# UVA-Computer-Vision-Lab/FrameINO

Measured on AMD Instinct MI355X. Metric: denoise-steps/sec (Wan2.2-5B FrameINO, 49f 704x1280, cond+uncond DiT forward + CFG + Euler), higher is better.
Workload: dtype bf16; 1 GPU; wan2.2-5b-49f-704x1280; layers=30, id_frames=1, hip_graph=False, parallelism=single, dead_rows_last_block=1760

## Files before the change

### frameino_amd/_lib.py

```python
import ctypes
import os
import re

_HERE = os.path.dirname(os.path.abspath(__file__))
LIB_PATH = os.environ.get("FINO_LIB_PATH") or os.path.join(_HERE, "lib", "libframeino_hip.so")
HEADER_PATH = os.path.join(os.path.dirname(_HERE), "include", "frameino_hip.h")

c_void_p, c_int, c_i64, c_float = ctypes.c_void_p, ctypes.c_int, ctypes.c_int64, ctypes.c_float

SIGNATURES = {
    "fino_version": [],
    "fino_last_error": [],
    "fino_tune_set": [c_int, c_int],
    "fino_tune_get": [c_int],
    "fino_adaln_modulate": [c_void_p, c_void_p, c_i64, c_int, c_i64, c_i64, c_void_p, c_void_p, c_i64, c_void_p,
                            c_float, c_int, c_void_p],
    "fino_layernorm": [c_void_p, c_void_p, c_i64, c_int, c_i64, c_i64, c_void_p, c_void_p, c_float, c_int, c_void_p],
    "fino_gated_residual": [c_void_p, c_void_p, c_void_p, c_i64, c_int, c_i64, c_i64, c_i64, c_void_p, c_i64,
                            c_void_p, c_int, c_void_p],
    "fino_gated_residual_staged": [c_void_p, c_void_p, c_void_p, c_i64, c_int, c_i64, c_i64, c_i64, c_void_p, c_i64,
                                   c_void_p, c_int, c_void_p],
    "fino_layernorm_zero": [c_void_p, c_void_p, c_i64, c_int, c_i64, c_i64, c_void_p, c_void_p, c_void_p, c_void_p,
                            c_i64, c_void_p, c_float, c_int, c_void_p],
    "fino_rmsnorm_rope": [c_void_p, c_i64, c_int, c_i64, c_void_p, c_float, c_void_p, c_void_p, c_int, c_int,
                          c_void_p],
    "fino_rmsnorm_rope_scaled": [c_void_p, c_i64, c_int, c_i64, c_void_p, c_float, c_void_p, c_void_p, c_int, c_float,
                                 c_int, c_void_p],
    "fino_qkv_rmsnorm_rope": [c_void_p, c_i64, c_int, c_i64, c_void_p, c_float, c_void_p, c_float, c_void_p, c_void_p, c_int,
                              c_float, c_void_p, c_void_p, c_void_p, c_int, c_void_p],
    "fino_rmsnorm_rope_scatter": [c_void_p, c_i64, c_int, c_i64, c_void_p, c_float, c_void_p, c_void_p, c_int, c_float,
                                  c_void_p, c_void_p, c_void_p, c_int, c_void_p],
    "fino_diag_mfma_peak": [c_int, c_int, c_int, c_void_p, ctypes.POINTER(ctypes.c_double), c_void_p],
    "fino_headnorm_rope": [c_void_p, c_int, c_i64, c_int, c_int, c_i64, c_i64, c_void_p, c_void_p, c_float,
                           c_void_p, c_void_p, c_i64, c_int, c_void_p],
    "fino_headnorm_rope_scaled": [c_void_p, c_int, c_i64, c_int, c_int, c_i64, c_i64, c_void_p, c_void_p, c_float,
                                  c_void_p, c_void_p, c_i64, c_float, c_int, c_void_p],
    "fino_attn_fwd": [c_void_p] * 4 + [c_int, c_int, c_i64, c_i64, c_int] + [c_i64] * 12 + [c_float, c_int, c_void_p],
    "fino_attn_fwd_ws": [c_void_p] * 4 + [c_int, c_int, c_i64, c_i64, c_int] + [c_i64] * 12 +
                        [c_float, c_int, c_void_p, c_i64, c_void_p],
    "fino_attn_workspace_bytes": [c_int, c_int, c_i64, c_i64, c_int],
    "fino_attn_tail_supported": [c_int, c_int, c_i64, c_i64, c_int],
    "fino_attn_ranges_supported": [c_int, c_int, c_i64, c_i64, c_int],
    "fino_attn_fwd_ranges": [c_void_p] * 4 + [c_int, c_int, c_i64, c_i64, c_int] + [c_i64] * 12 + [c_float, c_int, c_void_p, c_void_p],
    "fino_attn_tiles_supported": [c_int, c_int, c_i64, c_i64, c_int],
    "fino_attn_fwd_tiles": [c_void_p] * 4 + [c_int, c_int, c_i64, c_i64, c_int] + [c_i64] * 12 + [c_float, c_int, c_void_p, c_i64, c_i64,
                                                                                             c_int, c_void_p],
    "fino_attn_tile_plan_bytes": [c_int, c_int, c_i64, c_i64, c_int],
    "fino_attn_tile_plan": [c_void_p] * 2 + [c_int, c_int, c_i64, c_i64, c_int] + [c_i64] * 6 + [c_float, c_int, c_float, c_void_p,
                                                                                             c_void_p, c_int, c_void_p, c_i64, c_void_p],
    "fino_attn_tile_plan_gated_bytes": [c_int, c_int, c_i64, c_i64, c_int],
    "fino_attn_tile_plan_gated": [c_void_p] * 2 + [c_int, c_int, c_i64, c_i64, c_int] + [c_i64] * 6 +
                                 [c_float, c_int, c_float, c_void_p, c_float, c_void_p, c_void_p, c_int, c_void_p, c_i64, c_void_p],
    "fino_attn_fp8_ranges_supported": [c_int, c_int, c_i64, c_i64, c_int],
    "fino_attn_fwd_fp8_ranges": [c_void_p] * 4 + [c_int, c_int, c_i64, c_i64, c_int] + [c_i64] * 8 + [c_float, c_int, c_int, c_void_p,
                                                                                               c_i64, c_int, c_void_p, c_void_p],
    "fino_attn_fwd_tail": [c_void_p] * 4 + [c_int, c_int, c_i64, c_i64, c_int] + [c_i64] * 12 + [c_float, c_int, c_void_p, c_void_p,
                                                                                            c_void_p],
    "fino_attn_probs_supported": [c_int, c_int, c_i64, c_i64, c_int],
    "fino_attn_probs": [c_void_p] * 3 + [c_int, c_int, c_i64, c_i64, c_int] + [c_i64] * 6 + [c_int, c_i64, c_i64, c_float, c_int,
                                                                                         c_void_p, c_void_p, c_void_p, c_i64,
                                                                                         c_void_p, c_void_p],
    "fino_row_rrms": [c_void_p, c_i64, c_int, c_i64, c_float, c_void_p, c_int, c_void_p],
    "fino_attn_fp8_kv_bytes": [c_int, c_int, c_i64, c_int],
    "fino_attn_fwd_fp8": [c_void_p] * 4 + [c_int, c_int, c_i64, c_i64, c_int] + [c_i64] * 8 + [c_float, c_int, c_int, c_void_p,
                                                                                           c_i64, c_void_p],
    "fino_attn_fp8_smooth_kv_bytes": [c_int, c_int, c_i64, c_int],
    "fino_attn_fwd_fp8_smooth": [c_void_p] * 4 + [c_int, c_int, c_i64, c_i64, c_int] + [c_i64] * 8 + [c_float, c_int, c_int,
                                                                                                  c_void_p, c_i64, c_void_p],
    "fino_attn_fp8_smoothed_kv_bytes": [c_int, c_int, c_i64, c_int, c_int],
    "fino_attn_fwd_fp8_smoothed": [c_void_p] * 4 + [c_int, c_int, c_i64, c_i64, c_int] + [c_i64] * 8 + [c_float, c_int, c_int,
                                                                                                    c_void_p, c_i64, c_void_p, c_int],
    "fino_attn_fp8_tiles_supported": [c_int, c_int, c_i64, c_i64, c_int],
    "fino_attn_fwd_fp8_tiles": [c_void_p] * 4 + [c_int, c_int, c_i64, c_i64, c_int] + [c_i64] * 8 + [c_float, c_int, c_int,
                                                                                                 c_void_p, c_i64, c_int, c_void_p,
                                                                                                 c_i64, c_i64, c_int, c_void_p],
    "fino_attn_partial_bytes": [c_int, c_int, c_i64, c_int],
    "fino_attn_partial": [c_void_p] * 3 + [c_int, c_int, c_i64, c_i64, c_int] + [c_i64] * 9 + [c_float, c_int, c_void_p,
                                                                                               c_i64, c_void_p],
    "fino_attn_merge": [c_void_p, c_int, c_int, c_i64, c_int, c_i64, c_i64, c_i64, c_void_p, c_void_p, c_void_p, c_int,
                        c_void_p],
    "fino_mxfp8_scale_bytes": [c_i64, c_i64],
    "fino_quantize_mxfp8": [c_void_p, c_void_p, c_void_p, c_i64, c_i64, c_i64, c_int, c_void_p],
    "fino_gemm_mxfp8": [c_void_p] * 6 + [c_i64] * 4 + [c_int, c_void_p, c_i64, c_void_p, c_i64, c_void_p, c_int, c_void_p],
    "fino_gemm_mxfp8_keep": [c_void_p] * 6 + [c_i64] * 4 + [c_int, c_void_p, c_i64, c_void_p, c_i64, c_void_p, c_int, c_void_p,
                             c_i64, c_void_p],
    "fino_gemm_mxfp8_q": [c_void_p] * 7 + [c_i64] * 3 + [c_int, c_int, c_void_p],
    "fino_mxfp6_bytes": [c_i64, c_i64],
    "fino_mxfp6_scale_bytes": [c_i64, c_i64],
    "fino_quantize_mxfp6": [c_void_p, c_void_p, c_void_p, c_i64, c_i64, c_i64, c_int, c_void_p],
    "fino_quantize_mxfp6_rot": [c_void_p, c_void_p, c_void_p, c_i64, c_i64, c_i64, c_int, c_int, c_void_p],
    "fino_gemm_mxfp6": [c_void_p] * 6 + [c_i64] * 4 + [c_int, c_void_p, c_i64, c_void_p, c_i64, c_void_p, c_int, c_void_p],
    "fino_gemm_mxfp6_keep": [c_void_p] * 6 + [c_i64] * 4 + [c_int, c_void_p, c_i64, c_void_p, c_i64, c_void_p, c_int, c_void_p,
                             c_i64, c_void_p],
    "fino_traj_paint": [c_void_p, c_void_p, c_void_p, c_int, c_int, c_int, c_int, c_void_p],
    "fino_traj_blur_quantize": [c_void_p, c_void_p, c_void_p, c_void_p, c_int, c_int, c_int, c_int, c_void_p],
    "fino_groupnorm_workspace_bytes": [c_int],
    "fino_groupnorm_cl": [c_void_p, c_void_p] + [c_int] * 6 + [c_void_p, c_void_p, c_float, c_void_p, c_void_p] +
                         [c_int] * 4 + [c_void_p, c_i64, c_int, c_void_p],
    "fino_avg_pool_time2": [c_void_p, c_void_p] + [c_int] * 5 + [c_void_p],
    "fino_resize_area_pad_u8": [c_void_p, c_void_p] + [c_int] * 9 + [c_void_p],
    "fino_u8_hwc_to_chw_unit": [c_void_p, c_void_p, c_int, c_int, c_void_p],
    "fino_gemm": [c_void_p] * 4 + [c_i64] * 6 + [c_int, c_void_p, c_i64, c_void_p, c_i64, c_void_p, c_int, c_void_p],
    "fino_gemm_split_n": [c_void_p] * 4 + [c_i64] * 6 + [c_int, c_void_p, c_i64, c_void_p, c_i64, c_void_p, c_int, c_void_p,
                          c_i64, c_i64, c_int, c_void_p],
    "fino_gemm_keep": [c_void_p] * 4 + [c_i64] * 6 + [c_int, c_void_p, c_i64, c_void_p, c_i64, c_void_p, c_int, c_void_p,
                       c_i64, c_int, c_void_p],
    "fino_ln_mxfp8": [c_int, c_void_p, c_void_p, c_void_p, c_i64, c_int, c_i64, c_void_p, c_void_p, c_void_p, c_void_p, c_i64,
                      c_void_p, c_float, c_int, c_void_p],
    "fino_gemm_blocked_a": [c_void_p, c_void_p, c_void_p, c_void_p, c_i64, c_i64, c_i64, c_i64, c_i64, c_int, c_i64, c_i64, c_i64,
                            c_i64, c_void_p, c_i64, c_void_p, c_i64, c_void_p, c_int, c_int, c_void_p],
    "fino_gemm_plan": [c_i64, c_i64, ctypes.POINTER(c_i64), ctypes.POINTER(c_int)],
    "fino_skinny_linear": [c_void_p, c_void_p, c_void_p, c_void_p, c_int, c_i64, c_i64, c_int, c_int, c_void_p],
    "fino_patchify": [c_void_p, c_void_p] + [c_int] * 7 + [c_i64, c_int, c_void_p],
    "fino_unpatchify": [c_void_p, c_void_p] + [c_int] * 7 + [c_i64, c_int, c_void_p],
    "fino_wan_model_input": [c_void_p] * 5 + [c_int] * 6 + [c_void_p],
    "fino_cfg_euler_step": [c_void_p, c_void_p, c_void_p] + [c_int] * 5 + [c_float, c_void_p, c_int, c_int, c_void_p],
    "fino_cfg_unipc_step": [c_void_p] * 6 + [c_int] * 5 + [c_void_p, c_int, c_void_p],
    "fino_cfg_vpred_step": [c_void_p, c_void_p, c_i64, c_i64, c_void_p, c_int, c_int, c_void_p],
    "fino_cfg_dpm_step": [c_void_p, c_void_p, c_void_p, c_void_p, c_i64, c_i64, c_void_p, c_int, c_int, c_void_p],
    "fino_conv3d": [c_void_p] * 4 + [c_int] * 19 + [c_void_p, c_void_p, c_int, c_void_p],
    "fino_rmsnorm_silu_cl": [c_void_p, c_void_p, c_i64, c_int, c_int, c_void_p, c_int, c_int, c_void_p],
    "fino_split_bf16": [c_void_p, c_void_p, c_i64, c_int, c_i64, c_i64, c_int, ctypes.c_uint, c_void_p],
    "fino_rmsnorm_silu_cl_f32": [c_void_p, c_void_p, c_i64, c_int, c_int, c_void_p, c_int, c_int, ctypes.c_uint, c_void_p],
    "fino_conv3d_split": [c_void_p] * 4 + [c_int] * 20 + [c_void_p, c_void_p, c_void_p],
    "fino_vae_blend_tiles": [c_void_p, c_void_p] + [c_int] * 9 + [c_void_p],
    "fino_softmax_rows": [c_void_p, c_i64, c_int, c_i64, c_float, c_int, c_void_p],
    "fino_dup_up3d_add": [c_void_p] * 3 + [c_int] * 10 + [c_void_p],
    "fino_avg_down3d_add": [c_void_p] * 3 + [c_int] * 10 + [c_void_p],
    "fino_vae_unpatchify_clamp": [c_void_p, c_void_p] + [c_int] * 7 + [c_void_p],
    "fino_vae_patchify": [c_void_p, c_void_p] + [c_int] * 7 + [c_void_p],
    "fino_lora_merge": [c_void_p, c_i64, c_void_p, c_i64, c_i64, c_i64, c_int, ctypes.POINTER(c_void_p),
                        ctypes.POINTER(c_i64), ctypes.POINTER(c_void_p), ctypes.POINTER(c_i64), ctypes.POINTER(c_int),
                        ctypes.POINTER(c_float), c_int, c_void_p],
    "fino_step_cache_probe": [c_void_p, c_int, c_i64, c_void_p, c_void_p, c_int, c_void_p],
    "fino_step_cache_residual": [c_void_p, c_i64, c_void_p, c_i64, c_void_p, c_i64, c_i64, c_i64, c_int, c_int, c_void_p],
    "fino_pab_broadcast": [c_void_p, c_i64, c_void_p, c_i64, c_void_p, c_i64, c_i64, c_i64, c_void_p, c_i64, c_void_p, c_int,
                           c_void_p],
    "fino_taylor_update": [c_void_p, c_i64, c_void_p, c_i64, c_i64, c_i64, c_i64, c_int, c_int, c_int, c_int, c_int, c_void_p],
    "fino_taylor_predict": [c_void_p, c_i64, c_i64, c_int, ctypes.POINTER(c_float), c_void_p, c_i64, c_void_p, c_i64, c_i64, c_i64,
                            c_void_p, c_i64, c_void_p, c_int, c_int, c_void_p],
}


class StepCacheSegment(ctypes.Structure):
    _fields_ = [("h0", c_void_p), ("h1", c_void_p), ("p", c_void_p), ("r", c_void_p), ("h1_copy", c_void_p),
                ("rows", c_i64), ("ld_h0", c_i64), ("ld_h1", c_i64), ("ld_p", c_i64), ("ld_r", c_i64), ("ld_h1_copy", c_i64)]
_RESTYPES = {"fino_last_error": ctypes.c_char_p, "fino_attn_workspace_bytes": c_i64, "fino_mxfp8_scale_bytes": c_i64,
             "fino_groupnorm_workspace_bytes": c_i64,
             "fino_attn_partial_bytes": c_i64, "fino_attn_fp8_kv_bytes": c_i64, "fino_attn_fp8_smooth_kv_bytes": c_i64,
             "fino_attn_fp8_smoothed_kv_bytes": c_i64, "fino_mxfp6_bytes": c_i64,
             "fino_mxfp6_scale_bytes": c_i64, "fino_attn_tile_plan_bytes": c_i64,
             "fino_attn_tile_plan_gated_bytes": c_i64}


ABI_VERSION = 103


def declared_symbols(header_path=HEADER_PATH):
    text = open(header_path).read()
    text = re.sub(r"/\*.*?\*/", "", text, flags=re.S)
    return sorted(set(re.findall(r"\b(fino_[a-z0-9_]+)\s*\(", text)))


def load(path=LIB_PATH):
    if not os.path.exists(path):
        raise RuntimeError(
            f"frameino_amd: HIP library not found at {path}. Build it with `python -c 'import __graft_entry__ as g; "
            f"g.build()'` (or `make -C frameino_amd/csrc`). There is no CPU fallback for the product path.")
    lib = ctypes.CDLL(path)
    lib.fino_version.restype = c_int
    if lib.fino_version() < 0 and os.environ.get("FINO_ALLOW_EXPERIMENT") != "1":
        raise RuntimeError(
            f"frameino_amd: {path} is a timing-EXPERIMENT build (compiled with -DFINO_EXPERIMENT: its kernels may skip "
            f"work and return wrong results; fino_version() = {lib.fino_version()}).  It is refused as the product library; "
            f"set FINO_ALLOW_EXPERIMENT=1 for the tools/ scripts that time it.")
    if abs(lib.fino_version()) != ABI_VERSION:
        raise RuntimeError(
            f"frameino_amd: {path} reports fino_version() = {lib.fino_version()}, this package binds ABI version "
            f"{ABI_VERSION} (include/frameino_hip.h: FINO_VERSION).  Rebuild it (`make -C frameino_amd/csrc`).")
    for name, argtypes in SIGNATURES.items():
        fn = getattr(lib, name)
        fn.argtypes = argtypes
        fn.restype = _RESTYPES.get(name, c_int)
    return lib


_lib = None


def lib():
    global _lib
    if _lib is None:
        _lib = load()
    return _lib


def check(rc, what=""):
    if rc != 0:
        raise RuntimeError(f"{what} failed ({rc}): {lib().fino_last_error().decode()}")
```

### frameino_amd/csrc/fino_attention_probs.hip

```cpp
#include <stdlib.h>

#include "fino_attention_common.h"
using namespace fino_attn_ns;

namespace {

struct ProbsParams {
    const uint16_t* q;
    const uint16_t* k;
    uint16_t* p;
    int batch, heads, lq, lk;
    int64_t q_bs, q_rs, q_hs, k_bs, k_rs, k_hs, p_bs, p_rs;
    int kp;
    const float* q_rrms;
    const uint16_t* q_weight;
    int64_t q_rrms_bs;
    float scale_log2;
    int lk_b[4];
    float log2_mult[4];
};

template <typename T, int NKB>
__global__ __launch_bounds__(256) void attn_probs_kernel(const ProbsParams p) {
    typedef typename T::vec8 vec8;
    __shared__ __attribute__((aligned(16))) char smem[4 * 8192];
    const int tid = threadIdx.x;
    const int lane = tid & 63;
    const int wave = tid >> 6;
    const int r = lane & 31;
    const int h = lane >> 5;
    const int hb = blockIdx.y;
    const int bi = hb / p.heads;
    const int head = hb - bi * p.heads;

    const int lkc = p.lk_b[bi < 4 ? bi : 3];
    const float lm = p.log2_mult[bi < 4 ? bi : 3];
    const int nkb = (lkc + 31) >> 5;
    const uint16_t* kp_ = p.k + bi * p.k_bs + head * p.k_hs;
    for (int i = 0; i < nkb * 2; ++i) {
        const int c = tid + 256 * i;
        const int row = c >> 4, ch = c & 15;
        uint4 u = make_uint4(0, 0, 0, 0);
        if (row < p.lk) u = *reinterpret_cast<const uint4*>(kp_ + (int64_t)row * p.k_rs + ch * 8);
        *reinterpret_cast<uint4*>(smem + row * 256 + ((ch ^ (row & 15)) << 4)) = u;
    }
    const int qrow = blockIdx.x * 128 + wave * 32 + r;
    const int qrc = qrow < p.lq ? qrow : p.lq - 1;
    const uint16_t* qp = p.q + bi * p.q_bs + head * p.q_hs + (int64_t)qrc * p.q_rs + 8 * h;
    vec8 qf[8];
    if (p.q_rrms) {
        const float rs = p.q_rrms[bi * p.q_rrms_bs + qrc];
        const uint16_t* wp = p.q_weight + head * 128 + 8 * h;
#pragma unroll
        for (int ks = 0; ks < 8; ++ks) {
            float f[8], ww[8];
            unpack8<T>(*reinterpret_cast<const uint4*>(qp + 16 * ks), f);
            unpack8<T>(*reinterpret_cast<const uint4*>(wp + 16 * ks), ww);
#pragma unroll
            for (int j = 0; j < 8; ++j) f[j] = round_to<T>(round_to<T>(f[j] * rs) * ww[j]);
            qf[ks] = __builtin_bit_cast(vec8, pack8<T>(f));
        }
    } else {
#pragma unroll
        for (int ks = 0; ks < 8; ++ks) qf[ks] = __builtin_bit_cast(vec8, *reinterpret_cast<const uint4*>(qp + 16 * ks));
    }
    __syncthreads();

    f32x16_t acc[NKB];
#pragma unroll
    for (int kb = 0; kb < NKB; ++kb)
#pragma unroll
        for (int j = 0; j < 16; ++j) acc[kb][j] = 0.f;
#pragma unroll
    for (int kb = 0; kb < NKB; ++kb) {
        if (kb < nkb) {
#pragma unroll
            for (int ks = 0; ks < 8; ++ks) {
                const int row = kb * 32 + r;
                const uint4 a = *reinterpret_cast<const uint4*>(smem + row * 256 + (((2 * ks + h) ^ (row & 15)) << 4));
                acc[kb] = T::mfma32(__builtin_bit_cast(vec8, a), qf[ks], acc[kb]);
            }
        }
    }

    const float c2 = p.scale_log2;
    float m = -INFINITY;
#pragma unroll
    for (int kb = 0; kb < NKB; ++kb) {
#pragma unroll
        for (int j = 0; j < 16; ++j) {
            const int key = kb * 32 + (j & 3) + 8 * (j >> 2) + 4 * h;
            float x = acc[kb][j] * c2;
            x = key == lkc - 1 ? x + lm : x;
            x = key >= lkc ? -INFINITY : x;
            acc[kb][j] = x;
            m = fmaxf(m, x);
        }
    }
    {
        const auto sw = __builtin_amdgcn_permlane32_swap(__float_as_uint(m), __float_as_uint(m), false, false);
        m = fmaxf(__uint_as_float(sw[0]), __uint_as_float(sw[1]));
    }
    float l = 0.f;
#pragma unroll
    for (int kb = 0; kb < NKB; ++kb) {
#pragma unroll
        for (int j = 0; j < 16; ++j) {
            const float e = __builtin_amdgcn_exp2f(acc[kb][j] - m);
            acc[kb][j] = e;
            l += e;
        }
    }
    {
        const auto sw = __builtin_amdgcn_permlane32_swap(__float_as_uint(l), __float_as_uint(l), false, false);
        l = __uint_as_float(sw[0]) + __uint_as_float(sw[1]);
    }
    const float inv = 1.0f / l;
    __syncthreads();
    char* stage = smem + wave * 8192;
#pragma unroll
    for (int kb = 0; kb < NKB; ++kb) {
#pragma unroll
        for (int g4 = 0; g4 < 4; ++g4) {
            const int key0 = kb * 32 + 8 * g4 + 4 * h;
            if (key0 < p.kp) {
                const uint32_t w0 = (uint32_t)T::from_f32(acc[kb][4 * g4 + 0] * inv) | ((uint32_t)T::from_f32(acc[kb][4 * g4 + 1] * inv) << 16);
                const uint32_t w1 = (uint32_t)T::from_f32(acc[kb][4 * g4 + 2] * inv) | ((uint32_t)T::from_f32(acc[kb][4 * g4 + 3] * inv) << 16);
                *reinterpret_cast<uint2*>(stage + r * 256 + ((((key0 >> 3)) ^ (r & 15)) << 4) + ((key0 & 4) << 1)) = make_uint2(w0, w1);
            }
        }
    }
    __syncthreads();
    const int pieces = p.kp >> 3;
    const int total = 32 * pieces;
    const int row_base = blockIdx.x * 128 + wave * 32;
    uint16_t* pbase = p.p + bi * p.p_bs + head * p.kp;
    for (int i = lane; i < total; i += 64) {
        const int rr = i / pieces, pc = i - rr * pieces;
        const uint4 u = *reinterpret_cast<const uint4*>(stage + rr * 256 + ((pc ^ (rr & 15)) << 4));
        if (row_base + rr < p.lq) *reinterpret_cast<uint4*>(pbase + (int64_t)(row_base + rr) * p.p_rs + pc * 8) = u;
    }
}

}

extern "C" int fino_attn_probs_supported(int batch, int heads, int64_t lq, int64_t lk, int head_dim) {
    return head_dim == 128 && batch >= 1 && batch <= 4 && heads > 0 && lq > 0 && lk >= 1 && lk <= 128 &&
           (int64_t)batch * heads <= 65535;
}

extern "C" int fino_attn_probs(const void* q, const void* k, void* p, int batch, int heads, int64_t lq, int64_t lk,
                               int head_dim, int64_t q_bs, int64_t q_rs, int64_t q_hs, int64_t k_bs, int64_t k_rs, int64_t k_hs,
                               int kp, int64_t p_bs, int64_t p_rs, float scale, int dtype, const int* lk_b,
                               const float* tail_mult, const float* q_rrms, int64_t q_rrms_bs, const void* q_weight,
                               void* stream) {
    FINO_CHECK((q_rrms == nullptr) == (q_weight == nullptr) && fino_aligned16(q_weight), FINO_ERR_ARG,
               "fino_attn_probs: q_rrms and q_weight come together (q_weight 16-byte aligned)");
    FINO_CHECK(dtype == FINO_BF16 || dtype == FINO_F16, FINO_ERR_ARG, "fino_attn_probs: dtype %d", dtype);
    FINO_CHECK(q && k && p && lk_b && tail_mult, FINO_ERR_ARG, "fino_attn_probs: null pointer");
    FINO_CHECK(fino_attn_probs_supported(batch, heads, lq, lk, head_dim), FINO_ERR_UNSUPPORTED,
               "fino_attn_probs: needs head_dim 128, batch <= 4, lk <= 128 (got head_dim %d, batch %d, lk %lld)", head_dim, batch,
               (long long)lk);
    FINO_CHECK(fino_aligned16(q) && fino_aligned16(k) && fino_aligned16(p) && q_rs % 8 == 0 && k_rs % 8 == 0 && q_hs % 8 == 0 &&
                   k_hs % 8 == 0 && q_bs % 8 == 0 && k_bs % 8 == 0 && p_bs % 8 == 0 && p_rs % 8 == 0,
               FINO_ERR_ARG, "fino_attn_probs: pointers and strides must be 16-byte aligned");
    FINO_CHECK(kp > 0 && kp % 8 == 0 && kp <= 128 && p_rs >= (int64_t)heads * kp, FINO_ERR_ARG,
               "fino_attn_probs: kp %d (a multiple of 8, <= 128), row stride %lld", kp, (long long)p_rs);
    FINO_CHECK(scale > 0.f || scale == FINO_ATTN_SCALE_FOLDED, FINO_ERR_ARG, "fino_attn_probs: scale");
    if (lq == 0) return FINO_OK;
    ProbsParams pp;
    pp.q = (const uint16_t*)q; pp.k = (const uint16_t*)k; pp.p = (uint16_t*)p;
    pp.batch = batch; pp.heads = heads; pp.lq = (int)lq; pp.lk = (int)lk;
    pp.q_bs = q_bs; pp.q_rs = q_rs; pp.q_hs = q_hs; pp.k_bs = k_bs; pp.k_rs = k_rs; pp.k_hs = k_hs; pp.p_bs = p_bs; pp.p_rs = p_rs;
    pp.kp = kp;
    pp.q_rrms = q_rrms; pp.q_weight = (const uint16_t*)q_weight; pp.q_rrms_bs = q_rrms_bs;
    pp.scale_log2 = scale == FINO_ATTN_SCALE_FOLDED ? 1.0f : scale * 1.4426950408889634f;
    for (int b = 0; b < 4; ++b) {
        const int bb = b < batch ? b : batch - 1;
        FINO_CHECK(lk_b[bb] >= 1 && lk_b[bb] <= lk && lk_b[bb] <= kp && tail_mult[bb] >= 1.0f, FINO_ERR_ARG,
                   "fino_attn_probs: lk_b[%d] = %d (of %lld, kp %d), tail_mult %g", bb, lk_b[bb], (long long)lk, kp,
                   (double)tail_mult[bb]);
        pp.lk_b[b] = lk_b[bb];
        pp.log2_mult[b] = log2f(tail_mult[bb]);
    }
    hipStream_t st = (hipStream_t)stream;
    const dim3 grid((unsigned)((lq + 127) / 128), (unsigned)(batch * heads));
    int max_lk = 0;
    for (int b = 0; b < batch; ++b) max_lk = lk_b[b] > max_lk ? lk_b[b] : max_lk;
    const int need = max_lk > kp ? max_lk : kp;
    const int nkb = need <= 64 ? 2 : (need <= 96 ? 3 : 4);
#define PROBS_LAUNCH(T_)                                                                                      \
    {                                                                                                         \
        if (nkb == 2) attn_probs_kernel<T_, 2><<<grid, 256, 0, st>>>(pp);                                     \
        else if (nkb == 3) attn_probs_kernel<T_, 3><<<grid, 256, 0, st>>>(pp);                                \
        else attn_probs_kernel<T_, 4><<<grid, 256, 0, st>>>(pp);                                              \
    }
    if (dtype == FINO_BF16) PROBS_LAUNCH(BF16) else PROBS_LAUNCH(F16)
#undef PROBS_LAUNCH
    FINO_LAUNCH_CHECK();
    return FINO_OK;
}
```

### frameino_amd/csrc/fino_gemm.hip

```cpp
#include <stdlib.h>

#include <atomic>
#include <type_traits>

#include "fino_gemm_common.h"

using namespace fino_gemm_ns;

#ifdef FINO_GEMM_STAMP
extern "C" int fino_gemm_debug_read(unsigned long long* out) {
    return (int)hipMemcpyFromSymbol(out, HIP_SYMBOL(fino_gemm_dbg), sizeof(unsigned long long) * 64);
}
#endif

namespace {

template <typename T, int EPI, bool GENERIC, bool CONV, bool KEEP = false>
__global__ __launch_bounds__(kThreads, 2) void gemm_kernel(const GemmParams p) {
    extern __shared__ __attribute__((aligned(16))) char smem[];
    typedef typename T::vec8 vec8;
    const int tid = threadIdx.x;
    const int lane = tid & 63;
    const int wave = tid >> 6;
    const int wm = wave >> 2;
// ... 518 lines not shown
    FINO_LAUNCH_CHECK();
    return FINO_OK;
}

template <typename T, int EPI, bool CONV = false, int MI = 8, bool ABLK = false, bool KEEP = false>
int launch_gemm_pp(const GemmParams& p, hipStream_t st) {
    static FinoPerDeviceOnce once;
    if (int rc = fino_max_smem_once(once, reinterpret_cast<const void*>(&gemm_pp_kernel<T, EPI, CONV, MI, ABLK, KEEP>), kSmemBytes, "fino_gemm")) return rc;
    gemm_pp_kernel<T, EPI, CONV, MI, ABLK, KEEP><<<dim3((unsigned)(p.tiles_m * p.tiles_n)), kThreads, kSmemBytes, st>>>(p);
    FINO_LAUNCH_CHECK();
    return FINO_OK;
}

inline int gemm_device_cus() {
    static std::atomic<int> cus[kFinoMaxDevices];
    const int dev = fino_current_device();
    int c = cus[dev].load(std::memory_order_relaxed);
    if (c == 0) {
        int n = 0;
        c = (hipDeviceGetAttribute(&n, hipDeviceAttributeMultiprocessorCount, dev) == hipSuccess && n > 0) ? n : 256;
        cus[dev].store(c, std::memory_order_relaxed);
    }
    return c;
}

struct TilePlan { int64_t rows1; int mi2; };
inline double plan_launch_cost(int64_t rows, int mi, int tiles_n, int cus) {
    if (rows <= 0) return 0.0;
    const double bm = 32.0 * mi;
    const int64_t tiles = ((rows + 32 * mi - 1) / (32 * mi)) * tiles_n;
    const double mfma_raw = 0.85 * bm / 256.0, mfma = mfma_raw > 0.80 ? mfma_raw : 0.80, deliver = (bm + 256.0) / 512.0;
    const int64_t full = tiles / cus, rem = tiles % cus;
    double c = (double)full * (mfma > deliver ? mfma : deliver);
    if (rem) {
        const double d = deliver * (double)rem / cus;
        c += mfma > d ? mfma : d;
    }
    return c + 0.07;
}
inline TilePlan plan_tiles_search(int64_t m, int tiles_n, int cus);
inline TilePlan plan_tiles(int64_t m, int tiles_n, int cus, int tile_m = 0) {
    const int forced = tile_m ? tile_m : fino_tune_get(FINO_TUNE_GEMM_TILE_M);
    if (forced >= 2 && forced <= 7) return TilePlan{0, forced};
    if (forced == 8 || m <= 0) return TilePlan{m, 8};
    static std::atomic<uint64_t> memo[64];
    const bool memoable = m < (1ll << 24) && tiles_n > 0 && tiles_n < 512 && cus > 0 && cus < 512;
    const uint64_t key = ((uint64_t)m << 18) | ((uint64_t)tiles_n << 9) | (uint64_t)cus;
    std::atomic<uint64_t>& slot = memo[(key * 0x9E3779B97F4A7C15ull) >> 58];
    if (memoable) {
        const uint64_t e = slot.load(std::memory_order_relaxed);
        if ((e & 1) && (e >> 22) == key) {
            const uint64_t r = (e >> 6) & 0xffff;
            return TilePlan{r == 0xffff ? m : (int64_t)r * 256, (int)((e >> 3) & 7) + 1};
        }
    }
    const TilePlan tp = plan_tiles_search(m, tiles_n, cus);
    if (memoable && (tp.rows1 == m || (tp.rows1 % 256 == 0 && tp.rows1 / 256 < 0xffff)) && tp.mi2 >= 2 && tp.mi2 <= 8)
        slot.store((key << 22) | ((tp.rows1 == m ? 0xffffull : (uint64_t)(tp.rows1 / 256)) << 6) |
                       ((uint64_t)(tp.mi2 - 1) << 3) | 1ull, std::memory_order_relaxed);
    return tp;
}
inline TilePlan plan_tiles_search(int64_t m, int tiles_n, int cus) {
    TilePlan best{m, 8};
    double best_c = plan_launch_cost(m, 8, tiles_n, cus);
    const double base_c = best_c;
    const int64_t rows256 = (m + 255) / 256;
    for (int64_t r1 = 0; r1 < rows256; ++r1) {
        const int64_t rows1 = r1 * 256;
        const double c1 = plan_launch_cost(rows1, 8, tiles_n, cus);
        for (int mi = 2; mi <= 8; ++mi) {
            if (rows1 > 0 && mi == 8) continue;
            const double c = c1 + plan_launch_cost(m - rows1, mi, tiles_n, cus);
            if (c < best_c - 1e-9) { best_c = c; best = TilePlan{rows1, mi}; }
        }
    }
    if (best_c > (best.rows1 > 0 ? 0.97 : 0.985) * base_c) return TilePlan{m, 8};
    return best;
}

inline bool use_pingpong() {
    static int v = -1;
    if (v < 0) {
        const char* e = getenv("FINO_GEMM_PP");
        v = (e && e[0] == '0') ? 0 : 1;
    }
    return v == 1;
}

template <typename T, int EPI, bool KEEP = false>
int launch_gemm_pp_mi(const GemmParams& p, int mi, hipStream_t st) {
    if constexpr (KEEP) {
        switch (mi) {
            case 2: return launch_gemm_pp<T, EPI, false, 2, false, true>(p, st);
            case 3: return launch_gemm_pp<T, EPI, false, 3, false, true>(p, st);
            case 4: return launch_gemm_pp<T, EPI, false, 4, false, true>(p, st);
            case 5: return launch_gemm_pp<T, EPI, false, 5, false, true>(p, st);
            case 6: return launch_gemm_pp<T, EPI, false, 6, false, true>(p, st);
            case 7: return launch_gemm_pp<T, EPI, false, 7, false, true>(p, st);
            default: return launch_gemm_pp<T, EPI, false, 8, false, true>(p, st);
        }
    }
    if (p.a_tpb > 0) {
        if constexpr (EPI == FINO_EPI_GATED_RESIDUAL) {
            switch (mi) {
                case 2: return launch_gemm_pp<T, EPI, false, 2, true>(p, st);
                case 3: return launch_gemm_pp<T, EPI, false, 3, true>(p, st);
                case 4: return launch_gemm_pp<T, EPI, false, 4, true>(p, st);
                case 5: return launch_gemm_pp<T, EPI, false, 5, true>(p, st);
                case 6: return launch_gemm_pp<T, EPI, false, 6, true>(p, st);
                case 7: return launch_gemm_pp<T, EPI, false, 7, true>(p, st);
                default: return launch_gemm_pp<T, EPI, false, 8, true>(p, st);
            }
        } else {
            fino_set_error("fino_gemm_blocked_a: epilogue must be FINO_EPI_GATED_RESIDUAL");
            return FINO_ERR_UNSUPPORTED;
        }
    }
    switch (mi) {
        case 2: return launch_gemm_pp<T, EPI, false, 2>(p, st);
        case 3: return launch_gemm_pp<T, EPI, false, 3>(p, st);
        case 4: return launch_gemm_pp<T, EPI, false, 4>(p, st);
        case 5: return launch_gemm_pp<T, EPI, false, 5>(p, st);
        case 6: return launch_gemm_pp<T, EPI, false, 6>(p, st);
        case 7: return launch_gemm_pp<T, EPI, false, 7>(p, st);
        default: return launch_gemm_pp<T, EPI, false, 8>(p, st);
    }
}

template <typename T, bool KEEP = false>
int launch_gemm_rows(GemmParams p, int64_t r0, int64_t rows, int mi, int epi, hipStream_t st) {
    p.a += r0 * p.lda;
    p.c += r0 * p.ldc;
    if (p.c2) p.c2 += r0 * p.ldc2;
    if (p.r) p.r += r0 * p.ldr;
    if (p.sel) p.sel += r0;
    p.m = rows;
    p.tiles_m = (int)((rows + 32 * mi - 1) / (32 * mi));
    if constexpr (KEEP) {
        switch (epi) {
            case FINO_EPI_RESIDUAL: return launch_gemm_pp_mi<T, FINO_EPI_RESIDUAL, true>(p, mi, st);
            case FINO_EPI_GATED_RESIDUAL_STAGED: return launch_gemm_pp_mi<T, FINO_EPI_GATED_RESIDUAL_STAGED, true>(p, mi, st);
            default: return launch_gemm_pp_mi<T, FINO_EPI_GATED_RESIDUAL, true>(p, mi, st);
        }
    }
    switch (epi) {
        case FINO_EPI_NONE: return launch_gemm_pp_mi<T, FINO_EPI_NONE>(p, mi, st);
        case FINO_EPI_GELU_TANH: return launch_gemm_pp_mi<T, FINO_EPI_GELU_TANH>(p, mi, st);
        case FINO_EPI_RESIDUAL: return launch_gemm_pp_mi<T, FINO_EPI_RESIDUAL>(p, mi, st);
        case FINO_EPI_GATED_RESIDUAL_STAGED: return launch_gemm_pp_mi<T, FINO_EPI_GATED_RESIDUAL_STAGED>(p, mi, st);
        default: return launch_gemm_pp_mi<T, FINO_EPI_GATED_RESIDUAL>(p, mi, st);
    }
}

template <typename T, bool GENERIC, bool KEEP = false>
int launch_gemm_e(const GemmParams& p, int epi, int tile_m, hipStream_t st) {
    const bool fits32 = ((p.m - 1) * p.lda + p.k) * 2 < (1ll << 31) && ((p.n - 1) * p.ldw + p.k) * 2 < (1ll << 31);
    if (epi == FINO_EPI_F32 || epi == FINO_EPI_F32_RESIDUAL) {
        if (GENERIC || !fits32) {
            fino_set_error("fino_gemm: the fp32-output epilogues need K %% 64 == 0, 16-byte aligned operands and operands < 2 GiB");
            return FINO_ERR_UNSUPPORTED;
        }
        return epi == FINO_EPI_F32 ? launch_gemm_pp<T, FINO_EPI_F32, false, 8>(p, st)
                                   : launch_gemm_pp<T, FINO_EPI_F32_RESIDUAL, false, 8>(p, st);
    }
    if (!GENERIC && use_pingpong() && fits32) {
        const TilePlan tp = plan_tiles(p.m, p.tiles_n, gemm_device_cus(), tile_m);
        if (tp.rows1 > 0)
            if (int rc = launch_gemm_rows<T, KEEP>(p, 0, tp.rows1, 8, epi, st)) return rc;
        if (tp.rows1 < p.m) return launch_gemm_rows<T, KEEP>(p, tp.rows1, p.m - tp.rows1, tp.mi2, epi, st);
        return FINO_OK;
    }
    if constexpr (KEEP) {
        switch (epi) {
            case FINO_EPI_RESIDUAL: return launch_gemm_t<T, FINO_EPI_RESIDUAL, GENERIC, false, true>(p, st);
            case FINO_EPI_GATED_RESIDUAL_STAGED: return launch_gemm_t<T, FINO_EPI_GATED_RESIDUAL_STAGED, GENERIC, false, true>(p, st);
            default: return launch_gemm_t<T, FINO_EPI_GATED_RESIDUAL, GENERIC, false, true>(p, st);
        }
    }
    switch (epi) {
        case FINO_EPI_NONE: return launch_gemm_t<T, FINO_EPI_NONE, GENERIC>(p, st);
        case FINO_EPI_GELU_TANH: return launch_gemm_t<T, FINO_EPI_GELU_TANH, GENERIC>(p, st);
        case FINO_EPI_RESIDUAL: return launch_gemm_t<T, FINO_EPI_RESIDUAL, GENERIC>(p, st);
        case FINO_EPI_GATED_RESIDUAL_STAGED: return launch_gemm_t<T, FINO_EPI_GATED_RESIDUAL_STAGED, GENERIC>(p, st);
        default: return launch_gemm_t<T, FINO_EPI_GATED_RESIDUAL, GENERIC>(p, st);
    }
}

template <int WT>
__global__ __launch_bounds__(256) void skinny_linear_kernel(const float* __restrict__ x, const void* __restrict__ w,
                                                            const void* __restrict__ b, float* __restrict__ y, int m,
                                                            int64_t n, int64_t k, int silu_input) {
    const int lane = threadIdx.x & 63;
    const int64_t col = (int64_t)blockIdx.x * 4 + (threadIdx.x >> 6);
    if (col >= n) return;
    float acc[16];
#pragma unroll
    for (int i = 0; i < 16; ++i) acc[i] = 0.f;
    for (int64_t kk = lane; kk < k; kk += 64) {
        float wv;
        if (WT == -1) wv = ((const float*)w)[col * k + kk];
        else if (WT == FINO_BF16) wv = BF16::to_f32(((const uint16_t*)w)[col * k + kk]);
        else wv = F16::to_f32(((const uint16_t*)w)[col * k + kk]);
#pragma unroll
        for (int i = 0; i < 16; ++i) {
            if (i < m) {
                float xv = x[(int64_t)i * k + kk];
                if (silu_input) xv = xv / (1.0f + __expf(-xv));
                acc[i] += xv * wv;
            }
        }
    }
    float bias = 0.f;
    if (b) {
        if (WT == -1) bias = ((const float*)b)[col];
        else if (WT == FINO_BF16) bias = BF16::to_f32(((const uint16_t*)b)[col]);
        else bias = F16::to_f32(((const uint16_t*)b)[col]);
    }
#pragma unroll
    for (int i = 0; i < 16; ++i) {
        if (i < m) {
            const float s = wave_sum(acc[i]);
            if (lane == 0) y[(int64_t)i * n + col] = s + bias;
        }
    }
}

}

extern "C" int fino_gemm_plan(int64_t m, int64_t n, int64_t* rows_256, int* tile_rows_rest) {
    if (m <= 0 || n <= 0) return FINO_ERR_ARG;
    const TilePlan tp = plan_tiles(m, (int)((n + BN - 1) / BN), gemm_device_cus());
    if (rows_256) *rows_256 = tp.rows1;
    if (tile_rows_rest) *tile_rows_rest = tp.rows1 < m ? 32 * tp.mi2 : 0;
    return FINO_OK;
}

extern "C" int fino_gemm(const void* a, const void* w, const void* bias, void* c, int64_t m, int64_t n, int64_t k,
                         int64_t lda, int64_t ldw, int64_t ldc, int epilogue, const void* r, int64_t ldr,
                         const float* gate, int64_t mod_stride, const int32_t* sel, int dtype, void* stream) {
    return fino_gemm_split_n(a, w, bias, c, m, n, k, lda, ldw, ldc, epilogue, r, ldr, gate, mod_stride, sel, dtype, nullptr,
                             0, 0, 0, stream);
}

static int gemm_impl(const void* a, const void* w, const void* bias, void* c, int64_t m, int64_t n, int64_t k, int64_t lda,
                     int64_t ldw, int64_t ldc, int epilogue, const void* r, int64_t ldr, const float* gate,
                     int64_t mod_stride, const int32_t* sel, int dtype, void* c2, int64_t ldc2, int64_t n_split, void* keep,
                     int64_t ldk, int tile_m, void* stream) {
    FINO_CHECK(dtype == FINO_BF16 || dtype == FINO_F16, FINO_ERR_ARG, "fino_gemm: dtype %d", dtype);
    FINO_CHECK(tile_m == 0 || (tile_m >= 2 && tile_m <= 8), FINO_ERR_ARG, "fino_gemm: tile_m=%d (0 = planned, 2 .. 8)", tile_m);
    if (c2 || n_split) {
        FINO_CHECK(c2 && n_split > 0 && n_split < n && n_split % BN == 0 && ldc2 % 8 == 0 && ldc2 >= n - n_split &&
                       fino_aligned16(c2) && k % BK == 0 && epilogue <= FINO_EPI_GELU_TANH,
                   FINO_ERR_ARG,
                   "fino_gemm_split_n: needs c2, 0 < n_split < N a multiple of %d, ldc2 >= N - n_split, K %% %d == 0, no "
                   "residual epilogue", BN, BK);
        FINO_CHECK(ldc >= n_split, FINO_ERR_ARG, "fino_gemm_split_n: ldc must cover the first n_split columns");
    }
    FINO_CHECK(a && w && c, FINO_ERR_ARG, "fino_gemm: null pointer");
    FINO_CHECK(m >= 0 && n > 0 && k > 0, FINO_ERR_ARG, "fino_gemm: bad shape M=%lld N=%lld K=%lld", (long long)m,
               (long long)n, (long long)k);
    FINO_CHECK(n % 8 == 0 && k % 8 == 0, FINO_ERR_ARG, "fino_gemm: N=%lld and K=%lld must be multiples of 8",
               (long long)n, (long long)k);
    FINO_CHECK(lda % 8 == 0 && ldw % 8 == 0 && ldc % 8 == 0 && lda >= k && ldw >= k && ldc >= (n_split > 0 ? n_split : n),
               FINO_ERR_ARG, "fino_gemm: leading dimensions must be multiples of 8 and cover the row");
    FINO_CHECK(fino_aligned16(a) && fino_aligned16(w) && fino_aligned16(c), FINO_ERR_ARG,
               "fino_gemm: A/W/C must be 16-byte aligned");
    FINO_CHECK(epilogue >= FINO_EPI_NONE && epilogue <= FINO_EPI_F32_RESIDUAL, FINO_ERR_ARG,
               "fino_gemm: epilogue %d", epilogue);
    if (epilogue == FINO_EPI_F32 || epilogue == FINO_EPI_F32_RESIDUAL)
        FINO_CHECK(!c2 && tile_m == 0 && fino_aligned16(bias), FINO_ERR_ARG,
                   "fino_gemm: the fp32-output epilogues take one output, the planned tiling and a 16-byte aligned fp32 bias");
    if (epilogue >= FINO_EPI_RESIDUAL && epilogue != FINO_EPI_F32)
        FINO_CHECK(r && ldr % 8 == 0 && ldr >= n && fino_aligned16(r), FINO_ERR_ARG, "fino_gemm: residual operand");
    if (epilogue == FINO_EPI_GATED_RESIDUAL || epilogue == FINO_EPI_GATED_RESIDUAL_STAGED)
        FINO_CHECK(gate && fino_aligned16(gate) && mod_stride % 4 == 0, FINO_ERR_ARG, "fino_gemm: gate operand");
    if (m == 0) return FINO_OK;
    GemmParams p = {};
    p.c2 = (uint16_t*)c2; p.ldc2 = ldc2; p.n_split = n_split;
    if (keep) { p.c2 = (uint16_t*)keep; p.ldc2 = ldk; p.n_split = 0; }
    p.a = (const uint16_t*)a; p.w = (const uint16_t*)w; p.bias = (const uint16_t*)bias; p.c = (uint16_t*)c;
    p.r = (const uint16_t*)r; p.gate = gate; p.sel = sel;
    p.m = m; p.n = n; p.k = k; p.lda = lda; p.ldw = ldw; p.ldc = ldc; p.ldr = ldr; p.mod_stride = mod_stride;
    p.tiles_m = (int)((m + BM - 1) / BM);
    p.tiles_n = (int)((n + BN - 1) / BN);
    p.group_m = fino_tune_get(FINO_TUNE_GEMM_GROUP_M);
    hipStream_t st = (hipStream_t)stream;
    const bool generic = (k % BK) != 0;
    if (p.group_m <= 0) p.group_m = gemm_default_group_m(p.tiles_n, k);
    {
        const int rk = fino_tune_get(FINO_TUNE_GEMM_RASTER);
        if (rk == 1 || (rk == 3 && (k >= 8192 || n >= 8192)) || (rk != 2 && rk != 3 && k >= 8192)) p.group_m |= 0x100;
    }
    if (keep) {
        if (dtype == FINO_BF16)
            return generic ? launch_gemm_e<BF16, true, true>(p, epilogue, tile_m, st)
                           : launch_gemm_e<BF16, false, true>(p, epilogue, tile_m, st);
        return generic ? launch_gemm_e<F16, true, true>(p, epilogue, tile_m, st)
                       : launch_gemm_e<F16, false, true>(p, epilogue, tile_m, st);
    }
    if (dtype == FINO_BF16)
        return generic ? launch_gemm_e<BF16, true>(p, epilogue, tile_m, st) : launch_gemm_e<BF16, false>(p, epilogue, tile_m, st);
    return generic ? launch_gemm_e<F16, true>(p, epilogue, tile_m, st) : launch_gemm_e<F16, false>(p, epilogue, tile_m, st);
}

extern "C" int fino_gemm_split_n(const void* a, const void* w, const void* bias, void* c, int64_t m, int64_t n, int64_t k,
                                 int64_t lda, int64_t ldw, int64_t ldc, int epilogue, const void* r, int64_t ldr,
                                 const float* gate, int64_t mod_stride, const int32_t* sel, int dtype, void* c2,
                                 int64_t ldc2, int64_t n_split, int tile_m, void* stream) {
    return gemm_impl(a, w, bias, c, m, n, k, lda, ldw, ldc, epilogue, r, ldr, gate, mod_stride, sel, dtype, c2, ldc2, n_split,
                     nullptr, 0, tile_m, stream);
}

extern "C" int fino_gemm_keep(const void* a, const void* w, const void* bias, void* c, int64_t m, int64_t n, int64_t k,
                              int64_t lda, int64_t ldw, int64_t ldc, int epilogue, const void* r, int64_t ldr,
                              const float* gate, int64_t mod_stride, const int32_t* sel, int dtype, void* keep, int64_t ldk,
                              int tile_m, void* stream) {
    FINO_CHECK(dtype == FINO_BF16 || dtype == FINO_F16, FINO_ERR_ARG, "fino_gemm_keep: dtype %d", dtype);
    FINO_CHECK(epilogue == FINO_EPI_RESIDUAL || epilogue == FINO_EPI_GATED_RESIDUAL ||
                   epilogue == FINO_EPI_GATED_RESIDUAL_STAGED,
               FINO_ERR_ARG, "fino_gemm_keep: epilogue %d (the residual epilogues %d, %d and %d keep y)", epilogue,
               FINO_EPI_RESIDUAL, FINO_EPI_GATED_RESIDUAL, FINO_EPI_GATED_RESIDUAL_STAGED);
    FINO_CHECK(keep && fino_aligned16(keep) && ldk % 8 == 0 && ldk >= n, FINO_ERR_ARG,
               "fino_gemm_keep: needs a 16-byte aligned keep buffer with ldk >= N a multiple of 8");
    return gemm_impl(a, w, bias, c, m, n, k, lda, ldw, ldc, epilogue, r, ldr, gate, mod_stride, sel, dtype, nullptr, 0, 0,
                     keep, ldk, tile_m, stream);
}

extern "C" int fino_gemm_blocked_a(const void* a, const void* w, const void* bias, void* c, int64_t m, int64_t n, int64_t k,
                                   int64_t a_block_k, int64_t a_block_stride, int a_groups, int64_t a_group_stride,
                                   int64_t lda, int64_t ldw, int64_t ldc,
                                   const void* r, int64_t ldr, const float* gate, int64_t mod_stride, const int32_t* sel,
                                   int dtype, int tile_m, void* stream) {
    FINO_CHECK(dtype == FINO_BF16 || dtype == FINO_F16, FINO_ERR_ARG, "fino_gemm_blocked_a: dtype %d", dtype);
    FINO_CHECK(tile_m == 0 || (tile_m >= 2 && tile_m <= 8), FINO_ERR_ARG, "fino_gemm_blocked_a: tile_m=%d (0 = planned, 2 .. 8)",
               tile_m);
    FINO_CHECK(a && w && c && r && gate, FINO_ERR_ARG, "fino_gemm_blocked_a: null pointer");
    FINO_CHECK(m >= 0 && n > 0 && k > 0 && n % 8 == 0, FINO_ERR_ARG, "fino_gemm_blocked_a: bad shape");
    FINO_CHECK(a_block_k > 0 && a_block_k % BK == 0 && k % a_block_k == 0 && a_block_k / BK <= 256 && k / BK <= 4096,
               FINO_ERR_ARG, "fino_gemm_blocked_a: a_block_k=%lld must be a multiple of %d dividing K=%lld",
               (long long)a_block_k, BK, (long long)k);
    FINO_CHECK(lda % 8 == 0 && lda >= a_block_k && a_block_stride % 8 == 0 && ldw % 8 == 0 && ldw >= k && ldc % 8 == 0 &&
                   ldc >= n && ldr % 8 == 0 && ldr >= n && mod_stride % 4 == 0,
               FINO_ERR_ARG, "fino_gemm_blocked_a: leading dimensions");
    FINO_CHECK(fino_aligned16(a) && fino_aligned16(w) && fino_aligned16(c) && fino_aligned16(r) && fino_aligned16(gate),
               FINO_ERR_ARG, "fino_gemm_blocked_a: 16-byte alignment required");
    const int64_t nblk = k / a_block_k;
    FINO_CHECK(a_groups >= 1 && a_groups <= 16 && nblk % a_groups == 0 && a_group_stride % 8 == 0, FINO_ERR_ARG,
               "fino_gemm_blocked_a: a_groups=%d must divide the %lld K blocks", a_groups, (long long)nblk);
    const int64_t span = ((a_groups - 1) * a_group_stride + (nblk / a_groups - 1) * a_block_stride +
                          (m > 0 ? m - 1 : 0) * lda + a_block_k) * 2;
    FINO_CHECK(span < (1ll << 31) && ((n - 1) * ldw + k) * 2 < (1ll << 31), FINO_ERR_ARG,
               "fino_gemm_blocked_a: operands must span < 2 GiB");
    if (m == 0) return FINO_OK;
    GemmParams p = {};
    p.a = (const uint16_t*)a; p.w = (const uint16_t*)w; p.bias = (const uint16_t*)bias; p.c = (uint16_t*)c;
    p.r = (const uint16_t*)r; p.gate = gate; p.sel = sel;
    p.m = m; p.n = n; p.k = k; p.lda = lda; p.ldw = ldw; p.ldc = ldc; p.ldr = ldr; p.mod_stride = mod_stride;
    p.a_tpb = (int)(a_block_k / BK); p.a_inv = (65536 + p.a_tpb - 1) / p.a_tpb; p.a_blk_elems = a_block_stride;
    p.a_groups = a_groups; p.a_ginv = (65536 + a_groups - 1) / a_groups; p.a_grp_elems = a_group_stride;
    FINO_CHECK((k / BK - 1) * ((int64_t)p.a_inv * p.a_tpb - 65536) < 65536 &&
                   (nblk - 1) * ((int64_t)p.a_ginv * a_groups - 65536) < 65536,
               FINO_ERR_UNSUPPORTED,
               "fino_gemm_blocked_a: a_block_k=%lld / a_groups=%d with K=%lld is beyond the exact range of the kernel's "
               "reciprocal index arithmetic", (long long)a_block_k, a_groups, (long long)k);
    p.tiles_m = (int)((m + BM - 1) / BM);
    p.tiles_n = (int)((n + BN - 1) / BN);
    p.group_m = fino_tune_get(FINO_TUNE_GEMM_GROUP_M);
    if (p.group_m <= 0) p.group_m = gemm_default_group_m(p.tiles_n, k);
    hipStream_t st = (hipStream_t)stream;
    const TilePlan tp = plan_tiles(p.m, p.tiles_n, gemm_device_cus(), tile_m);
    auto rows = [&](int64_t r0, int64_t nr, int mi) {
        return dtype == FINO_BF16 ? launch_gemm_rows<BF16>(p, r0, nr, mi, FINO_EPI_GATED_RESIDUAL, st)
                                  : launch_gemm_rows<F16>(p, r0, nr, mi, FINO_EPI_GATED_RESIDUAL, st);
    };
    if (tp.rows1 > 0)
        if (int rc = rows(0, tp.rows1, 8)) return rc;
    if (tp.rows1 < p.m) return rows(tp.rows1, p.m - tp.rows1, tp.mi2);
    return FINO_OK;
}

static int conv3d_impl(const void* x, const void* w, const void* bias, void* y, int t_in, int h_in, int w_in,
                       int c_in_pad, int t_out, int h_out, int w_out, int c_out_pad, int kt, int kh, int kw, int st,
                       int sh, int sw, int pt, int ph, int pw, int upsample2x, int epilogue, const void* r,
                       const void* zero_page, int dtype, int planes, void* stream);

extern "C" int fino_conv3d(const void* x, const void* w, const void* bias, void* y, int t_in, int h_in, int w_in,
                           int c_in_pad, int t_out, int h_out, int w_out, int c_out_pad, int kt, int kh, int kw, int st,
                           int sh, int sw, int pt, int ph, int pw, int upsample2x, int epilogue, const void* r,
                           const void* zero_page, int dtype, void* stream) {
    return conv3d_impl(x, w, bias, y, t_in, h_in, w_in, c_in_pad, t_out, h_out, w_out, c_out_pad, kt, kh, kw, st, sh, sw, pt, ph,
                       pw, upsample2x, epilogue, r, zero_page, dtype, 0, stream);
}

extern "C" int fino_conv3d_split(const void* x_planes, const void* w_products, const float* bias, float* y, int t_in, int h_in,
                                 int w_in, int c_in_pad, int planes, int t_out, int h_out, int w_out, int c_out_pad, int kt,
                                 int kh, int kw, int st, int sh, int sw, int pt, int ph, int pw, int upsample2x, int epilogue,
                                 const float* r, const void* zero_page, void* stream) {
    FINO_CHECK(planes == 2 || planes == 3, FINO_ERR_ARG, "fino_conv3d_split: planes = %d (2: hi | lo, 3: hi | mid | lo)", planes);
    return conv3d_impl(x_planes, w_products, bias, y, t_in, h_in, w_in, c_in_pad, t_out, h_out, w_out, c_out_pad, kt, kh, kw, st,
                       sh, sw, pt, ph, pw, upsample2x, epilogue, r, zero_page, FINO_BF16, planes, stream);
}

static int conv3d_impl(const void* x, const void* w, const void* bias, void* y, int t_in, int h_in, int w_in,
                       int c_in_pad, int t_out, int h_out, int w_out, int c_out_pad, int kt, int kh, int kw, int st,
                       int sh, int sw, int pt, int ph, int pw, int upsample2x, int epilogue, const void* r,
                       const void* zero_page, int dtype, int planes, void* stream) {
    FINO_CHECK(dtype == FINO_BF16 || dtype == FINO_F16, FINO_ERR_ARG, "fino_conv3d: dtype %d", dtype);
    FINO_CHECK(x && w && y && zero_page, FINO_ERR_ARG, "fino_conv3d: null pointer");
    FINO_CHECK(c_in_pad > 0 && c_in_pad % BK == 0, FINO_ERR_ARG,
               "fino_conv3d: c_in_pad=%d must be a multiple of %d (pad channels with zeros)", c_in_pad, BK);
    FINO_CHECK(c_out_pad > 0 && c_out_pad % 8 == 0, FINO_ERR_ARG, "fino_conv3d: c_out_pad=%d %% 8 != 0", c_out_pad);
    FINO_CHECK(t_in > 0 && h_in > 0 && w_in > 0 && t_out > 0 && h_out > 0 && w_out > 0 && kt > 0 && kh > 0 && kw > 0 &&
                   st > 0 && sh > 0 && sw > 0 && pt >= 0 && ph >= 0 && pw >= 0,
               FINO_ERR_ARG, "fino_conv3d: bad geometry");
    FINO_CHECK(epilogue == FINO_EPI_NONE || (epilogue == FINO_EPI_RESIDUAL && r), FINO_ERR_ARG,
               "fino_conv3d: epilogue %d (NONE or RESIDUAL with r)", epilogue);
    FINO_CHECK(fino_aligned16(x) && fino_aligned16(w) && fino_aligned16(y) && fino_aligned16(r) &&
                   fino_aligned16(zero_page),
               FINO_ERR_ARG, "fino_conv3d: 16-byte alignment required");
    FINO_CHECK(planes == 0 || fino_aligned16(bias), FINO_ERR_ARG, "fino_conv3d_split: bias must be 16-byte aligned");
    const int products = planes == 0 ? 1 : (planes == 2 ? 3 : 6);
    const int64_t a_width = (int64_t)(planes == 0 ? 1 : planes) * c_in_pad;
    GemmParams p = {};
    p.a = (const uint16_t*)x; p.w = (const uint16_t*)w; p.bias = (const uint16_t*)bias; p.c = (uint16_t*)y;
    p.r = (const uint16_t*)r; p.gate = nullptr; p.sel = nullptr;
    p.m = (int64_t)t_out * h_out * w_out; p.n = c_out_pad; p.k = (int64_t)kt * kh * kw * c_in_pad * products;
    p.lda = a_width; p.ldw = p.k; p.ldc = c_out_pad; p.ldr = c_out_pad; p.mod_stride = 0;
    p.a_cc = planes == 0 ? 0 : c_in_pad / BK; p.a_nplanes = planes;
    p.tiles_m = (int)((p.m + BM - 1) / BM); p.tiles_n = (int)((p.n + BN - 1) / BN);
    p.group_m = fino_tune_get(FINO_TUNE_GEMM_GROUP_M);
    p.to = t_out; p.ho = h_out; p.wo = w_out; p.ti = t_in; p.hi = h_in; p.wi = w_in;
    p.kt = kt; p.kh = kh; p.kw = kw; p.st = st; p.sh = sh; p.sw = sw; p.pt = pt; p.ph = ph; p.pw = pw;
    p.up = upsample2x; p.cin_chunks = c_in_pad / BK * products; p.zero_page = (const uint16_t*)zero_page;
    hipStream_t s = (hipStream_t)stream;
    const int64_t hw_out = (int64_t)h_out * w_out;
    const int64_t t_span = (BM - 1 + hw_out - 1) / hw_out + 1;
    const int64_t in_span_bytes = (t_span * st + kt) * (int64_t)h_in * w_in * a_width * 2;
    const bool pp = use_pingpong() && fino_tune_get(FINO_TUNE_CONV_LOOP) != 1 && in_span_bytes < (1ll << 31) &&
                    h_out < 4096 && w_out < 4096 && t_span < 256 && c_out_pad % 32 == 0 && ((p.n - 1) * p.ldw + p.k) * 2 < (1ll << 31);
    if (planes > 0) {
        if (!pp) {
            fino_set_error("fino_conv3d_split: a 256-row tile's input span (%lld bytes) exceeds the 2 GiB the gather offsets cover, "
                           "or c_out_pad %% 32 != 0 -- run the layer in chunks of fewer frames", (long long)in_span_bytes);
            return FINO_ERR_UNSUPPORTED;
        }
        return epilogue == FINO_EPI_NONE ? launch_gemm_pp<BF16, FINO_EPI_F32, true>(p, s)
                                         : launch_gemm_pp<BF16, FINO_EPI_F32_RESIDUAL, true>(p, s);
    }
    if (pp) {
        if (dtype == FINO_BF16)
            return epilogue == FINO_EPI_NONE ? launch_gemm_pp<BF16, FINO_EPI_NONE, true>(p, s)
                                             : launch_gemm_pp<BF16, FINO_EPI_RESIDUAL, true>(p, s);
        return epilogue == FINO_EPI_NONE ? launch_gemm_pp<F16, FINO_EPI_NONE, true>(p, s)
                                         : launch_gemm_pp<F16, FINO_EPI_RESIDUAL, true>(p, s);
    }
// ... 22 lines not shown
```

### frameino_amd/ops.py

```python
import math
import os

import torch

from . import _lib

BF16, F16 = 0, 1
EPI_NONE, EPI_GELU_TANH, EPI_RESIDUAL, EPI_GATED_RESIDUAL, EPI_GATED_RESIDUAL_STAGED = 0, 1, 2, 3, 4
EPI_F32, EPI_F32_RESIDUAL = 5, 6


class KernelTimer:

    active = None

    def __init__(self, names):
        self.names = set(names)
        self.events = {n: [] for n in self.names}
        self.flops = {}
        self.bytes = {}

    def __enter__(self):
        KernelTimer.active = self
        return self
# ... 314 lines not shown

def attention_tile_plan_gated_bytes(b, heads, lq, lk, dh):
    return int(_lib.lib().fino_attn_tile_plan_gated_bytes(int(b), int(heads), int(lq), int(lk), int(dh)))


def attention_tile_plan(q, k, heads, cdf, keep_ranges=None, scale=None, out=None, workspace=None, cdf_heads=None,
                        similarity_threshold=None, return_similarity=False):
    assert q.dim() == 3 and k.dim() == 3 and q.shape[0] == k.shape[0] and q.shape[2] == k.shape[2]
    for t in (q, k):
        assert t.stride(2) == 1 and t.is_cuda
    b, lq, hd = q.shape
    lk = k.shape[1]
    dh = hd // heads
    nqb, words = (lq + 255) // 256, ((lk + 63) // 64 + 31) // 32
    if keep_ranges is not None:
        _check_ranges(keep_ranges, lq)
    if cdf_heads is not None:
        assert isinstance(cdf_heads, torch.Tensor) and cdf_heads.dtype == torch.float32 and cdf_heads.is_cuda and \
            cdf_heads.is_contiguous() and tuple(cdf_heads.shape) == (heads,), \
            f"cdf_heads: a contiguous fp32 device tensor [{heads}] is needed, got {getattr(cdf_heads, 'dtype', type(cdf_heads))} " \
            f"{tuple(getattr(cdf_heads, 'shape', ()))}"
    gate = similarity_threshold is not None
    if gate:
        theta = float(similarity_threshold)
        assert 0.0 < theta <= 1.0, f"similarity_threshold = {similarity_threshold!r}: a number in (0, 1] is needed"
    assert gate or not return_similarity, "return_similarity needs similarity_threshold: the similarities are computed under the gate only"
    if out is None:
        out = torch.empty((b, heads, nqb, words), dtype=torch.int32, device=q.device)
    assert out.dtype in _MASK_DTYPES and out.is_cuda and out.is_contiguous() and \
        tuple(out.shape[:3]) == (b, heads, nqb) and out.dim() == 4 and out.shape[3] * 32 >= (lk + 63) // 64, \
        f"out: a contiguous int32 device tensor [{b}, {heads}, {nqb}, >= {words}] is needed, got {out.dtype} {tuple(out.shape)}"
    plain = _lib.lib().fino_attn_tile_plan_bytes(b, heads, lq, lk, dh)
    need = _lib.lib().fino_attn_tile_plan_gated_bytes(b, heads, lq, lk, dh) if gate else plain
    if need <= 0:
        raise NotImplementedError(f"attention_tile_plan: B={b} H={heads} Lq={lq} Lk={lk} head_dim={dh} is not supported "
                                  f"(head_dim 64 | 128, at most 65536 keys)")
    if workspace is None:
        key = (q.device.index, torch.cuda.current_stream().cuda_stream)
        workspace = _plan_ws.get(key)
        if workspace is None or workspace.numel() * 4 < need:
            workspace = _plan_ws[key] = torch.empty(need // 4, dtype=torch.float32, device=q.device)
    assert workspace.dtype == torch.float32 and workspace.is_cuda and workspace.is_contiguous() and workspace.numel() * 4 >= need
    scale = dh ** -0.5 if scale is None else scale
    ev = _timed("attn_tile_plan")
    if cdf_heads is None and not gate:
        _lib.check(_lib.lib().fino_attn_tile_plan(_p(q), _p(k), b, heads, lq, lk, dh, q.stride(0), q.stride(1), dh,
                                                 k.stride(0), k.stride(1), dh, float(scale), _dt(q), float(cdf),
                                                 _p(keep_ranges), _p(out), out.shape[3], _p(workspace), workspace.numel() * 4,
                                                 _stream()), "fino_attn_tile_plan")
    else:
        _lib.check(_lib.lib().fino_attn_tile_plan_gated(_p(q), _p(k), b, heads, lq, lk, dh, q.stride(0), q.stride(1), dh,
                                                       k.stride(0), k.stride(1), dh, float(scale), _dt(q), float(cdf),
                                                       _p(cdf_heads), theta if gate else 0.0, _p(keep_ranges), _p(out),
                                                       out.shape[3], _p(workspace), workspace.numel() * 4, _stream()),
                   "fino_attn_tile_plan_gated")
    if ev is not None:
        ev.record()
    if return_similarity:
        nt = (lk + 63) // 64
        tail = workspace[plain // 4:plain // 4 + b * heads * (nqb + nt)]
        return out, (tail[:b * heads * nqb].view(b, heads, nqb).clone(), tail[b * heads * nqb:].view(b, heads, nt).clone())
    return out


def _timed_tiles_done(ev, mask, b, heads, lq, lk, hd, dh):
    ev.record()
    kt_ = KernelTimer.active
    bits = _tile_mask_bits(mask, lk).expand(b, heads, -1, -1).to(torch.float64)
    keys = torch.full((bits.shape[-1],), 64.0, dtype=torch.float64)
    keys[-1] = lk - 64 * (bits.shape[-1] - 1)
    rows = torch.tensor([min(256, lq - 256 * i) for i in range(bits.shape[2])], dtype=torch.float64)
    pairs = float(((bits * keys).sum(-1) * rows).sum())
    kt_.flops["attn_self"] = kt_.flops.get("attn_self", 0.0) + 4.0 * pairs * dh
    kt_.bytes["attn_self"] = kt_.bytes.get("attn_self", 0.0) + 2.0 * b * hd * (2 * lq + 2 * lk)


def attention_tiles(q, k, v, heads, mask, out=None, scale=None):
    b, lq, lk, hd, dh, out, scale = _attn_args(q, k, v, heads, out, scale)
    words, mask_bs, mask_hs = _check_tile_mask(mask, b, heads, lq, lk)
    ev = _timed("attn_self")
    _lib.check(_lib.lib().fino_attn_fwd_tiles(_p(q), _p(k), _p(v), _p(out), b, heads, lq, lk, dh,
                                             q.stride(0), q.stride(1), dh, k.stride(0), k.stride(1), dh,
                                             v.stride(0), v.stride(1), dh, out.stride(0), out.stride(1), dh,
                                             float(scale), _dt(q), _p(mask), mask_bs, mask_hs, words, _stream()),
               "fino_attn_fwd_tiles")
    if ev is not None:
        _timed_tiles_done(ev, mask, b, heads, lq, lk, hd, dh)
    return out


def attention_tail_supported(b, heads, lq, lk, dh):
    return bool(_lib.lib().fino_attn_tail_supported(int(b), int(heads), int(lq), int(lk), int(dh)))


def attention_tail(q, k, v, heads, lk_b, tail_mult, out=None, scale=None):
    import ctypes
    b, lq, lk, hd, dh, out, scale = _attn_args(q, k, v, heads, out, scale)
    assert len(lk_b) == b and len(tail_mult) == b
    lk_arr = (ctypes.c_int * b)(*[int(x) for x in lk_b])
    mult_arr = (ctypes.c_float * b)(*[float(x) for x in tail_mult])
    ev = _timed("attn_cross")
    _lib.check(_lib.lib().fino_attn_fwd_tail(_p(q), _p(k), _p(v), _p(out), b, heads, lq, lk, dh,
                                            q.stride(0), q.stride(1), dh, k.stride(0), k.stride(1), dh,
                                            v.stride(0), v.stride(1), dh, out.stride(0), out.stride(1), dh,
                                            float(scale), _dt(q), ctypes.cast(lk_arr, ctypes.c_void_p),
                                            ctypes.cast(mult_arr, ctypes.c_void_p), _stream()), "fino_attn_fwd_tail")
    if ev is not None:
        ev.record()
        kt_ = KernelTimer.active
        kt_.flops["attn_cross"] = kt_.flops.get("attn_cross", 0.0) + 4.0 * lq * hd * sum(int(x) for x in lk_b)
    return out


def attention_probs_supported(b, heads, lq, lk, dh):
    return bool(_lib.lib().fino_attn_probs_supported(int(b), int(heads), int(lq), int(lk), int(dh)))


def row_rrms(x, eps, out=None):
    x2, rows, dim, ldx = _rows2d(x)
    if out is None:
        out = torch.empty(rows, dtype=torch.float32, device=x.device)
    assert out.dtype == torch.float32 and out.is_contiguous() and out.numel() >= rows
    _lib.check(_lib.lib().fino_row_rrms(_p(x2), rows, dim, ldx, float(eps), _p(out), _dt(x), _stream()), "fino_row_rrms")
    return out


def attention_probs(q, k, heads, lk_b, tail_mult, kp, out=None, scale=None, q_rrms=None, q_weight=None):
    import ctypes
    assert q.dim() == 3 and k.dim() == 3
    b, lq, hd = q.shape
    lk = k.shape[1]
    dh = hd // heads
    for t in (q, k):
        assert t.stride(2) == 1 and t.is_cuda
    if out is None:
        out = torch.empty((b, lq, heads * kp), dtype=q.dtype, device=q.device)
    assert out.shape == (b, lq, heads * kp) and out.stride(2) == 1
    scale = dh ** -0.5 if scale is None else scale
    lk_arr = (ctypes.c_int * b)(*[int(x) for x in lk_b])
    mult_arr = (ctypes.c_float * b)(*[float(x) for x in tail_mult])
    ev = _timed("attn_cross")
    _lib.check(_lib.lib().fino_attn_probs(_p(q), _p(k), _p(out), b, heads, lq, lk, dh, q.stride(0), q.stride(1), dh,
                                         k.stride(0), k.stride(1), dh, int(kp), out.stride(0), out.stride(1), float(scale),
                                         _dt(q), ctypes.cast(lk_arr, ctypes.c_void_p), ctypes.cast(mult_arr, ctypes.c_void_p),
                                         _p(q_rrms), q_rrms.stride(0) if q_rrms is not None else 0, _p(q_weight), _stream()),
               "fino_attn_probs")
    if ev is not None:
        ev.record()
        kt_ = KernelTimer.active
        kt_.flops["attn_cross"] = kt_.flops.get("attn_cross", 0.0) + 2.0 * lq * hd * sum(int(x) for x in lk_b)
    return out


_attn_fp8_ws = {}


FP8_P_EXP2, FP8_P_RAMP = 0, 1
FP8_P_MODES = {"exp2": FP8_P_EXP2, "ramp": FP8_P_RAMP}
_p_env = os.environ.get("FINO_FP8_P_MODE", "ramp")
if _p_env not in FP8_P_MODES:
    raise ValueError(f"FINO_FP8_P_MODE={_p_env!r}: expected one of {' | '.join(FP8_P_MODES)} (how the opt-in fp8 attention turns a "
                     f"softmax weight into its e4m3 byte; 'ramp' -- a piecewise-linear exp2, the default since round 4 -- adds "
                     f"~0.3e-2 to the 5.5e-2 rel-RMS of the fp8 operands, 'exp2' is the exact form)")
FP8_P_DEFAULT = FP8_P_MODES[_p_env]


def _attn_fp8_workspace(need, device):
    key = (device.index, torch.cuda.current_stream().cuda_stream)
    ws = _attn_fp8_ws.get(key)
    if ws is None or ws.numel() < need:
        ws = _attn_fp8_ws[key] = torch.empty(need, dtype=torch.uint8, device=device)
    return ws


def _fp8_smooth_flags(smooth_k, smooth_v):
    return (1 if smooth_k else 0) | (2 if smooth_v else 0)


def attention_fp8(q, k, v, heads, out=None, scale=None, p_mode=None, smooth_k=False, smooth_v=False):
    p_mode = FP8_P_DEFAULT if p_mode is None else FP8_P_MODES.get(p_mode, p_mode)
    b, lq, lk, hd, dh, out, scale = _attn_args(q, k, v, heads, out, scale)
    flags = _fp8_smooth_flags(smooth_k, smooth_v)
    fwd = "fino_attn_fwd_fp8_smoothed" if smooth_v else ("fino_attn_fwd_fp8_smooth" if smooth_k else "fino_attn_fwd_fp8")
    need = _lib.lib().fino_attn_fp8_smoothed_kv_bytes(b, heads, lk, dh, flags)
    if need <= 0:
        raise RuntimeError(f"attention_fp8: head_dim {dh} is not supported (64 or 128)")
    ws = _attn_fp8_workspace(need, q.device)
    done = _timed_attn(b, lq, lk, hd)
    _lib.check(getattr(_lib.lib(), fwd)(_p(q), _p(k), _p(v), _p(out), b, heads, lq, lk, dh, q.stride(0), q.stride(1),
                                        k.stride(0), k.stride(1), v.stride(0), v.stride(1), out.stride(0), out.stride(1),
                                        float(scale), _dt(q), int(p_mode), _p(ws), need, _stream(),
                                        *((flags,) if smooth_v else ())), fwd)
    if done is not None:
        done()
    return out


def attention_fp8_ranges_supported(b, heads, lq, lk, dh):
    return bool(_lib.lib().fino_attn_fp8_ranges_supported(int(b), int(heads), int(lq), int(lk), int(dh)))


def attention_fp8_ranges(q, k, v, heads, ranges, out=None, scale=None, p_mode=None, smooth_k=False, smooth_v=False):
    p_mode = FP8_P_DEFAULT if p_mode is None else FP8_P_MODES.get(p_mode, p_mode)
    b, lq, lk, hd, dh, out, scale = _attn_args(q, k, v, heads, out, scale)
    _check_ranges(ranges, lq)
    if dh != 64:
        raise RuntimeError(f"attention_fp8_ranges: head_dim {dh} is not supported (64 only)")
    flags = _fp8_smooth_flags(smooth_k, smooth_v)
    need = _lib.lib().fino_attn_fp8_smoothed_kv_bytes(b, heads, lk, dh, flags)
    ws = _attn_fp8_workspace(need, q.device)
    done = _timed_attn(b, lq, lk, hd, ranges)
    _lib.check(_lib.lib().fino_attn_fwd_fp8_ranges(_p(q), _p(k), _p(v), _p(out), b, heads, lq, lk, dh, q.stride(0), q.stride(1),
                                                  k.stride(0), k.stride(1), v.stride(0), v.stride(1), out.stride(0),
                                                  out.stride(1), float(scale), _dt(q), int(p_mode), _p(ws), need,
                                                  flags, _p(ranges), _stream()), "fino_attn_fwd_fp8_ranges")
    if done is not None:
        done()
    return out


def attention_fp8_tiles_supported(b, heads, lq, lk, dh):
    return bool(_lib.lib().fino_attn_fp8_tiles_supported(int(b), int(heads), int(lq), int(lk), int(dh)))


def attention_fp8_tiles(q, k, v, heads, mask, out=None, scale=None, p_mode=None, smooth_k=False, smooth_v=False):
    p_mode = FP8_P_DEFAULT if p_mode is None else FP8_P_MODES.get(p_mode, p_mode)
    b, lq, lk, hd, dh, out, scale = _attn_args(q, k, v, heads, out, scale)
    words, mask_bs, mask_hs = _check_tile_mask(mask, b, heads, lq, lk)
    if dh != 128:
        raise RuntimeError(f"attention_fp8_tiles: head_dim {dh} is not supported (the fp8 tile walk exists for head_dim 128 only)")
    flags = _fp8_smooth_flags(smooth_k, smooth_v)
    need = _lib.lib().fino_attn_fp8_smoothed_kv_bytes(b, heads, lk, dh, flags)
    ws = _attn_fp8_workspace(need, q.device)
    ev = _timed("attn_self")
    _lib.check(_lib.lib().fino_attn_fwd_fp8_tiles(_p(q), _p(k), _p(v), _p(out), b, heads, lq, lk, dh, q.stride(0), q.stride(1),
                                                 k.stride(0), k.stride(1), v.stride(0), v.stride(1), out.stride(0),
                                                 out.stride(1), float(scale), _dt(q), int(p_mode), _p(ws), need, flags,
                                                 _p(mask), mask_bs, mask_hs, words, _stream()), "fino_attn_fwd_fp8_tiles")
    if ev is not None:
        _timed_tiles_done(ev, mask, b, heads, lq, lk, hd, dh)
    return out


def attention_partial_floats(batch, heads, lq, head_dim):
    return _lib.lib().fino_attn_partial_bytes(batch, heads, lq, head_dim) // 4


def attention_partial(q, k, v, heads, out=None, scale=None):
    assert q.dim() == 3 and k.dim() == 3 and v.dim() == 3
    b, lq, hd = q.shape
    lk = k.shape[1]
    dh = hd // heads
    for t in (q, k, v):
        assert t.stride(2) == 1 and t.is_cuda
    need = _lib.lib().fino_attn_partial_bytes(b, heads, lq, dh)
    if out is None or out.numel() * 4 < need:
        out = torch.empty(need // 4, dtype=torch.float32, device=q.device)
    scale = dh ** -0.5 if scale is None else scale
    _lib.check(_lib.lib().fino_attn_partial(_p(q), _p(k), _p(v), b, heads, lq, lk, dh, q.stride(0), q.stride(1), dh,
                                           k.stride(0), k.stride(1), dh, v.stride(0), v.stride(1), dh, float(scale),
                                           _dt(q), _p(out), need, _stream()), "fino_attn_partial")
    return out


def attention_merge(parts, batch, lq, heads, head_dim, dtype, out=None):
    assert 1 <= len(parts) <= 3
    if out is None:
        out = torch.empty((batch, lq, heads * head_dim), dtype=dtype, device=parts[0].device)
    ps = list(parts) + [None] * (3 - len(parts))
    _lib.check(_lib.lib().fino_attn_merge(_p(out), batch, heads, lq, head_dim, out.stride(0), out.stride(1), head_dim,
                                         _p(ps[0]), _p(ps[1]), _p(ps[2]), _dt(out), _stream()), "fino_attn_merge")
    return out


def gemm_plan(m, n):
    import ctypes
    r, t = ctypes.c_int64(), ctypes.c_int()
    _lib.check(_lib.lib().fino_gemm_plan(m, n, ctypes.byref(r), ctypes.byref(t)), "fino_gemm_plan")
    return r.value, t.value


def gemm(a, w, bias=None, epilogue=EPI_NONE, residual=None, gate=None, sel=None, out=None, out2=None, split=0, tile_m=0,
         keep=None):
    a2, m, k, lda = _rows2d(a)
    assert w.dim() == 2 and w.stride(1) == 1 and w.shape[1] == k and w.dtype == a.dtype
    n = w.shape[0]
    if out is None:
        out = torch.empty((m, split or n), dtype=a.dtype, device=a.device)
    o2, _, _, ldc = _rows2d(out)
    if out2 is not None:
        if keep is not None:
            raise ValueError("gemm: keep= goes with a residual epilogue, out2= / split= with none: they do not combine")
        assert 0 < split < n and residual is None
        c2, _, _, ldc2 = _rows2d(out2)
        done = _timed_gemm(None, 2.0 * m * n * k)
        _lib.check(_lib.lib().fino_gemm_split_n(_p(a2), _p(w), _p(bias), _p(o2), m, n, k, lda, w.stride(0), ldc, epilogue,
                                               0, 0, 0, 0, 0, _dt(a), _p(c2), ldc2, split, tile_m, _stream()),
                   "fino_gemm_split_n")
        if done is not None:
            done()
        return out, out2
    r2, ldr, ms = _epi_operands(residual, gate)
    if bias is not None:
        assert bias.dtype == a.dtype and bias.is_contiguous()
    done = _timed_gemm(epilogue, 2.0 * m * n * k, 2.0 * (m * k + n * k + m * n * (2 if residual is not None else 1)))
    if keep is not None:
        k2, km, kn, ldk = _rows2d(keep)
        assert (km, kn) == (m, n) and keep.dtype == a.dtype and keep.is_cuda
        _lib.check(_lib.lib().fino_gemm_keep(_p(a2), _p(w), _p(bias), _p(o2), m, n, k, lda, w.stride(0), ldc, epilogue,
                                            _p(r2), ldr, _p(gate), ms, _p(sel), _dt(a), _p(k2), ldk, tile_m, _stream()),
                   "fino_gemm_keep")
    elif tile_m:
        _lib.check(_lib.lib().fino_gemm_split_n(_p(a2), _p(w), _p(bias), _p(o2), m, n, k, lda, w.stride(0), ldc, epilogue,
                                               _p(r2), ldr, _p(gate), ms, _p(sel), _dt(a), None, 0, 0, tile_m, _stream()),
                   "fino_gemm_split_n")
    else:
        _lib.check(_lib.lib().fino_gemm(_p(a2), _p(w), _p(bias), _p(o2), m, n, k, lda, w.stride(0), ldc, epilogue, _p(r2),
                                       ldr, _p(gate), ms, _p(sel), _dt(a), _stream()), "fino_gemm")
    if done is not None:
        done()
    return out


def gemm_blocked_a(a_blocks, rows, w, bias, residual, gate, sel, out, tile_m=0):
    if a_blocks.dim() == 3:
        a_blocks = a_blocks[None]
    assert a_blocks.dim() == 4 and a_blocks.stride(3) == 1 and w.dtype == a_blocks.dtype and w.stride(1) == 1
    groups, peers, _, bk = a_blocks.shape
    n, k = w.shape
    assert k == groups * peers * bk and residual.shape == (rows, n) and out.shape == (rows, n)
    r2, _, _, ldr = _rows2d(residual)
    o2, _, _, ldc = _rows2d(out)
    ms = gate.stride(0) if gate.dim() == 2 else 0
    done = _timed_gemm(None, 2.0 * rows * n * k)
    _lib.check(_lib.lib().fino_gemm_blocked_a(_p(a_blocks), _p(w), _p(bias), _p(o2), rows, n, k, bk, a_blocks.stride(1),
                                              groups, a_blocks.stride(0), a_blocks.stride(2), w.stride(0), ldc, _p(r2),
                                              ldr, _p(gate), ms, _p(sel), _dt(a_blocks), tile_m, _stream()),
               "fino_gemm_blocked_a")
    if done is not None:
        done()
    return out


def quantize_mxfp8(x, out=None):
    x2, rows, cols, ldx = _rows2d(x)
    nbytes = _lib.lib().fino_mxfp8_scale_bytes(rows, cols)
    if nbytes <= 0:
        raise ValueError(f"quantize_mxfp8: cols={cols} must be a positive multiple of 128")
    q, s = _mx_pair((rows, cols), nbytes, x.device, out)
    _lib.check(_lib.lib().fino_quantize_mxfp8(_p(x2), _p(q), _p(s), rows, cols, ldx, _dt(x), _stream()),
               "fino_quantize_mxfp8")
    return q, s


def ln_mxfp8(mode, x, weight=None, bias=None, shift=None, scale=None, sel=None, eps=1e-6, out=None):
    x2, rows, dim, ldx = _rows2d(x)
    nbytes = _lib.lib().fino_mxfp8_scale_bytes(rows, dim)
    if nbytes <= 0:
        raise ValueError(f"ln_mxfp8: dim={dim} must be a positive multiple of 128")
    q, s = _mx_pair((rows, dim), nbytes, x.device, out)
    for t in (weight, bias, shift, scale):
        assert t is None or t.dtype == torch.float32
    ms = shift.stride(0) if (shift is not None and shift.dim() == 2) else 0
    _lib.check(_lib.lib().fino_ln_mxfp8(mode, _p(x2), _p(q), _p(s), rows, dim, ldx, _p(weight), _p(bias), _p(shift),
                                       _p(scale), ms, _p(sel), eps, _dt(x), _stream()), "fino_ln_mxfp8")
    return q, s


def _mx_gemm(entry, aq, a_scales, wq, w_scales, bias, epilogue, residual, gate, sel, out, out_dtype, m, n, k, keep=None):
    if out is None:
        out = torch.empty((m, n), dtype=out_dtype, device=aq.device)
    o2, _, _, ldc = _rows2d(out)
    r2, ldr, ms = _epi_operands(residual, gate)
    done = _timed_gemm(None, 2.0 * m * n * k)
    if keep is not None:
        k2, km, kn, ldk = _rows2d(keep)
        assert (km, kn) == (m, n) and keep.dtype == out.dtype and keep.is_cuda
        entry += "_keep"
        _lib.check(getattr(_lib.lib(), entry)(_p(aq), _p(a_scales), _p(wq), _p(w_scales), _p(bias), _p(o2), m, n, k, ldc,
                                              epilogue, _p(r2), ldr, _p(gate), ms, _p(sel), _dt(out), _p(k2), ldk, _stream()),
                   entry)
    else:
        _lib.check(getattr(_lib.lib(), entry)(_p(aq), _p(a_scales), _p(wq), _p(w_scales), _p(bias), _p(o2), m, n, k, ldc,
                                              epilogue, _p(r2), ldr, _p(gate), ms, _p(sel), _dt(out), _stream()), entry)
    if done is not None:
        done()
    return out


def gemm_mxfp8(aq, a_scales, wq, w_scales, bias=None, epilogue=EPI_NONE, residual=None, gate=None, sel=None, out=None,
               out_dtype=torch.bfloat16, keep=None):
    m, k = aq.shape
    n = wq.shape[0]
    assert wq.shape[1] == k and aq.dtype == torch.uint8 and wq.dtype == torch.uint8 and aq.is_contiguous() \
        and wq.is_contiguous()
    return _mx_gemm("fino_gemm_mxfp8", aq, a_scales, wq, w_scales, bias, epilogue, residual, gate, sel, out, out_dtype, m, n, k,
                    keep)


def gemm_mxfp8_q(aq, a_scales, wq, w_scales, bias, epilogue=EPI_NONE, out=None):
    m, k = aq.shape
    n = wq.shape[0]
    assert bias is not None and wq.shape[1] == k
    q, s = _mx_pair((m, n), _lib.lib().fino_mxfp8_scale_bytes(m, n), aq.device, out)
    done = _timed_gemm(None, 2.0 * m * n * k)
    _lib.check(_lib.lib().fino_gemm_mxfp8_q(_p(aq), _p(a_scales), _p(wq), _p(w_scales), _p(bias), _p(q), _p(s), m, n, k,
                                           epilogue, _dt(bias), _stream()), "fino_gemm_mxfp8_q")
    if done is not None:
        done()
    return q, s


MX_ROTATE = {"act": 1, "weight": 2}


def quantize_mxfp6(x, out=None, rotate=None):
    if rotate is not None and rotate not in MX_ROTATE:
        raise ValueError(f"quantize_mxfp6: rotate={rotate!r} must be None, 'act' or 'weight'")
    x2, rows, cols, ldx = _rows2d(x)
    nbytes = _lib.lib().fino_mxfp6_scale_bytes(rows, cols)
    if nbytes <= 0:
        raise ValueError(f"quantize_mxfp6: cols={cols} must be a positive multiple of 128")
    q, s = _mx_pair(_lib.lib().fino_mxfp6_bytes(rows, cols), nbytes, x.device, out)
    if rotate is None:
        _lib.check(_lib.lib().fino_quantize_mxfp6(_p(x2), _p(q), _p(s), rows, cols, ldx, _dt(x), _stream()),
                   "fino_quantize_mxfp6")
    else:
        _lib.check(_lib.lib().fino_quantize_mxfp6_rot(_p(x2), _p(q), _p(s), rows, cols, ldx, _dt(x), MX_ROTATE[rotate],
                                                     _stream()), "fino_quantize_mxfp6_rot")
    q.mx_shape = (rows, cols)
    return q, s


def gemm_mxfp6(aq, a_scales, wq, w_scales, bias=None, epilogue=EPI_NONE, residual=None, gate=None, sel=None, out=None,
               out_dtype=torch.bfloat16, m=None, n=None, k=None, keep=None):
    assert aq.dtype == torch.uint8 and wq.dtype == torch.uint8 and aq.is_contiguous() and wq.is_contiguous()
    sa_, sw_ = getattr(aq, "mx_shape", None), getattr(wq, "mx_shape", None)
    m = m if m is not None else (sa_[0] if sa_ else None)
    n = n if n is not None else (sw_[0] if sw_ else None)
    k = k if k is not None else (sa_[1] if sa_ else (sw_[1] if sw_ else None))
    if m is None or n is None or k is None:
        raise ValueError("gemm_mxfp6: operands without mx_shape need m / n / k")
    if sw_ and sw_[1] != k:
        raise ValueError(f"gemm_mxfp6: K of A ({k}) and of W ({sw_[1]}) differ")
    lib = _lib.lib()
    if aq.numel() != lib.fino_mxfp6_bytes(m, k) or wq.numel() != lib.fino_mxfp6_bytes(n, k):
        raise ValueError(f"gemm_mxfp6: operand sizes {aq.numel()} / {wq.numel()} do not match M={m} N={n} K={k}")
    return _mx_gemm("fino_gemm_mxfp6", aq, a_scales, wq, w_scales, bias, epilogue, residual, gate, sel, out, out_dtype, m, n, k,
                    keep)


def skinny_linear(x, w, b=None, silu_input=False):
    assert x.dtype == torch.float32 and x.dim() == 2 and x.is_contiguous() and w.is_contiguous()
    m, k = x.shape
    n = w.shape[0]
    wd = -1 if w.dtype == torch.float32 else _dt(w)
    if b is not None:
        assert b.dtype == w.dtype
    y = torch.empty((m, n), dtype=torch.float32, device=x.device)
    _lib.check(_lib.lib().fino_skinny_linear(_p(x), _p(w), _p(b), _p(y), m, n, k, wd, int(silu_input), _stream()),
               "fino_skinny_linear")
    return y


def patchify(x, patch, out=None):
    assert x.dim() == 4 and x.is_contiguous()
    c, f, h, w = x.shape
    pt, ph, pw = patch
    L = (f // pt) * (h // ph) * (w // pw)
    if out is None:
        out = torch.empty((L, c * pt * ph * pw), dtype=x.dtype, device=x.device)
    _lib.check(_lib.lib().fino_patchify(_p(x), _p(out), c, f, h, w, pt, ph, pw, out.stride(0), _dt(x), _stream()),
               "fino_patchify")
    return out


# ... 458 lines not shown
```

### frameino_amd/transformer_wan.py

```python
import contextlib
import math
import os
from types import SimpleNamespace

import torch
from torch import nn

from . import ops
from .attention_processor import Attention, MI355WanAttnProcessor
from .loading import FromPretrainedMixin
from .lora import LoraModelMixin
from .mx_linears import MXLinearsMixin
from .step_cache import FirstBlockCacheMixin
from .window_attention import SelfAttentionOptionsMixin


class _Config(dict):
    __getattr__ = dict.__getitem__


class _FP32LayerNormParams(nn.Module):

    def __init__(self, dim, eps, elementwise_affine):
        super().__init__()
        self.eps = eps
        if elementwise_affine:
            self.weight = nn.Parameter(torch.ones(dim))
            self.bias = nn.Parameter(torch.zeros(dim))
        else:
            self.register_parameter("weight", None)
            self.register_parameter("bias", None)


class _GELUProj(nn.Module):
    def __init__(self, dim_in, dim_out):
        super().__init__()
        self.proj = nn.Linear(dim_in, dim_out)


class FeedForward(nn.Module):

    def __init__(self, dim, inner_dim):
        super().__init__()
        self.net = nn.ModuleList([_GELUProj(dim, inner_dim), nn.Dropout(0.0), nn.Linear(inner_dim, dim)])


class _MLP2(nn.Module):
    def __init__(self, d_in, d_hidden, d_out=None):
        super().__init__()
        self.linear_1 = nn.Linear(d_in, d_hidden)
        self.linear_2 = nn.Linear(d_hidden, d_out or d_hidden)


class WanTimeTextImageEmbedding(nn.Module):

    def __init__(self, dim, time_freq_dim, time_proj_dim, text_embed_dim):
        super().__init__()
        self.time_embedder = _MLP2(time_freq_dim, dim)
        self.time_proj = nn.Linear(dim, time_proj_dim)
        self.text_embedder = _MLP2(text_embed_dim, dim)


def wan_rope_tables(head_dim, max_seq_len, ppf, pph, ppw, theta=10000.0):
    h_dim = w_dim = 2 * (head_dim // 6)
    t_dim = head_dim - h_dim - w_dim

    def axis(dim):
        freqs = 1.0 / (theta ** (torch.arange(0, dim, 2, dtype=torch.float64)[: dim // 2] / dim))
        ang = torch.outer(torch.arange(max_seq_len, dtype=torch.float64), freqs)
        return ang.cos().float(), ang.sin().float()

    (ct, st), (ch, sh), (cw, sw) = axis(t_dim), axis(h_dim), axis(w_dim)

    def build(t, h, w):
        a = t[:ppf].view(ppf, 1, 1, -1).expand(ppf, pph, ppw, -1)
        b = h[:pph].view(1, pph, 1, -1).expand(ppf, pph, ppw, -1)
        c = w[:ppw].view(1, 1, ppw, -1).expand(ppf, pph, ppw, -1)
        return torch.cat([a, b, c], dim=-1).reshape(ppf * pph * ppw, -1).contiguous()

    return build(ct, ch, cw), build(st, sh, sw)


class WanTransformerBlock(nn.Module):
    def __init__(self, dim, ffn_dim, num_heads, qk_norm="rms_norm_across_heads", cross_attn_norm=False, eps=1e-6):
        super().__init__()
        self.attn1 = Attention(dim, heads=num_heads, dim_head=dim // num_heads, qk_norm=qk_norm, eps=eps, bias=True,
                               out_bias=True, processor=MI355WanAttnProcessor())
        self.attn2 = Attention(dim, heads=num_heads, dim_head=dim // num_heads, qk_norm=qk_norm, eps=eps, bias=True,
                               out_bias=True, processor=MI355WanAttnProcessor())
        self.norm2 = _FP32LayerNormParams(dim, eps, True) if cross_attn_norm else None
        self.ffn = FeedForward(dim, ffn_dim)
        self.scale_shift_table = nn.Parameter(torch.randn(1, 6, dim) / dim ** 0.5)


class WanTransformer3DModel(nn.Module, FromPretrainedMixin, LoraModelMixin, FirstBlockCacheMixin, MXLinearsMixin,
                            SelfAttentionOptionsMixin):
    _window_table_cache = "_rope_cache"
    _loader_name = "load_wan_transformer"
    _keep_in_fp32_modules = ["time_embedder", "scale_shift_table", "norm1", "norm2", "norm3"]
    _lora_wan_layout = True

    def __init__(self, patch_size=(1, 2, 2), num_attention_heads=40, attention_head_dim=128, in_channels=16,
                 out_channels=16, text_dim=4096, freq_dim=256, ffn_dim=13824, num_layers=40, cross_attn_norm=True,
                 qk_norm="rms_norm_across_heads", eps=1e-6, image_dim=None, added_kv_proj_dim=None,
                 rope_max_seq_len=1024, pos_embed_seq_len=None):
        super().__init__()
        if image_dim is not None or added_kv_proj_dim is not None:
            raise NotImplementedError("Wan2.1 image-embedding branch is outside FrameINO's TI2V-5B path")
        self.config = _Config(patch_size=tuple(patch_size), num_attention_heads=num_attention_heads,
                              attention_head_dim=attention_head_dim, in_channels=in_channels,
                              out_channels=out_channels or in_channels, text_dim=text_dim, freq_dim=freq_dim,
                              ffn_dim=ffn_dim, num_layers=num_layers, cross_attn_norm=cross_attn_norm, qk_norm=qk_norm,
                              eps=eps, image_dim=image_dim, added_kv_proj_dim=added_kv_proj_dim,
                              rope_max_seq_len=rope_max_seq_len, pos_embed_seq_len=pos_embed_seq_len)
        inner = num_attention_heads * attention_head_dim
        self.inner_dim = inner
        self.patch_embedding = nn.Conv3d(in_channels, inner, kernel_size=patch_size, stride=patch_size)
        self.condition_embedder = WanTimeTextImageEmbedding(inner, freq_dim, inner * 6, text_dim)
        self.blocks = nn.ModuleList([WanTransformerBlock(inner, ffn_dim, num_attention_heads, qk_norm, cross_attn_norm,
                                                         eps) for _ in range(num_layers)])
        self.proj_out = nn.Linear(inner, self.config.out_channels * math.prod(patch_size))
        self.scale_shift_table = nn.Parameter(torch.randn(1, 2, inner) / inner ** 0.5)
        self._packed = None
        self._rope_cache = {}
        self._text_cache = {}
        self._ws = {}
        self._ctx_name = None
        self.ops = ops
        self.parallel = None
        self.dedup_shared_prefix = True
        self.fold_softmax_scale = False
        self._init_self_attention_options()
        self.dedup_text_padding = os.environ.get("FINO_TEXT_FOLD", "1") != "0"
        self.reassociate_text_out = os.environ.get("FINO_TEXT_REASSOC", "1") != "0"
        self.skip_dead_rows = os.environ.get("FINO_SKIP_DEAD_ROWS", "1") != "0"

    @property
    def dtype(self):
        return self.proj_out.weight.dtype

    @property
    def device(self):
        return self.proj_out.weight.device

    @contextlib.contextmanager
    def cache_context(self, name):
        prev, self._ctx_name = self._ctx_name, name
        try:
            yield
        finally:
            self._ctx_name = prev

    @property
    def attn_processors(self):
        out = {}
        for i, blk in enumerate(self.blocks):
            out[f"blocks.{i}.attn1.processor"] = blk.attn1.processor
            out[f"blocks.{i}.attn2.processor"] = blk.attn2.processor
        return out

    def load_reference_state_dict(self, sd, dtype=None):
        own = self.state_dict()
        missing = [k for k in own if k not in sd]
        extra = [k for k in sd if k not in own]
        if missing or extra:
            raise KeyError(f"state-dict mismatch: missing {missing[:5]} unexpected {extra[:5]}")
        with torch.no_grad():
            for k, p in self.named_parameters():
                keep32 = any(s in k for s in self._keep_in_fp32_modules)
                t = sd[k].to(torch.float32 if keep32 else (dtype or sd[k].dtype))
                p.data = t.to(p.device).contiguous()
        self.reset_caches()
        return self

    def reset_caches(self):
        had_fp8 = self._mx_invalidate()
        self._reset_stateful_cache()
        self._packed = None
        self._text_cache.clear()
        self._rope_cache.clear()
        self._ws.clear()
        return had_fp8

    def _apply(self, fn, *args, **kwargs):
        out = super()._apply(fn, *args, **kwargs)
        if hasattr(self, "_text_cache"):
            self.reset_caches()
        return out

    def load_state_dict(self, *args, **kwargs):
        out = super().load_state_dict(*args, **kwargs)
        self.reset_caches()
        return out

    def _default_processors(self):
        return all(type(b.attn1.processor) is MI355WanAttnProcessor and type(b.attn2.processor) is MI355WanAttnProcessor
                   for b in self.blocks)

    def _pack(self):
        d = self.inner_dim
        pk = SimpleNamespace(layers=[])
        for blk in self.blocks:
            a1, a2 = blk.attn1, blk.attn2
            e = SimpleNamespace()
            e.wqkv = torch.cat([a1.to_q.weight, a1.to_k.weight, a1.to_v.weight]).detach().contiguous()
            e.bqkv = torch.cat([a1.to_q.bias, a1.to_k.bias, a1.to_v.bias]).detach().contiguous()
            e.wkv2 = torch.cat([a2.to_k.weight, a2.to_v.weight]).detach().contiguous()
            e.bkv2 = torch.cat([a2.to_k.bias, a2.to_v.bias]).detach().contiguous()
            pk.layers.append(e)
        pk.sst = torch.stack([b.scale_shift_table.detach().float()[0] for b in self.blocks])
        pk.w_patch = self.patch_embedding.weight.detach().reshape(d, -1).contiguous()
        self._packed = pk
        return pk

    def _mx_linear_weights(self, pk):
        for li, (blk, e) in enumerate(zip(self.blocks, pk.layers)):
            for key, w in (("qkv", e.wqkv), ("out", blk.attn1.to_out[0].weight), ("q2", blk.attn2.to_q.weight),
                           ("out2", blk.attn2.to_out[0].weight), ("ff1", blk.ffn.net[0].proj.weight),
                           ("ff2", blk.ffn.net[2].weight)):
                yield li, key, w

    def _window_refusals(self, fp8, default_procs, shard=None):
        what = "window attention (enable_window_attention)"
        if fp8:
            raise NotImplementedError(f"{what} with fp8 attention: the range walk exists in the bf16 / fp16 kernel only; switch "
                                      f"one of them off first (disable_window_attention() / enable_fp8_attention(False))")
        if self._pab_on:
            raise NotImplementedError(f"{what} with Pyramid Attention Broadcast: not implemented in this version (first-block "
                                      f"caching is)")
        if self._taylor_on:
            raise NotImplementedError(f"{what} with TaylorSeer caching: not implemented in this version (first-block caching is)")
        if shard is not None and getattr(shard, "active", True):
            raise NotImplementedError(f"{what} with a token-sharded plan: it runs on one GPU")
        if not default_procs:
            raise NotImplementedError(f"{what} with a user-installed attention processor: the windows are applied by the "
                                      f"built-in MI355WanAttnProcessor path only")

    def enable_cache(self, config):
        from .step_cache import _is_pab_config
        if self._sparse is not None and _is_pab_config(config):
            raise NotImplementedError("Pyramid Attention Broadcast with sparse attention (enable_sparse_attention): not "
                                      "implemented in this version (first-block caching is)")
        if self._window is not None and _is_pab_config(config):
            raise NotImplementedError("Pyramid Attention Broadcast with window attention (enable_window_attention): not "
                                      "implemented in this version (first-block caching is)")
        return super().enable_cache(config)

    def _taylorseer_refusals(self, config):
        what = "TaylorSeer caching (TaylorSeerCacheConfig)"
        if self._window is not None:
            raise NotImplementedError(f"{what} with window attention (enable_window_attention): not implemented in this version "
                                      f"(first-block caching is)")
        if self._sparse is not None:
            raise NotImplementedError(f"{what} with sparse attention (enable_sparse_attention): not implemented in this version "
                                      f"(first-block caching is)")
        if self.parallel is not None and getattr(self.parallel, "active", True):
            raise NotImplementedError(f"{what} with a token-sharded plan: it runs on one GPU")
        if not getattr(config, "use_lite_mode", False) and not self._default_processors():
            raise NotImplementedError(f"{what} with a user-installed attention processor: the attention branches are predicted on "
                                      f"the built-in MI355WanAttnProcessor path only (lite mode, `use_lite_mode=True`, predicts "
                                      f"the model's output and takes any processor)")

    def disable_cache(self):
        super().disable_cache()
        for ws in self._ws.values():
            ws.taylor_y = None

    def _workspace(self, L, dtype, device):
        key = (L, dtype, str(device), self._ctx_name)
        ws = self._ws.get(key)
        if ws is None:
            d, f = self.inner_dim, self.config.ffn_dim
            mk = lambda *s: torch.empty(*s, dtype=dtype, device=device)
            ws = SimpleNamespace(x=mk(L, d), n=mk(L, d), qkv=mk(L, 3 * d), att=mk(L, d), q2=mk(L, d), ff=mk(L, f),
                                 a=mk(L, self.config.in_channels * math.prod(self.config.patch_size)),
                                 po=mk(L, self.config.out_channels * math.prod(self.config.patch_size)))
            self._ws = {k: v for k, v in self._ws.items() if k[:3] == key[:3]}
            self._ws[key] = ws
        return ws

    def _rope(self, ppf, pph, ppw, device):
        key = (ppf, pph, ppw, str(device))
        if key not in self._rope_cache:
            cos, sin = wan_rope_tables(self.config.attention_head_dim, self.config.rope_max_seq_len, ppf, pph, ppw)
            self._rope_cache[key] = (cos.to(device), sin.to(device))
        return self._rope_cache[key]

# ... 298 lines not shown
        _keep_copy(c, a.reshape(c.nr, c.d))
        o.gated_residual(c.x, a.reshape(c.nr, c.d), m[:, 2], c.sel, out=c.x)
        return True

    def _sa_shared_prefix(self, c, li, blk, e, m):
        o, n, d, x, to_out = self.ops, c.n, c.d, c.x, blk.attn1.to_out[0]
        n1, q1, a1, sel1 = c.nrm[:n], c.qkv[:n], c.att[:n], _sel_rows(c.sel, 0, n)
        o.adaln_modulate(x[:n], m[:, 0], m[:, 1], sel1, c.eps, out=n1)
        self._lin(li, "qkv", n1, e.wqkv, e.bqkv, out=q1)
        self._qk_norm_rope(blk, q1, d, c.cos1, c.sin1, c.dh, c.qfold)
        q3 = q1.view(1, n, 3 * d)
        self._attend(o, q3[:, :, :d], q3[:, :, d:2 * d], q3[:, :, 2 * d:], c.heads, fp8=c.fp8,
                     ranges=self._window_ranges(c.win, li, (0, n)), tiles=self._sparse_tiles(c.sp, li, (0, n)),
                     out=a1.view(1, n, d), **c.afold)
        self._lin(li, "out", a1, to_out.weight, to_out.bias, o.EPI_GATED_RESIDUAL, residual=x[:n], gate=m[:, 2], sel=sel1,
                  out=x[:n])
        for bi in range(1, c.b):
            x[bi * n:(bi + 1) * n].copy_(x[:n])
        return True

    def _sa_single(self, c, li, blk, e, m):
        o, b, n, d = self.ops, c.b, c.n, c.d
        xq = self._ln_q(li, "qkv", 0, c.x, shift=m[:, 0], scale=m[:, 1], sel=c.sel, eps=c.eps)
        if xq is None:
            o.adaln_modulate(c.x, m[:, 0], m[:, 1], c.sel, c.eps, out=c.nrm)
        self._lin(li, "qkv", c.nrm, e.wqkv, e.bqkv, xq=xq, out=c.qkv)
        self._qk_norm_rope(blk, c.qkv, d, c.cos, c.sin, c.dh, c.qfold)
        q3 = c.qkv.view(b, n, 3 * d)
        s0, s1 = c.rows
        self._attend(o, q3[:, s0:s1, :d], q3[:, :, d:2 * d], q3[:, :, 2 * d:], c.heads, fp8=c.fp8,
                     ranges=self._window_ranges(c.win, li, (s0, s1)), tiles=self._sparse_tiles(c.sp, li, (s0, s1)),
                     out=c.att.view(b, n, d)[:, s0:s1], **c.afold)
        return False

    def _sa_heads_exchange(self, c, li, blk, e, m):
        o, sh, n, L, lpad, heads, dh, dt, dev = self.ops, c.sh, c.n, c.L, c.lpad, c.heads, c.dh, c.dt, c.dev
        ways = sh.ways
        hp = heads // ways
        self._lin(li, "qkv", c.nrm, e.wqkv, e.bqkv, out=c.qkv, **c.tk)
        lay = sh.heads_send_layout(heads, dh, lpad, dt, dev)
        self._qk_norm_rope(blk, c.qkv, c.d, c.cos, c.sin, dh, c.qfold, out=lay.flat, head_off=lay.off_qkv, head_ld=lay.ld)
        inflight = [(gi, h0, h1, (h1 - h0) * dh) + sh.all_to_all(f"qkv_recv{gi}", lay.views[gi], async_op=True)
                    for gi, (h0, h1) in enumerate(sh.head_ranges(hp))]
        orl = sh.heads_recv_layout(heads, dh, lpad, dt, dev) if not self._fp8 else None
        back = []
        for gi, h0, h1, dg, recv, work in inflight:
            if work is not None:
                work.wait()
            r3 = recv.view(1, ways * lpad, 3 * dg)[:, :L]
            oh = sh.a2a_buffer(f"o_send{gi}", (ways, lpad, dg), dt, dev)
            o.attention(r3[:, :, :dg], r3[:, :, dg:2 * dg], r3[:, :, 2 * dg:], h1 - h0,
                        out=oh.view(1, ways * lpad, dg)[:, :L], **c.afold)
            back.append((h0, h1) + sh.all_to_all(f"o_recv{gi}", oh, async_op=True))
        blocked = orl is not None and all(orv.data_ptr() == orl[gi].data_ptr() for gi, (_, _, orv, _) in enumerate(back))
        a3 = c.att.view(n, ways, hp * dh)
        for h0, h1, orv, work in back:
            if work is not None:
                work.wait()
            if not blocked:
                a3[:, :, h0 * dh:h1 * dh].copy_(orv[:, :n].permute(1, 0, 2))
        if blocked:
            to_out = blk.attn1.to_out[0]
            o.gemm_blocked_a(orl, n, to_out.weight, to_out.bias, c.x, m[:, 2], c.sel, out=c.x, **c.tk)
        return blocked

    def _project_kv(self, c, li, e, fused):
        kv_loc = c.sh.kv_local(c.lpad, 2 * c.d, c.dt, c.dev)
        if fused:
            self.ops.gemm(c.nrm, e.wqkv, e.bqkv, out=c.q2, out2=kv_loc[:c.n], split=c.d, **c.tk)
        else:
            self._lin(li, "kv", c.nrm, e.wqkv[c.d:], e.bqkv[c.d:], out=kv_loc[:c.n], **c.tk)
        return kv_loc

    def _project_q(self, c, li, blk, e, fused):
        if not fused:
            self._lin(li, "q", c.nrm, e.wqkv[:c.d], e.bqkv[:c.d], out=c.q2, **c.tk)
        self.ops.rmsnorm_rope_(c.q2, blk.attn1.norm_q.weight, blk.attn1.norm_q.eps, c.cos, c.sin, c.dh, **c.qfold)

    def _sa_kv_head_groups(self, c, li, blk, e):
        o, sh, n, d, dh, nk = self.ops, c.sh, c.n, c.d, c.dh, blk.attn1.norm_k
        fused = sh.fused_qkv_ok() and not self._fp8
        kv_loc = self._project_kv(c, li, e, fused)
        lay = sh.kv_group_layout(c.heads, dh, c.lpad, c.dt, c.dev)
        o.rmsnorm_rope_scatter(kv_loc[:n, :d], nk.weight, nk.eps, c.cos, c.sin, dh, lay.flat, lay.off_k, lay.ld)
        o.rmsnorm_rope_scatter(kv_loc[:n, d:], None, 0.0, None, None, dh, lay.flat, lay.off_v, lay.ld)
        flying = [sh._all_gather(f"kv_all_g{gi}", v_, True) for gi, v_ in enumerate(lay.views)]
        self._project_q(c, li, blk, e, fused)
        q3, a3 = c.q2.view(1, n, d), c.att.view(1, n, d)
        for (h0, h1), (kv_all, work) in zip(lay.ranges, flying):
            if work is not None:
                work.wait()
            dg = (h1 - h0) * dh
            kv3 = kv_all.view(1, -1, 2 * dg)[:, :c.L]
            o.attention(q3[:, :, h0 * dh:h1 * dh], kv3[:, :, :dg], kv3[:, :, dg:], h1 - h0, out=a3[:, :, h0 * dh:h1 * dh],
                        **c.afold)
        return False

    def _sa_kv_gather(self, c, li, blk, e):
        o, sh, n, d, dh, heads, lo, L, nk = self.ops, c.sh, c.n, c.d, c.dh, c.heads, c.lo, c.L, blk.attn1.norm_k
        fused = sh.fused_qkv_ok() and not self._fp8
        kv_loc = self._project_kv(c, li, e, fused)
        o.rmsnorm_rope_(kv_loc[:n, :d], nk.weight, nk.eps, c.cos, c.sin, dh)
        kv_all, work = sh.all_gather_kv(kv_loc)
        self._project_q(c, li, blk, e, fused)
        qv, av = c.q2.view(1, n, d), c.att.view(1, n, d)
        if not sh.local_first():
            if work is not None:
                work.wait()
            kv3 = kv_all.view(1, -1, 2 * d)[:, :L]
            o.attention(qv, kv3[:, :, :d], kv3[:, :, d:], heads, out=av, **c.afold)
            return False
        pf = o.attention_partial_floats(1, heads, n, dh) if hasattr(o, "attention_partial_floats") else 0
        parts = [o.attention_partial(qv, kv_loc[:n, :d][None], kv_loc[:n, d:][None], heads, out=sh.partial_buf(0, pf, c.dev),
                                     **c.afold)]
        if work is not None:
            work.wait()
        kv3 = kv_all.view(1, -1, 2 * d)
        for pi, (k0, k1) in enumerate(((0, lo), (lo + c.lpad, L))):
            if k1 > k0:
                parts.append(o.attention_partial(qv, kv3[:, k0:k1, :d], kv3[:, k0:k1, d:], heads,
                                                 out=sh.partial_buf(1 + pi, pf, c.dev), **c.afold))
        o.attention_merge(parts, 1, n, heads, dh, c.dt, out=av)
        return False

    def _self_attention_out(self, c, li, blk, m):
        to_out = blk.attn1.to_out[0]
        for r0, r1 in c.segs:
            self._lin(li, "out", c.att[r0:r1], to_out.weight, to_out.bias, self.ops.EPI_GATED_RESIDUAL, residual=c.x[r0:r1],
                      gate=m[:, 2], sel=_sel_rows(c.sel, r0, r1), out=c.x[r0:r1], **c.tk, **_keep_kw(c, r0, r1))

    def _cross_attention(self, c, li, blk):
        o, x, nrm, q2, att, segs, text = self.ops, c.x, c.nrm, c.q2, c.att, c.segs, c.text
        b, n, d, heads, n2, a2 = c.b, c.n, c.d, c.heads, blk.norm2, blk.attn2
        xq = self._ln_q(li, "q2", 1, x, weight=n2.weight, bias=n2.bias, eps=c.eps) if (n2 is not None
                                                                                       and c.default_procs) else None
        if xq is None and n2 is not None:
            for r0, r1 in segs:
                o.layernorm(x[r0:r1], n2.weight, n2.bias, c.eps, out=nrm[r0:r1])
        elif xq is None:
            nrm.copy_(x)
        if not c.default_procs:
            a = a2(nrm.view(b, n, d), encoder_hidden_states=text.txt.view(b, text.lt, d), **(c.attention_kwargs or {}))
            _keep_copy(c, a.reshape(c.nr, d))
            o.gated_residual(x, a.reshape(c.nr, d), out=x)
            return
        for r0, r1 in segs:
            self._lin(li, "q2", nrm[r0:r1], a2.to_q.weight, a2.to_q.bias, xq=xq, out=q2[r0:r1], **c.tk)
        kv = text.kv[li].view(b, text.lt, 2 * d)
        s0, s1 = c.rows
        if text.w2 is not None:
            rr = text.rrms
            for r0, r1 in segs:
                o.row_rrms(q2[r0:r1], a2.norm_q.eps, out=rr[r0:r1])
            for i in range(b):
                r0, r1 = i * n + s0, i * n + s1
                pr = o.attention_probs(q2[r0:r1].view(1, s1 - s0, d), kv[i:i + 1, :, :d], heads, text.tail[0][i:i + 1],
                                       text.tail[1][i:i + 1], text.kp[i], out=text.pbuf[i][:s1 - s0].view(1, s1 - s0, -1),
                                       q_rrms=rr[r0:r1].view(1, s1 - s0), q_weight=a2.norm_q.weight)
                xi = x[r0:r1]
                o.gemm(pr.view(s1 - s0, -1), text.w2[li][i], a2.to_out[0].bias, o.EPI_RESIDUAL, residual=xi, out=xi, **c.tk,
                       **_keep_kw(c, r0, r1))
            return
        for r0, r1 in segs:
            o.rmsnorm_rope_(q2[r0:r1], a2.norm_q.weight, a2.norm_q.eps)
        qv, av = q2.view(b, n, d)[:, s0:s1], att.view(b, n, d)[:, s0:s1]
        if text.tail is not None:
            o.attention_tail(qv, kv[:, :, :d], kv[:, :, d:], heads, text.tail[0], text.tail[1], out=av)
        else:
            o.attention(qv, kv[:, :, :d], kv[:, :, d:], heads, out=av)
        for r0, r1 in segs:
            self._lin(li, "out2", att[r0:r1], a2.to_out[0].weight, a2.to_out[0].bias, o.EPI_RESIDUAL, residual=x[r0:r1],
                      out=x[r0:r1], **c.tk, **_keep_kw(c, r0, r1))

    def _pab_attention(self, c, li, blk, e, m):
        pab, n = c.pab, c.n
        stages = (("self", lambda cc: self._self_attention(cc, li, blk, e, m) or self._self_attention_out(cc, li, blk, m)),
                  ("cross", lambda cc: self._cross_attention(cc, li, blk)))
        for kind, run in stages:
            if not pab.hooked[kind]:
                run(c)
                continue
            for i in range(c.b):
                seg = next(s_ for s_ in pab.segs if s_.r0 <= i * n < s_.r1)
                if not seg.compute[kind]:
                    (self._pab_reuse if pab.taylor is None else self._taylor_predict)(c, kind, seg, i, li, m)
                    continue
                cc = c if c.b == 1 else c.element(i)
                if pab.taylor is None:
                    y = self._pab_buffer(seg, kind, li, c.d, c.dt, c.dev)[i * n - seg.r0:(i + 1) * n - seg.r0]
                else:
                    y = self._taylor_scratch(c)
                cc.keep = {(0, n): y}
                try:
                    run(cc)
                finally:
                    cc.keep = None
                if pab.taylor is not None:
                    f = self._taylor_buffer(pab, seg, (kind, li), c.d, c.dev)[:, i * n - seg.r0:(i + 1) * n - seg.r0]
                    self.ops.taylor_update(y, f, seg.n_old, seg.k, seg.n_new)

    def _pab_reuse(self, c, kind, seg, i, li, m):
        o, r0, r1 = self.ops, i * c.n, (i + 1) * c.n
        y, x = self._pab_buffer(seg, kind, li)[r0 - seg.r0:r1 - seg.r0], c.x[r0:r1]
        gate, sel = (m[:, 2], _sel_rows(c.sel, r0, r1)) if kind == "self" else (None, None)
        (o.pab_broadcast if c.default_procs else o.gated_residual)(x, y, gate, sel, out=x)

    def _taylor_scratch(self, c):
        ws = c.ws
        if getattr(ws, "taylor_y", None) is None:
            ws.taylor_y = torch.empty((c.n, c.d), dtype=c.dt, device=c.dev)
        return ws.taylor_y

    def _taylor_predict(self, c, kind, seg, i, li, m):
        r0, r1 = i * c.n, (i + 1) * c.n
        f, x = self._taylor_buffer(c.pab, seg, (kind, li))[:, r0 - seg.r0:r1 - seg.r0], c.x[r0:r1]
        gate, sel = (m[:, 2], _sel_rows(c.sel, r0, r1)) if kind == "self" else (None, None)
        self.ops.taylor_predict(f, seg.n_old, seg.k, x, gate, sel, out=x)

    def _taylor_lite_rows(self, c, po):
        o, lite = self.ops, c.lite
        for seg in lite.segs:
            if seg.compute["self"]:
                o.taylor_update(po[seg.r0:seg.r1], self._taylor_buffer(lite, seg, "out", po.shape[1], c.dev), seg.n_old, seg.k,
                                seg.n_new)
            else:
                o.taylor_predict(self._taylor_buffer(lite, seg, "out"), seg.n_old, seg.k, out=po[seg.r0:seg.r1])
        return self._unpatchify(c, po)

    def _ffn(self, c, li, blk, m):
        o, x, nrm, ff, sel = self.ops, c.x, c.nrm, c.ff, c.sel
        up, down = blk.ffn.net[0].proj, blk.ffn.net[2]
        xq = self._ln_q(li, "ff1", 0, x, shift=m[:, 3], scale=m[:, 4], sel=sel, eps=c.eps) if (li, "ff2") in self._fp8 else None
        if xq is None:
            for r0, r1 in c.segs:
                o.adaln_modulate(x[r0:r1], m[:, 3], m[:, 4], _sel_rows(sel, r0, r1), c.eps, out=nrm[r0:r1])
        if self._ffn_mxfp8(li, nrm, xq, up.bias, down.bias, o.EPI_GATED_RESIDUAL, residual=x, gate=m[:, 5], sel=sel,
                           out=x) is None:
            for r0, r1 in c.segs:
                self._lin(li, "ff1", nrm[r0:r1], up.weight, up.bias, o.EPI_GELU_TANH, out=ff[r0:r1], **c.tk)
                self._lin(li, "ff2", ff[r0:r1], down.weight, down.bias, o.EPI_GATED_RESIDUAL, residual=x[r0:r1], gate=m[:, 5],
                          sel=_sel_rows(sel, r0, r1), out=x[r0:r1], **c.tk)

    def _output_head(self, c):
        o, nrm, sh = self.ops, c.nrm, c.sh
        for r0, r1 in c.segs:
            o.adaln_modulate(c.x[r0:r1], c.head[:, 0], c.head[:, 1], _sel_rows(c.sel, r0, r1), c.eps, out=nrm[r0:r1])
        if sh is None:
            po = c.ws.po[:c.nr]
            if c.live is not None:
                po.zero_()
            for r0, r1 in c.segs:
                o.gemm(nrm[r0:r1], self.proj_out.weight, self.proj_out.bias, out=po[r0:r1])
        else:
            po_loc = sh.out_local(c.lpad, c.ws.po.shape[1], c.dt, c.dev)
            o.gemm(nrm, self.proj_out.weight, self.proj_out.bias, out=po_loc[:c.n], **c.tk)
            po = sh.all_gather_out(po_loc)[:c.L]
        if c.lite is not None:
            return self._taylor_lite_rows(c, po)
        return self._unpatchify(c, po)

    def _unpatchify(self, c, po):
        o, cfg = self.ops, self.config
        unpatch = lambda rows: o.unpatchify(rows, cfg.out_channels, c.nf, c.hh, c.ww, cfg.patch_size)
        if c.b == 1:
            return unpatch(po)[None]
        po3 = po.view(c.b, c.L, -1)
        return torch.stack([unpatch(po3[i]) for i in range(c.b)])


class _Call:
    __slots__ = ("b", "n", "nr", "lo", "lpad", "L", "nf", "hh", "ww", "d", "heads", "dh", "dev", "dt", "eps", "sh", "tk", "pk",
                 "ws", "x", "nrm", "att", "q2", "ff", "qkv", "cos", "sin", "cos1", "sin1", "sel", "mod", "head", "text", "qfold",
                 "afold", "fp8", "default_procs", "shared", "fbc", "pab", "keep", "h0", "h1c", "attention_kwargs", "live",
                 "live_segs", "rows", "segs", "win", "sp", "lite", "elements")

    def __init__(self, **fields):
        self.elements = None
        for k, v in fields.items():
            setattr(self, k, v)

    def element(self, i):
        if self.elements is None:
            self.elements = {}
        if i in self.elements:
            return self.elements[i]
        r0, r1 = i * self.n, (i + 1) * self.n
        f = {k: getattr(self, k) for k in self.__slots__ if k != "elements"}
        for k in ("x", "nrm", "att", "q2", "ff", "qkv"):
            f[k] = f[k][r0:r1]
        f.update(b=1, nr=self.n, cos=self.cos1, sin=self.sin1, sel=_sel_rows(self.sel, r0, r1), segs=[(0, self.n)],
                 text=_text_element(self.text, i, self.b, self.n, self.d), keep=None)
        self.elements[i] = _Call(**f)
        return self.elements[i]


def _sel_rows(sel, r0, r1):
    return None if sel is None else sel[r0:r1]


def _keep_kw(c, r0, r1):
    return {} if c.keep is None else {"keep": c.keep[(r0, r1)]}


def _keep_copy(c, y):
    if c.keep is not None:
        for (r0, r1), buf in c.keep.items():
# ... 15 lines not shown
```

### include/frameino_hip.h

```cpp
#ifndef FRAMEINO_HIP_H
#define FRAMEINO_HIP_H
#include <stdint.h>

#ifdef __cplusplus
extern "C" {
#endif

#define FINO_VERSION 103

enum { FINO_BF16 = 0, FINO_F16 = 1, FINO_F32 = 2 };
enum {
    FINO_OK = 0,
    FINO_ERR_ARG = -1,
    FINO_ERR_LAUNCH = -2,
    FINO_ERR_UNSUPPORTED = -3
};

int fino_version(void);
const char* fino_last_error(void);

enum { FINO_TUNE_GEMM_GROUP_M = 0, FINO_TUNE_GEMM_RASTER = 1, FINO_TUNE_CONV_LOOP = 2, FINO_TUNE_GEMM_TILE_M = 3,
       FINO_TUNE_ATTN_KERNEL = 4, FINO_TUNE_ATTN_FP8_KERNEL = 5, FINO_TUNE_ATTN_WALK_GRID = 6, FINO_TUNE_COUNT = 8 };
int fino_tune_set(int key, int value);
int fino_tune_get(int key);

int fino_adaln_modulate(const void* x, void* y, int64_t rows, int dim, int64_t ldx, int64_t ldy,
                        const float* shift, const float* scale, int64_t mod_stride, const int32_t* sel,
                        float eps, int dtype, void* stream);

int fino_layernorm(const void* x, void* y, int64_t rows, int dim, int64_t ldx, int64_t ldy, const float* w,
                   const float* b, float eps, int dtype, void* stream);

int fino_gated_residual(const void* x, const void* y, void* out, int64_t rows, int dim, int64_t ldx, int64_t ldy,
                        int64_t ldo, const float* gate, int64_t mod_stride, const int32_t* sel, int dtype,
                        void* stream);

int fino_gated_residual_staged(const void* x, const void* y, void* out, int64_t rows, int dim, int64_t ldx, int64_t ldy,
                               int64_t ldo, const float* gate, int64_t mod_stride, const int32_t* sel, int dtype,
                               void* stream);

int fino_layernorm_zero(const void* x, void* y, int64_t rows, int dim, int64_t ldx, int64_t ldy, const float* w,
                        const float* b, const float* shift, const float* scale, int64_t mod_stride, const int32_t* sel,
                        float eps, int dtype, void* stream);

int fino_ln_mxfp8(int mode, const void* x, void* q, void* scales, int64_t rows, int dim, int64_t ldx, const float* w,
                  const float* b, const float* shift, const float* scale, int64_t mod_stride, const int32_t* sel,
                  float eps, int dtype, void* stream);

int fino_rmsnorm_rope(void* x, int64_t rows, int dim, int64_t ldx, const void* weight, float eps,
                      const float* cos_t, const float* sin_t, int head_dim, int dtype, void* stream);
int fino_rmsnorm_rope_scaled(void* x, int64_t rows, int dim, int64_t ldx, const void* weight, float eps,
                             const float* cos_t, const float* sin_t, int head_dim, float out_scale, int dtype,
                             void* stream);

int fino_rmsnorm_rope_scatter(const void* x, int64_t rows, int dim, int64_t ldx, const void* weight, float eps,
                              const float* cos_t, const float* sin_t, int head_dim, float out_scale, void* out,
                              const int64_t* head_off, const int64_t* head_ld, int dtype, void* stream);

int fino_qkv_rmsnorm_rope(void* qkv, int64_t rows, int dim, int64_t ldx, const void* q_weight, float q_eps,
                          const void* k_weight, float k_eps, const float* cos_t, const float* sin_t, int head_dim,
                          float q_out_scale, void* out, const int64_t* head_off, const int64_t* head_ld, int dtype,
                          void* stream);

int fino_headnorm_rope(void* x, int batch, int64_t rows, int heads, int head_dim, int64_t ldx, int64_t batch_stride,
                       const void* w, const void* b, float eps, const float* cos_t, const float* sin_t,
                       int64_t rope_row0, int dtype, void* stream);
int fino_headnorm_rope_scaled(void* x, int batch, int64_t rows, int heads, int head_dim, int64_t ldx,
                              int64_t batch_stride, const void* w, const void* b, float eps, const float* cos_t,
                              const float* sin_t, int64_t rope_row0, float out_scale, int dtype, void* stream);

#define FINO_ATTN_SCALE_FOLDED (-1.0f)
int fino_attn_fwd(const void* q, const void* k, const void* v, void* o, int batch, int heads, int64_t lq,
                  int64_t lk, int head_dim, int64_t q_bs, int64_t q_rs, int64_t q_hs, int64_t k_bs, int64_t k_rs,
                  int64_t k_hs, int64_t v_bs, int64_t v_rs, int64_t v_hs, int64_t o_bs, int64_t o_rs,
                  int64_t o_hs, float scale, int dtype, void* stream);
enum { FINO_FP8_P_EXP2 = 0, FINO_FP8_P_RAMP = 1 };
int64_t fino_attn_fp8_kv_bytes(int batch, int heads, int64_t lk, int head_dim);
int fino_attn_fwd_fp8(const void* q, const void* k, const void* v, void* o, int batch, int heads, int64_t lq, int64_t lk,
                      int head_dim, int64_t q_bs, int64_t q_rs, int64_t k_bs, int64_t k_rs, int64_t v_bs, int64_t v_rs,
                      int64_t o_bs, int64_t o_rs, float scale, int dtype, int p_mode, void* kv_workspace,
                      int64_t kv_workspace_bytes, void* stream);
int64_t fino_attn_fp8_smooth_kv_bytes(int batch, int heads, int64_t lk, int head_dim);
int fino_attn_fwd_fp8_smooth(const void* q, const void* k, const void* v, void* o, int batch, int heads, int64_t lq, int64_t lk,
                             int head_dim, int64_t q_bs, int64_t q_rs, int64_t k_bs, int64_t k_rs, int64_t v_bs, int64_t v_rs,
                             int64_t o_bs, int64_t o_rs, float scale, int dtype, int p_mode, void* kv_workspace,
                             int64_t kv_workspace_bytes, void* stream);
#define FINO_FP8_SMOOTH_K 1
#define FINO_FP8_SMOOTH_V 2
int64_t fino_attn_fp8_smoothed_kv_bytes(int batch, int heads, int64_t lk, int head_dim, int smooth);
int fino_attn_fwd_fp8_smoothed(const void* q, const void* k, const void* v, void* o, int batch, int heads, int64_t lq, int64_t lk,
                               int head_dim, int64_t q_bs, int64_t q_rs, int64_t k_bs, int64_t k_rs, int64_t v_bs, int64_t v_rs,
                               int64_t o_bs, int64_t o_rs, float scale, int dtype, int p_mode, void* kv_workspace,
                               int64_t kv_workspace_bytes, void* stream, int smooth);

int fino_attn_tail_supported(int batch, int heads, int64_t lq, int64_t lk, int head_dim);
int fino_attn_fwd_tail(const void* q, const void* k, const void* v, void* o, int batch, int heads, int64_t lq, int64_t lk,
                       int head_dim, int64_t q_bs, int64_t q_rs, int64_t q_hs, int64_t k_bs, int64_t k_rs, int64_t k_hs,
                       int64_t v_bs, int64_t v_rs, int64_t v_hs, int64_t o_bs, int64_t o_rs, int64_t o_hs, float scale,
                       int dtype, const int* lk_b, const float* tail_mult, void* stream);

int fino_attn_ranges_supported(int batch, int heads, int64_t lq, int64_t lk, int head_dim);
int fino_attn_fwd_ranges(const void* q, const void* k, const void* v, void* o, int batch, int heads, int64_t lq, int64_t lk,
                         int head_dim, int64_t q_bs, int64_t q_rs, int64_t q_hs, int64_t k_bs, int64_t k_rs, int64_t k_hs,
                         int64_t v_bs, int64_t v_rs, int64_t v_hs, int64_t o_bs, int64_t o_rs, int64_t o_hs, float scale,
                         int dtype, const int* ranges, void* stream);
int fino_attn_tiles_supported(int batch, int heads, int64_t lq, int64_t lk, int head_dim);
int fino_attn_fwd_tiles(const void* q, const void* k, const void* v, void* o, int batch, int heads, int64_t lq, int64_t lk,
                        int head_dim, int64_t q_bs, int64_t q_rs, int64_t q_hs, int64_t k_bs, int64_t k_rs, int64_t k_hs,
                        int64_t v_bs, int64_t v_rs, int64_t v_hs, int64_t o_bs, int64_t o_rs, int64_t o_hs, float scale,
                        int dtype, const uint32_t* mask, int64_t mask_bs, int64_t mask_hs, int words, void* stream);
int64_t fino_attn_tile_plan_bytes(int batch, int heads, int64_t lq, int64_t lk, int head_dim);
int fino_attn_tile_plan(const void* q, const void* k, int batch, int heads, int64_t lq, int64_t lk, int head_dim, int64_t q_bs,
                        int64_t q_rs, int64_t q_hs, int64_t k_bs, int64_t k_rs, int64_t k_hs, float scale, int dtype, float cdf,
                        const int* keep_ranges, uint32_t* mask, int words, void* workspace, int64_t workspace_bytes,
                        void* stream);
int64_t fino_attn_tile_plan_gated_bytes(int batch, int heads, int64_t lq, int64_t lk, int head_dim);
int fino_attn_tile_plan_gated(const void* q, const void* k, int batch, int heads, int64_t lq, int64_t lk, int head_dim,
                              int64_t q_bs, int64_t q_rs, int64_t q_hs, int64_t k_bs, int64_t k_rs, int64_t k_hs, float scale,
                              int dtype, float cdf, const float* cdf_heads, float sim_threshold, const int* keep_ranges,
                              uint32_t* mask, int words, void* workspace, int64_t workspace_bytes, void* stream);
int fino_attn_fp8_ranges_supported(int batch, int heads, int64_t lq, int64_t lk, int head_dim);
int fino_attn_fwd_fp8_ranges(const void* q, const void* k, const void* v, void* o, int batch, int heads, int64_t lq, int64_t lk,
                             int head_dim, int64_t q_bs, int64_t q_rs, int64_t k_bs, int64_t k_rs, int64_t v_bs, int64_t v_rs,
                             int64_t o_bs, int64_t o_rs, float scale, int dtype, int p_mode, void* kv_workspace,
                             int64_t kv_workspace_bytes, int smooth_k, const int* ranges, void* stream);
int fino_attn_fp8_tiles_supported(int batch, int heads, int64_t lq, int64_t lk, int head_dim);
int fino_attn_fwd_fp8_tiles(const void* q, const void* k, const void* v, void* o, int batch, int heads, int64_t lq, int64_t lk,
                            int head_dim, int64_t q_bs, int64_t q_rs, int64_t k_bs, int64_t k_rs, int64_t v_bs, int64_t v_rs,
                            int64_t o_bs, int64_t o_rs, float scale, int dtype, int p_mode, void* kv_workspace,
                            int64_t kv_workspace_bytes, int smooth, const uint32_t* mask, int64_t mask_bs, int64_t mask_hs,
                            int words, void* stream);

int fino_attn_probs_supported(int batch, int heads, int64_t lq, int64_t lk, int head_dim);
int fino_attn_probs(const void* q, const void* k, void* p, int batch, int heads, int64_t lq, int64_t lk, int head_dim,
                    int64_t q_bs, int64_t q_rs, int64_t q_hs, int64_t k_bs, int64_t k_rs, int64_t k_hs, int kp, int64_t p_bs,
                    int64_t p_rs, float scale, int dtype, const int* lk_b, const float* tail_mult, const float* q_rrms,
                    int64_t q_rrms_bs, const void* q_weight, void* stream);
int fino_row_rrms(const void* x, int64_t rows, int dim, int64_t ldx, float eps, float* rrms, int dtype, void* stream);

int64_t fino_attn_partial_bytes(int batch, int heads, int64_t lq, int head_dim);
int fino_attn_partial(const void* q, const void* k, const void* v, int batch, int heads, int64_t lq, int64_t lk,
                      int head_dim, int64_t q_bs, int64_t q_rs, int64_t q_hs, int64_t k_bs, int64_t k_rs, int64_t k_hs,
                      int64_t v_bs, int64_t v_rs, int64_t v_hs, float scale, int dtype, void* partial,
                      int64_t partial_bytes, void* stream);
int fino_attn_merge(void* o, int batch, int heads, int64_t lq, int head_dim, int64_t o_bs, int64_t o_rs, int64_t o_hs,
                    const void* part0, const void* part1, const void* part2, int dtype, void* stream);


int64_t fino_attn_workspace_bytes(int batch, int heads, int64_t lq, int64_t lk, int head_dim);
int fino_attn_fwd_ws(const void* q, const void* k, const void* v, void* o, int batch, int heads, int64_t lq,
                     int64_t lk, int head_dim, int64_t q_bs, int64_t q_rs, int64_t q_hs, int64_t k_bs, int64_t k_rs,
                     int64_t k_hs, int64_t v_bs, int64_t v_rs, int64_t v_hs, int64_t o_bs, int64_t o_rs, int64_t o_hs,
                     float scale, int dtype, void* workspace, int64_t workspace_bytes, void* stream);

enum { FINO_EPI_NONE = 0, FINO_EPI_GELU_TANH = 1, FINO_EPI_RESIDUAL = 2, FINO_EPI_GATED_RESIDUAL = 3,
       FINO_EPI_GATED_RESIDUAL_STAGED = 4, FINO_EPI_F32 = 5, FINO_EPI_F32_RESIDUAL = 6 };
int fino_gemm(const void* a, const void* w, const void* bias, void* c, int64_t m, int64_t n, int64_t k,
              int64_t lda, int64_t ldw, int64_t ldc, int epilogue, const void* r, int64_t ldr, const float* gate,
              int64_t mod_stride, const int32_t* sel, int dtype, void* stream);
int fino_gemm_split_n(const void* a, const void* w, const void* bias, void* c, int64_t m, int64_t n, int64_t k, int64_t lda,
                      int64_t ldw, int64_t ldc, int epilogue, const void* r, int64_t ldr, const float* gate,
                      int64_t mod_stride, const int32_t* sel, int dtype, void* c2, int64_t ldc2, int64_t n_split,
                      int tile_m, void* stream);
int fino_gemm_keep(const void* a, const void* w, const void* bias, void* c, int64_t m, int64_t n, int64_t k, int64_t lda,
                   int64_t ldw, int64_t ldc, int epilogue, const void* r, int64_t ldr, const float* gate,
                   int64_t mod_stride, const int32_t* sel, int dtype, void* keep, int64_t ldk, int tile_m, void* stream);
int fino_gemm_blocked_a(const void* a, const void* w, const void* bias, void* c, int64_t m, int64_t n, int64_t k,
                        int64_t a_block_k, int64_t a_block_stride, int a_groups, int64_t a_group_stride, int64_t lda,
                        int64_t ldw, int64_t ldc, const void* r, int64_t ldr, const float* gate, int64_t mod_stride,
                        const int32_t* sel, int dtype, int tile_m, void* stream);

int fino_gemm_plan(int64_t m, int64_t n, int64_t* rows_256, int* tile_rows_rest);
int fino_skinny_linear(const float* x, const void* w, const void* b, float* y, int m, int64_t n, int64_t k,
                       int w_dtype, int silu_input, void* stream);

int fino_patchify(const void* x, void* a, int channels, int frames, int height, int width, int pt, int ph, int pw,
                  int64_t lda, int dtype, void* stream);
int fino_unpatchify(const void* y, void* out, int cout, int frames, int height, int width, int pt, int ph, int pw,
                    int64_t ldy, int dtype, void* stream);

int fino_wan_model_input(const float* lat, const float* cond, const float* id_lat, const float* traj, void* out,
                         int channels, int gen_frames, int id_frames, int height, int width, int dtype, void* stream);
int fino_cfg_euler_step(const void* cond_pred, const void* uncond_pred, float* lat, int channels, int gen_frames,
                        int total_frames, int height, int width, float guidance, const float* dt_dev, int round_out,
                        int dtype, void* stream);

int fino_cfg_unipc_step(const void* cond_pred, const void* uncond_pred, float* x, float* last, float* m0, float* m1,
                        int channels, int gen_frames, int total_frames, int height, int width, const float* coef_dev,
                        int dtype, void* stream);

int fino_cfg_vpred_step(const void* pred, void* lat, int64_t n_lat, int64_t batch_stride, const float* coef_dev,
                        int has_uncond, int dtype, void* stream);

int fino_cfg_dpm_step(const void* pred, void* lat, float* x0_old, const void* noise, int64_t n_lat, int64_t batch_stride,
                      const float* coef_dev, int has_uncond, int dtype, void* stream);

int fino_conv3d(const void* x, const void* w, const void* bias, void* y, int t_in, int h_in, int w_in, int c_in_pad,
                int t_out, int h_out, int w_out, int c_out_pad, int kt, int kh, int kw, int st, int sh, int sw, int pt,
                int ph, int pw, int upsample2x, int epilogue, const void* r, const void* zero_page, int dtype,
                void* stream);
int fino_rmsnorm_silu_cl(const void* x, void* y, int64_t rows, int c_valid, int c_pad, const float* gamma, int silu,
                         int dtype, void* stream);
int fino_softmax_rows(void* s, int64_t rows, int n, int64_t ld, float scale, int dtype, void* stream);
int fino_dup_up3d_add(const void* main_in, const void* x, void* out, int t_in, int h_in, int w_in, int c_in,
                      int c_in_pad, int c_out, int c_out_pad, int factor_t, int factor_s, int dtype, void* stream);
int fino_avg_down3d_add(const void* main_in, const void* x, void* out, int t_in, int h_in, int w_in, int c_in,
                        int c_in_pad, int c_out, int c_out_pad, int factor_t, int factor_s, int dtype, void* stream);
int fino_vae_unpatchify_clamp(const void* y, float* out, int t, int h, int w, int c_pad, int channels, int patch,
                              int dtype, void* stream);
int fino_vae_patchify(const float* x, void* y, int t, int h, int w, int c_pad, int channels, int patch, int dtype,
                      void* stream);
int fino_split_bf16(const float* x, void* out, int64_t rows, int cols, int64_t ldx, int64_t ldo, int nseg,
                    unsigned planes_packed, void* stream);
int fino_rmsnorm_silu_cl_f32(const float* x, void* y, int64_t rows, int c_valid, int c_pad, const float* gamma, int silu,
                             int nseg, unsigned planes_packed, void* stream);
int fino_conv3d_split(const void* x_planes, const void* w_products, const float* bias, float* y, int t_in, int h_in, int w_in,
                      int c_in_pad, int planes, int t_out, int h_out, int w_out, int c_out_pad, int kt, int kh, int kw, int st,
                      int sh, int sw, int pt, int ph, int pw, int upsample2x, int epilogue, const float* r,
                      const void* zero_page, void* stream);

int64_t fino_mxfp8_scale_bytes(int64_t rows, int64_t cols);
int fino_quantize_mxfp8(const void* x, void* q, void* scales, int64_t rows, int64_t cols, int64_t ldx, int dtype,
                        void* stream);
int fino_gemm_mxfp8(const void* aq, const void* a_scales, const void* wq, const void* w_scales, const void* bias,
                    void* c, int64_t m, int64_t n, int64_t k, int64_t ldc, int epilogue, const void* r, int64_t ldr,
                    const float* gate, int64_t mod_stride, const int32_t* sel, int out_dtype, void* stream);
int fino_gemm_mxfp8_keep(const void* aq, const void* a_scales, const void* wq, const void* w_scales, const void* bias,
                         void* c, int64_t m, int64_t n, int64_t k, int64_t ldc, int epilogue, const void* r, int64_t ldr,
                         const float* gate, int64_t mod_stride, const int32_t* sel, int out_dtype, void* keep, int64_t ldk,
                         void* stream);
int fino_gemm_mxfp8_q(const void* aq, const void* a_scales, const void* wq, const void* w_scales, const void* bias,
                      void* cq, void* c_scales, int64_t m, int64_t n, int64_t k, int epilogue, int bias_dtype,
                      void* stream);

#define FINO_MX_ROT_ACT 1
#define FINO_MX_ROT_WEIGHT 2
int64_t fino_mxfp6_bytes(int64_t rows, int64_t cols);
int64_t fino_mxfp6_scale_bytes(int64_t rows, int64_t cols);
int fino_quantize_mxfp6(const void* x, void* q, void* scales, int64_t rows, int64_t cols, int64_t ldx, int dtype,
                        void* stream);
int fino_quantize_mxfp6_rot(const void* x, void* q, void* scales, int64_t rows, int64_t cols, int64_t ldx, int dtype,
                            int mode, void* stream);
int fino_gemm_mxfp6(const void* aq, const void* a_scales, const void* wq, const void* w_scales, const void* bias,
                    void* c, int64_t m, int64_t n, int64_t k, int64_t ldc, int epilogue, const void* r, int64_t ldr,
                    const float* gate, int64_t mod_stride, const int32_t* sel, int out_dtype, void* stream);
int fino_gemm_mxfp6_keep(const void* aq, const void* a_scales, const void* wq, const void* w_scales, const void* bias,
                         void* c, int64_t m, int64_t n, int64_t k, int64_t ldc, int epilogue, const void* r, int64_t ldr,
                         const float* gate, int64_t mod_stride, const int32_t* sel, int out_dtype, void* keep, int64_t ldk,
                         void* stream);

int fino_traj_paint(const int32_t* points, const int32_t* frame_offsets, float* canvas, int frames, int height, int width,
                    int radius, void* stream);
int fino_traj_blur_quantize(const float* canvas, float* scratch, float* out, const float* taps_dev, int taps, int planes,
                            int height, int width, void* stream);


int64_t fino_groupnorm_workspace_bytes(int c_pad);
int fino_groupnorm_cl(const void* x, void* y, int t, int h, int w, int channels, int c_pad, int groups,
                      const float* gamma, const float* beta, float eps, const void* mod_scale, const void* mod_shift,
                      int tz, int hz, int wz, int silu, void* workspace, int64_t workspace_bytes, int dtype,
                      void* stream);
int fino_avg_pool_time2(const void* x, void* y, int t_in, int h, int w, int c_pad, int dtype, void* stream);
int fino_vae_blend_tiles(const void* a, void* b, int t, int h_a, int w_a, int h_b, int w_b, int c_pad, int extent, int axis,
                         int dtype, void* stream);

int fino_resize_area_pad_u8(const void* src, void* dst, int src_h, int src_w, int region_h, int region_w, int out_h,
                            int out_w, int off_y, int off_x, int fill, void* stream);
int fino_u8_hwc_to_chw_unit(const void* src, float* dst, int height, int width, void* stream);

enum { FINO_LORA_MAX_ADAPTERS = 8, FINO_LORA_MAX_TOTAL_RANK = 1024 };
int fino_lora_merge(const void* w_base, int64_t ldw_base, void* w_out, int64_t ldw_out, int64_t n, int64_t k,
                    int n_adapters, const void* const* a, const int64_t* lda, const void* const* b, const int64_t* ldb,
                    const int* rank, const float* scale, int dtype, void* stream);

typedef struct {
    const void* h0;
    const void* h1;
    const void* p;
    void* r;
    void* h1_copy;
    int64_t rows, ld_h0, ld_h1, ld_p, ld_r, ld_h1_copy;
} FinoStepCacheSegment;
enum { FINO_STEP_CACHE_MAX_SEGMENTS = 4, FINO_STEP_CACHE_BLOCKS = 1024,
       FINO_STEP_CACHE_WORKSPACE_FLOATS = 2 * FINO_STEP_CACHE_MAX_SEGMENTS * FINO_STEP_CACHE_BLOCKS };
int fino_step_cache_probe(const FinoStepCacheSegment* segs, int nseg, int64_t dim, float* sums, float* workspace, int dtype,
                          void* stream);
int fino_step_cache_residual(const void* a, int64_t lda, const void* b, int64_t ldb, void* out, int64_t ldo, int64_t rows,
                             int64_t dim, int subtract, int dtype, void* stream);
int fino_pab_broadcast(const void* x, int64_t ldx, const void* y, int64_t ldy, void* out, int64_t ldo, int64_t rows,
                       int64_t dim, const float* gate, int64_t mod_stride, const int32_t* sel, int dtype, void* stream);
enum { FINO_TAYLOR_MAX_PLANES = 4 };
int fino_taylor_update(const void* y, int64_t ldy, void* factors, int64_t plane_stride, int64_t ldf, int64_t rows, int64_t dim,
                       int n_old, int n_new, int delta, int dtype, int fdtype, void* stream);
int fino_taylor_predict(const void* factors, int64_t plane_stride, int64_t ldf, int n, const float* coef, const void* x,
                        int64_t ldx, void* out, int64_t ldo, int64_t rows, int64_t dim, const float* gate, int64_t mod_stride,
                        const int32_t* sel, int dtype, int fdtype, void* stream);

int fino_diag_mfma_peak(int kind, int waves_per_simd, int iters, void* scratch, double* flops, void* stream);

#ifdef __cplusplus
}
#endif
#endif
```

Before: 3.731 denoise-steps/s.

## Batch text cross-attention tail into one probs launch and paired short-K GEMM

Adds a per-sample variant of the cross-attention probability kernel so cond and uncond samples write into separate buffers with different key widths in a single launch. Adds a new short-K 128x128 GEMM kernel that runs two independent GEMMs (one per sample) in one grid. The text cross-attention tail now uses both, replacing the per-sample loop of probs plus GEMM launches. This removes launch overhead and fills the GPU better on these small GEMMs, at the cost of a new kernel path whose tiling may not match the tuned default GEMM.

```diff
diff --git a/frameino_amd/_lib.py b/frameino_amd/_lib.py
--- a/frameino_amd/_lib.py
+++ b/frameino_amd/_lib.py
@@ -60,6 +60,9 @@
     "fino_attn_probs": [c_void_p] * 3 + [c_int, c_int, c_i64, c_i64, c_int] + [c_i64] * 6 + [c_int, c_i64, c_i64, c_float, c_int,
                                                                                          c_void_p, c_void_p, c_void_p, c_i64,
                                                                                          c_void_p, c_void_p],
+    "fino_attn_probs_per_sample": [c_void_p] * 5 + [c_int, c_int, c_i64, c_i64, c_int] + [c_i64] * 6 + [c_float, c_int, c_void_p,
+                                                                                                    c_void_p, c_void_p, c_i64,
+                                                                                                    c_void_p, c_void_p],
     "fino_row_rrms": [c_void_p, c_i64, c_int, c_i64, c_float, c_void_p, c_int, c_void_p],
     "fino_attn_fp8_kv_bytes": [c_int, c_int, c_i64, c_int],
     "fino_attn_fwd_fp8": [c_void_p] * 4 + [c_int, c_int, c_i64, c_i64, c_int] + [c_i64] * 8 + [c_float, c_int, c_int, c_void_p,
@@ -105,6 +108,7 @@
                           c_i64, c_i64, c_int, c_void_p],
     "fino_gemm_keep": [c_void_p] * 4 + [c_i64] * 6 + [c_int, c_void_p, c_i64, c_void_p, c_i64, c_void_p, c_int, c_void_p,
                        c_i64, c_int, c_void_p],
+    "fino_gemm_pair": ([c_void_p] * 5 + [c_i64] * 6) * 2 + [c_void_p, c_i64, c_int, c_void_p, c_i64, c_int, c_void_p],
     "fino_ln_mxfp8": [c_int, c_void_p, c_void_p, c_void_p, c_i64, c_int, c_i64, c_void_p, c_void_p, c_void_p, c_void_p, c_i64,
                       c_void_p, c_float, c_int, c_void_p],
     "fino_gemm_blocked_a": [c_void_p, c_void_p, c_void_p, c_void_p, c_i64, c_i64, c_i64, c_i64, c_i64, c_int, c_i64, c_i64, c_i64,
diff --git a/frameino_amd/csrc/fino_attention_probs.hip b/frameino_amd/csrc/fino_attention_probs.hip
--- a/frameino_amd/csrc/fino_attention_probs.hip
+++ b/frameino_amd/csrc/fino_attention_probs.hip
@@ -8,10 +8,11 @@
 struct ProbsParams {
     const uint16_t* q;
     const uint16_t* k;
-    uint16_t* p;
     int batch, heads, lq, lk;
-    int64_t q_bs, q_rs, q_hs, k_bs, k_rs, k_hs, p_bs, p_rs;
-    int kp;
+    int64_t q_bs, q_rs, q_hs, k_bs, k_rs, k_hs;
+    uint16_t* p_b[4];
+    int64_t p_rs_b[4];
+    int kp_b[4];
     const float* q_rrms;
     const uint16_t* q_weight;
     int64_t q_rrms_bs;
@@ -35,6 +36,7 @@
 
     const int lkc = p.lk_b[bi < 4 ? bi : 3];
     const float lm = p.log2_mult[bi < 4 ? bi : 3];
+    const int kp = p.kp_b[bi < 4 ? bi : 3];
     const int nkb = (lkc + 31) >> 5;
     const uint16_t* kp_ = p.k + bi * p.k_bs + head * p.k_hs;
     for (int i = 0; i < nkb * 2; ++i) {
@@ -123,7 +125,7 @@
 #pragma unroll
         for (int g4 = 0; g4 < 4; ++g4) {
             const int key0 = kb * 32 + 8 * g4 + 4 * h;
-            if (key0 < p.kp) {
+            if (key0 < kp) {
                 const uint32_t w0 = (uint32_t)T::from_f32(acc[kb][4 * g4 + 0] * inv) | ((uint32_t)T::from_f32(acc[kb][4 * g4 + 1] * inv) << 16);
                 const uint32_t w1 = (uint32_t)T::from_f32(acc[kb][4 * g4 + 2] * inv) | ((uint32_t)T::from_f32(acc[kb][4 * g4 + 3] * inv) << 16);
                 *reinterpret_cast<uint2*>(stage + r * 256 + ((((key0 >> 3)) ^ (r & 15)) << 4) + ((key0 & 4) << 1)) = make_uint2(w0, w1);
@@ -131,14 +133,15 @@
         }
     }
     __syncthreads();
-    const int pieces = p.kp >> 3;
+    const int pieces = kp >> 3;
     const int total = 32 * pieces;
     const int row_base = blockIdx.x * 128 + wave * 32;
-    uint16_t* pbase = p.p + bi * p.p_bs + head * p.kp;
+    uint16_t* pbase = p.p_b[bi < 4 ? bi : 3] + head * kp;
+    const int64_t p_rs = p.p_rs_b[bi < 4 ? bi : 3];
     for (int i = lane; i < total; i += 64) {
         const int rr = i / pieces, pc = i - rr * pieces;
         const uint4 u = *reinterpret_cast<const uint4*>(stage + rr * 256 + ((pc ^ (rr & 15)) << 4));
-        if (row_base + rr < p.lq) *reinterpret_cast<uint4*>(pbase + (int64_t)(row_base + rr) * p.p_rs + pc * 8) = u;
+        if (row_base + rr < p.lq) *reinterpret_cast<uint4*>(pbase + (int64_t)(row_base + rr) * p_rs + pc * 8) = u;
     }
 }
 
@@ -149,45 +152,47 @@
            (int64_t)batch * heads <= 65535;
 }
 
-extern "C" int fino_attn_probs(const void* q, const void* k, void* p, int batch, int heads, int64_t lq, int64_t lk,
-                               int head_dim, int64_t q_bs, int64_t q_rs, int64_t q_hs, int64_t k_bs, int64_t k_rs, int64_t k_hs,
-                               int kp, int64_t p_bs, int64_t p_rs, float scale, int dtype, const int* lk_b,
-                               const float* tail_mult, const float* q_rrms, int64_t q_rrms_bs, const void* q_weight,
-                               void* stream) {
+static int attn_probs_impl(const void* q, const void* k, void* const* p_b, const int* kp_b, const int64_t* p_rs_b, int batch,
+                           int heads, int64_t lq, int64_t lk, int head_dim, int64_t q_bs, int64_t q_rs, int64_t q_hs, int64_t k_bs,
+                           int64_t k_rs, int64_t k_hs, float scale, int dtype, const int* lk_b, const float* tail_mult,
+                           const float* q_rrms, int64_t q_rrms_bs, const void* q_weight, void* stream) {
     FINO_CHECK((q_rrms == nullptr) == (q_weight == nullptr) && fino_aligned16(q_weight), FINO_ERR_ARG,
                "fino_attn_probs: q_rrms and q_weight come together (q_weight 16-byte aligned)");
     FINO_CHECK(dtype == FINO_BF16 || dtype == FINO_F16, FINO_ERR_ARG, "fino_attn_probs: dtype %d", dtype);
-    FINO_CHECK(q && k && p && lk_b && tail_mult, FINO_ERR_ARG, "fino_attn_probs: null pointer");
+    FINO_CHECK(q && k && p_b && kp_b && p_rs_b && lk_b && tail_mult, FINO_ERR_ARG, "fino_attn_probs: null pointer");
     FINO_CHECK(fino_attn_probs_supported(batch, heads, lq, lk, head_dim), FINO_ERR_UNSUPPORTED,
                "fino_attn_probs: needs head_dim 128, batch <= 4, lk <= 128 (got head_dim %d, batch %d, lk %lld)", head_dim, batch,
                (long long)lk);
-    FINO_CHECK(fino_aligned16(q) && fino_aligned16(k) && fino_aligned16(p) && q_rs % 8 == 0 && k_rs % 8 == 0 && q_hs % 8 == 0 &&
-                   k_hs % 8 == 0 && q_bs % 8 == 0 && k_bs % 8 == 0 && p_bs % 8 == 0 && p_rs % 8 == 0,
+    FINO_CHECK(fino_aligned16(q) && fino_aligned16(k) && q_rs % 8 == 0 && k_rs % 8 == 0 && q_hs % 8 == 0 && k_hs % 8 == 0 &&
+                   q_bs % 8 == 0 && k_bs % 8 == 0,
                FINO_ERR_ARG, "fino_attn_probs: pointers and strides must be 16-byte aligned");
-    FINO_CHECK(kp > 0 && kp % 8 == 0 && kp <= 128 && p_rs >= (int64_t)heads * kp, FINO_ERR_ARG,
-               "fino_attn_probs: kp %d (a multiple of 8, <= 128), row stride %lld", kp, (long long)p_rs);
+    for (int b = 0; b < batch; ++b) {
+        FINO_CHECK(p_b[b] && fino_aligned16(p_b[b]) && p_rs_b[b] % 8 == 0, FINO_ERR_ARG,
+                   "fino_attn_probs: pointers and strides must be 16-byte aligned (output of sample %d)", b);
+        FINO_CHECK(kp_b[b] > 0 && kp_b[b] % 8 == 0 && kp_b[b] <= 128 && p_rs_b[b] >= (int64_t)heads * kp_b[b], FINO_ERR_ARG,
+                   "fino_attn_probs: kp %d (a multiple of 8, <= 128), row stride %lld", kp_b[b], (long long)p_rs_b[b]);
+    }
     FINO_CHECK(scale > 0.f || scale == FINO_ATTN_SCALE_FOLDED, FINO_ERR_ARG, "fino_attn_probs: scale");
     if (lq == 0) return FINO_OK;
     ProbsParams pp;
-    pp.q = (const uint16_t*)q; pp.k = (const uint16_t*)k; pp.p = (uint16_t*)p;
+    pp.q = (const uint16_t*)q; pp.k = (const uint16_t*)k;
     pp.batch = batch; pp.heads = heads; pp.lq = (int)lq; pp.lk = (int)lk;
-    pp.q_bs = q_bs; pp.q_rs = q_rs; pp.q_hs = q_hs; pp.k_bs = k_bs; pp.k_rs = k_rs; pp.k_hs = k_hs; pp.p_bs = p_bs; pp.p_rs = p_rs;
-    pp.kp = kp;
+    pp.q_bs = q_bs; pp.q_rs = q_rs; pp.q_hs = q_hs; pp.k_bs = k_bs; pp.k_rs = k_rs; pp.k_hs = k_hs;
     pp.q_rrms = q_rrms; pp.q_weight = (const uint16_t*)q_weight; pp.q_rrms_bs = q_rrms_bs;
     pp.scale_log2 = scale == FINO_ATTN_SCALE_FOLDED ? 1.0f : scale * 1.4426950408889634f;
     for (int b = 0; b < 4; ++b) {
         const int bb = b < batch ? b : batch - 1;
-        FINO_CHECK(lk_b[bb] >= 1 && lk_b[bb] <= lk && lk_b[bb] <= kp && tail_mult[bb] >= 1.0f, FINO_ERR_ARG,
-                   "fino_attn_probs: lk_b[%d] = %d (of %lld, kp %d), tail_mult %g", bb, lk_b[bb], (long long)lk, kp,
+        FINO_CHECK(lk_b[bb] >= 1 && lk_b[bb] <= lk && lk_b[bb] <= kp_b[bb] && tail_mult[bb] >= 1.0f, FINO_ERR_ARG,
+                   "fino_attn_probs: lk_b[%d] = %d (of %lld, kp %d), tail_mult %g", bb, lk_b[bb], (long long)lk, kp_b[bb],
                    (double)tail_mult[bb]);
+        pp.p_b[b] = (uint16_t*)p_b[bb]; pp.p_rs_b[b] = p_rs_b[bb]; pp.kp_b[b] = kp_b[bb];
         pp.lk_b[b] = lk_b[bb];
         pp.log2_mult[b] = log2f(tail_mult[bb]);
     }
     hipStream_t st = (hipStream_t)stream;
     const dim3 grid((unsigned)((lq + 127) / 128), (unsigned)(batch * heads));
-    int max_lk = 0;
-    for (int b = 0; b < batch; ++b) max_lk = lk_b[b] > max_lk ? lk_b[b] : max_lk;
-    const int need = max_lk > kp ? max_lk : kp;
+    int need = 0;
+    for (int b = 0; b < batch; ++b) need = kp_b[b] > need ? kp_b[b] : need;
     const int nkb = need <= 64 ? 2 : (need <= 96 ? 3 : 4);
 #define PROBS_LAUNCH(T_)                                                                                      \
     {                                                                                                         \
@@ -200,3 +205,28 @@
     FINO_LAUNCH_CHECK();
     return FINO_OK;
 }
+
+extern "C" int fino_attn_probs(const void* q, const void* k, void* p, int batch, int heads, int64_t lq, int64_t lk,
+                               int head_dim, int64_t q_bs, int64_t q_rs, int64_t q_hs, int64_t k_bs, int64_t k_rs, int64_t k_hs,
+                               int kp, int64_t p_bs, int64_t p_rs, float scale, int dtype, const int* lk_b,
+                               const float* tail_mult, const float* q_rrms, int64_t q_rrms_bs, const void* q_weight,
+                               void* stream) {
+    FINO_CHECK(p && p_bs % 8 == 0, FINO_ERR_ARG, "fino_attn_probs: null pointer or a batch stride that is not 16-byte aligned");
+    FINO_CHECK(batch >= 1 && batch <= 4, FINO_ERR_UNSUPPORTED, "fino_attn_probs: batch %d (1 .. 4)", batch);
+    void* p_b[4];
+    int kp_b[4];
+    int64_t p_rs_b[4];
+    for (int b = 0; b < 4; ++b) { p_b[b] = (uint16_t*)p + b * p_bs; kp_b[b] = kp; p_rs_b[b] = p_rs; }
+    return attn_probs_impl(q, k, p_b, kp_b, p_rs_b, batch, heads, lq, lk, head_dim, q_bs, q_rs, q_hs, k_bs, k_rs, k_hs, scale, dtype,
+                           lk_b, tail_mult, q_rrms, q_rrms_bs, q_weight, stream);
+}
+
+extern "C" int fino_attn_probs_per_sample(const void* q, const void* k, void* const* p_b, const int* kp_b, const int64_t* p_rs_b,
+                                          int batch, int heads, int64_t lq, int64_t lk, int head_dim, int64_t q_bs, int64_t q_rs,
+                                          int64_t q_hs, int64_t k_bs, int64_t k_rs, int64_t k_hs, float scale, int dtype,
+                                          const int* lk_b, const float* tail_mult, const float* q_rrms, int64_t q_rrms_bs,
+                                          const void* q_weight, void* stream) {
+    FINO_CHECK(batch >= 1 && batch <= 4, FINO_ERR_UNSUPPORTED, "fino_attn_probs: batch %d (1 .. 4)", batch);
+    return attn_probs_impl(q, k, p_b, kp_b, p_rs_b, batch, heads, lq, lk, head_dim, q_bs, q_rs, q_hs, k_bs, k_rs, k_hs, scale, dtype,
+                           lk_b, tail_mult, q_rrms, q_rrms_bs, q_weight, stream);
+}
diff --git a/frameino_amd/csrc/fino_gemm.hip b/frameino_amd/csrc/fino_gemm.hip
--- a/frameino_amd/csrc/fino_gemm.hip
+++ b/frameino_amd/csrc/fino_gemm.hip
@@ -694,8 +694,278 @@
     }
 }
 
+constexpr int kSkBM = 128, kSkBN = 128, kSkThreads = 256;
+constexpr int kSkTileBytes = kSkBM * BK * 2;
+constexpr int kSkStageBytes = 2 * kSkTileBytes;
+constexpr int kSkCsStride = kSkBN * 2 + 16;
+constexpr int kSkSmemBytes = 2 * kSkStageBytes;
+constexpr int kSkMaxK = 2048;
+static_assert(kSkBM * kSkCsStride <= kSkSmemBytes, "the staged epilogue tile lives in the operand stages");
+
+struct SkParams {
+    const uint16_t* a;
+    const uint16_t* w;
+    const uint16_t* bias;
+    uint16_t* c;
+    const uint16_t* r;
+    const float* gate;
+    const int32_t* sel;
+    uint16_t* c2;
+    int64_t m, n, lda, ldw, ldc, ldr, ldc2, mod_stride;
+    int a_bytes, w_bytes;
+    int nk, tiles_m, tiles_n, group_m;
+};
+
+template <typename T, int EPI, bool KEEP>
+__global__ __launch_bounds__(kSkThreads, 2) void gemm_sk_kernel(const SkParams p0, const SkParams p1, const int tiles0) {
+    extern __shared__ __attribute__((aligned(16))) char smem[];
+    typedef typename T::vec8 vec8;
+    constexpr bool kHasRes = EPI == FINO_EPI_RESIDUAL || EPI == FINO_EPI_GATED_RESIDUAL;
+    constexpr bool kGated = EPI == FINO_EPI_GATED_RESIDUAL;
+    constexpr int kIters = (kSkBM * kSkBN / 8) / kSkThreads;
+    static_assert(kIters == 8, "the counted wait below leaves kIters residual loads in flight");
+    const int tid = threadIdx.x;
+    const int lane = tid & 63;
+    const int wave = __builtin_amdgcn_readfirstlane(tid >> 6);
+    const int wm = wave >> 1, wn = wave & 1;
+    const bool second = (int)blockIdx.x >= tiles0;
+    const SkParams& p = second ? p1 : p0;
+    int tm, tn;
+    {
+        const int id = xcd_remap((int)blockIdx.x - (second ? tiles0 : 0), p.tiles_m * p.tiles_n);
+        const int group = id / (p.group_m * p.tiles_n);
+        const int first_m = group * p.group_m;
+        const int gsz = (p.tiles_m - first_m) < p.group_m ? (p.tiles_m - first_m) : p.group_m;
+        const int in_group = id - group * p.group_m * p.tiles_n;
+        tm = first_m + in_group % gsz;
+        tn = in_group / gsz;
+    }
+    const int64_t m0 = (int64_t)tm * kSkBM, n0 = (int64_t)tn * kSkBN;
+    const int nk = p.nk;
+
+    float bv[4][4];
+#pragma unroll
+    for (int j = 0; j < 4; ++j) {
+        int64_t gn = n0 + wn * 64 + j * 16 + (lane >> 4) * 4;
+        gn = gn + 4 <= p.n ? gn : p.n - 4;
+        uint2 b4 = make_uint2(0, 0);
+        if (p.bias) b4 = *reinterpret_cast<const uint2*>(p.bias + gn);
+        bv[j][0] = T::to_f32((uint16_t)(b4.x & 0xffffu)); bv[j][1] = T::to_f32((uint16_t)(b4.x >> 16));
+        bv[j][2] = T::to_f32((uint16_t)(b4.y & 0xffffu)); bv[j][3] = T::to_f32((uint16_t)(b4.y >> 16));
+    }
+
+    const int r8 = lane >> 3;
+    const int sk = ((lane & 7) ^ ((4 * (wave & 1) + (lane >> 4)) & 7)) * 8;
+    const __amdgpu_buffer_rsrc_t a_rsrc = __builtin_amdgcn_make_buffer_rsrc((void*)p.a, 0, p.a_bytes, 0x00020000);
+    const __amdgpu_buffer_rsrc_t w_rsrc = __builtin_amdgcn_make_buffer_rsrc((void*)p.w, 0, p.w_bytes, 0x00020000);
+    uint32_t a_off[4], w_off[4];
+#pragma unroll
+    for (int q = 0; q < 4; ++q) {
+        int64_t gm = m0 + q * 32 + wave * 8 + r8, gn = n0 + q * 32 + wave * 8 + r8;
+        gm = gm < p.m ? gm : p.m - 1;
+        gn = gn < p.n ? gn : p.n - 1;
+        a_off[q] = (uint32_t)((gm * p.lda + sk) * 2);
+        w_off[q] = (uint32_t)((gn * p.ldw + sk) * 2);
+    }
+#define SK_DMA(STAGE_, KT_)                                                                                        \
+    _Pragma("unroll") for (int q_ = 0; q_ < 4; ++q_) {                                                             \
+        __builtin_amdgcn_raw_ptr_buffer_load_lds(                                                                  \
+            a_rsrc, (FINO_LDS void*)(smem + (STAGE_) * kSkStageBytes + (q_ * 32 + wave * 8) * 128), 16, a_off[q_], \
+            (KT_) * (BK * 2), 0, 0);                                                                               \
+        __builtin_amdgcn_raw_ptr_buffer_load_lds(                                                                  \
+            w_rsrc, (FINO_LDS void*)(smem + (STAGE_) * kSkStageBytes + kSkTileBytes + (q_ * 32 + wave * 8) * 128), \
+            16, w_off[q_], (KT_) * (BK * 2), 0, 0);                                                                \
+    }
+    uint4 rres[kHasRes ? kIters : 1];
+    auto load_residual = [&]() {
+#pragma unroll
+        for (int it = 0; it < kIters; ++it) {
+            const int idx = it * kSkThreads + tid;
+            int64_t gm = m0 + (idx >> 4), gn = n0 + (idx & 15) * 8;
+            gm = gm < p.m ? gm : p.m - 1;
+            gn = gn < p.n ? gn : p.n - 8;
+            rres[kHasRes ? it : 0] = *reinterpret_cast<const uint4*>(p.r + gm * p.ldr + gn);
+        }
+    };
+
+    const int frow = lane & 15;
+    const int pch0 = (lane >> 4) ^ (frow >> 1);
+    const int a_base = (wm * 64 + frow) * 128;
+    const int w_base = kSkTileBytes + (wn * 64 + frow) * 128;
+    f32x4_t acc[4][4];
+#pragma unroll
+    for (int i = 0; i < 4; ++i)
+#pragma unroll
+        for (int j = 0; j < 4; ++j) acc[i][j] = f32x4_t{0.f, 0.f, 0.f, 0.f};
+
+    __builtin_amdgcn_sched_barrier(0);
+    SK_DMA(0, 0)
+    __builtin_amdgcn_sched_barrier(0);
+    if (kHasRes && nk == 1) load_residual();
+    for (int kt = 0; kt < nk; ++kt) {
+        const int cur = kt & 1;
+        const char* sb = smem + cur * kSkStageBytes;
+        __builtin_amdgcn_sched_barrier(0);
+        if (kHasRes && kt + 1 == nk) asm volatile("s_waitcnt vmcnt(8) lgkmcnt(0)" ::: "memory");
+        else asm volatile("s_waitcnt vmcnt(0) lgkmcnt(0)" ::: "memory");
+        __builtin_amdgcn_s_barrier();
+        __builtin_amdgcn_sched_barrier(0);
+        u32x4_t af[2][4], wf[2][4];
+#pragma unroll
+        for (int kk = 0; kk < 2; ++kk) {
+            const int pch = (pch0 ^ (kk << 2)) << 4;
+#pragma unroll
+            for (int j = 0; j < 4; ++j) wf[kk][j] = *reinterpret_cast<const u32x4_t*>(sb + w_base + j * 2048 + pch);
+#pragma unroll
+            for (int i = 0; i < 4; ++i) af[kk][i] = *reinterpret_cast<const u32x4_t*>(sb + a_base + i * 2048 + pch);
+        }
+        __builtin_amdgcn_sched_barrier(0);
+        if (kt + 1 < nk) {
+            SK_DMA(cur ^ 1, kt + 1)
+            __builtin_amdgcn_sched_barrier(0);
+            if (kHasRes && kt + 2 == nk) load_residual();
+        }
+        __builtin_amdgcn_sched_barrier(0);
+#pragma unroll
+        for (int kk = 0; kk < 2; ++kk) {
+#pragma unroll
+            for (int i = 0; i < 4; ++i) {
+#pragma unroll
+                for (int jj = 0; jj < 4; ++jj) {
+                    const int j = ((i + 4 * kk) & 1) ? 3 - jj : jj;
+                    acc[i][j] = T::mfma16(__builtin_bit_cast(vec8, wf[kk][j]), __builtin_bit_cast(vec8, af[kk][i]), acc[i][j]);
+                }
+            }
+        }
+    }
+#undef SK_DMA
+    __builtin_amdgcn_sched_barrier(0);
+    asm volatile("s_waitcnt lgkmcnt(0)" ::: "memory");
+    __builtin_amdgcn_s_barrier();
+    __builtin_amdgcn_sched_barrier(0);
+
+#pragma unroll
+    for (int i = 0; i < 4; ++i) {
+        const int row = wm * 64 + i * 16 + (lane & 15);
+#pragma unroll
+        for (int j = 0; j < 4; ++j) {
+            float y[4];
+#pragma unroll
+            for (int e = 0; e < 4; ++e) y[e] = acc[i][j][e] + bv[j][e];
+            const uint32_t w0 = (uint32_t)T::from_f32(y[0]) | ((uint32_t)T::from_f32(y[1]) << 16);
+            const uint32_t w1 = (uint32_t)T::from_f32(y[2]) | ((uint32_t)T::from_f32(y[3]) << 16);
+            const int col = wn * 64 + j * 16 + (lane >> 4) * 4;
+            *reinterpret_cast<uint2*>(smem + row * kSkCsStride + col * 2) = make_uint2(w0, w1);
+        }
+    }
+    __builtin_amdgcn_sched_barrier(0);
+    asm volatile("s_waitcnt lgkmcnt(0)" ::: "memory");
+    __builtin_amdgcn_s_barrier();
+    __builtin_amdgcn_sched_barrier(0);
+    int rsel[kGated ? kIters : 1];
+    if (kGated) {
+#pragma unroll
+        for (int it = 0; it < kIters; ++it) {
+            int64_t gm = m0 + ((it * kSkThreads + tid) >> 4);
+            gm = gm < p.m ? gm : p.m - 1;
+            rsel[kGated ? it : 0] = p.sel ? p.sel[gm] : 0;
+        }
+    }
+    int gsel = -1;
+    float gg[8] = {0.f, 0.f, 0.f, 0.f, 0.f, 0.f, 0.f, 0.f};
+#pragma unroll
+    for (int it = 0; it < kIters; ++it) {
+        const int idx = it * kSkThreads + tid;
+        const int row = idx >> 4;
+        const int ch = idx & 15;
+        const int64_t gm = m0 + row, gn = n0 + ch * 8;
+        if (gm >= p.m || gn >= p.n) continue;
+        uint4 yv = *reinterpret_cast<const uint4*>(smem + row * kSkCsStride + ch * 16);
+        if constexpr (KEEP) *reinterpret_cast<uint4*>(p.c2 + gm * p.ldc2 + gn) = yv;
+        if (kHasRes) {
+            float y[8], rv[8], o[8];
+            unpack8<T>(yv, y);
+            unpack8<T>(rres[kHasRes ? it : 0], rv);
+            if (kGated) {
+                if (rsel[kGated ? it : 0] != gsel) {
+                    gsel = rsel[kGated ? it : 0];
+                    const float* g = p.gate + (int64_t)gsel * p.mod_stride + gn;
+                    const float4 g0 = *reinterpret_cast<const float4*>(g);
+                    const float4 g1 = *reinterpret_cast<const float4*>(g + 4);
+                    gg[0] = g0.x; gg[1] = g0.y; gg[2] = g0.z; gg[3] = g0.w;
+                    gg[4] = g1.x; gg[5] = g1.y; gg[6] = g1.z; gg[7] = g1.w;
+                }
+#pragma unroll
+                for (int e = 0; e < 8; ++e) o[e] = rv[e] + y[e] * gg[e];
+            } else {
+#pragma unroll
+                for (int e = 0; e < 8; ++e) o[e] = rv[e] + y[e];
+            }
+            yv = pack8<T>(o);
+        }
+        *reinterpret_cast<uint4*>(p.c + gm * p.ldc + gn) = yv;
+    }
+}
+
+inline SkParams sk_params(const GemmParams& g) {
+    SkParams s = {};
+    s.a = g.a; s.w = g.w; s.bias = g.bias; s.c = g.c; s.r = g.r; s.gate = g.gate; s.sel = g.sel; s.c2 = g.c2;
+    s.m = g.m; s.n = g.n; s.lda = g.lda; s.ldw = g.ldw; s.ldc = g.ldc; s.ldr = g.ldr; s.ldc2 = g.ldc2; s.mod_stride = g.mod_stride;
+    s.a_bytes = (int)(((g.m - 1) * g.lda + g.k) * 2);
+    s.w_bytes = (int)(((g.n - 1) * g.ldw + g.k) * 2);
+    s.nk = (int)(g.k / BK);
+    s.tiles_m = (int)((g.m + kSkBM - 1) / kSkBM);
+    s.tiles_n = (int)((g.n + kSkBN - 1) / kSkBN);
+    const int gm = fino_tune_get(FINO_TUNE_GEMM_GROUP_M);
+    s.group_m = gm > 0 ? gm : 8;
+    return s;
+}
+
+inline bool sk_legal(const GemmParams& p, int epi) {
+    return p.k % BK == 0 && p.k <= kSkMaxK && p.m > 0 &&
+           (epi == FINO_EPI_NONE || epi == FINO_EPI_RESIDUAL || epi == FINO_EPI_GATED_RESIDUAL) && p.n_split == 0 &&
+           p.a_tpb == 0 && (reinterpret_cast<uintptr_t>(p.bias) & 7) == 0 && ((p.m - 1) * p.lda + p.k) * 2 < (1ll << 31) && ((p.n - 1) * p.ldw + p.k) * 2 < (1ll << 31) &&
+           ((p.m + kSkBM - 1) / kSkBM) * ((p.n + kSkBN - 1) / kSkBN) < (1ll << 30);
+}
+#ifndef GP_SK_DEFAULT_MAX_K
+#define GP_SK_DEFAULT_MAX_K 512
+#endif
+inline bool sk_wanted(const GemmParams& p, int epi, int tile_m) {
+    const int knob = fino_tune_get(FINO_TUNE_GEMM_SHORT_K);
+    if (knob == 1 || !sk_legal(p, epi)) return false;
+    if (knob == 2) return true;
+    if (tile_m != 0 || fino_tune_get(FINO_TUNE_GEMM_TILE_M) != 0 || !use_pingpong()) return false;
+    const int64_t tiles = ((p.m + kSkBM - 1) / kSkBM) * ((p.n + kSkBN - 1) / kSkBN);
+    return p.k <= GP_SK_DEFAULT_MAX_K && tiles >= 2 * (int64_t)gemm_device_cus();
+}
+
+template <typename T, int EPI, bool KEEP>
+int launch_gemm_sk_t(const SkParams& s0, const SkParams& s1, int tiles0, int tiles, hipStream_t st) {
+    static FinoPerDeviceOnce once;
+    if (int rc = fino_max_smem_once(once, reinterpret_cast<const void*>(&gemm_sk_kernel<T, EPI, KEEP>), kSkSmemBytes, "fino_gemm")) return rc;
+    gemm_sk_kernel<T, EPI, KEEP><<<dim3((unsigned)tiles), kSkThreads, kSkSmemBytes, st>>>(s0, s1, tiles0);
+    FINO_LAUNCH_CHECK();
+    return FINO_OK;
+}
+
+template <typename T, bool KEEP = false>
+int launch_gemm_sk(const GemmParams& p0, const GemmParams* p1, int epi, hipStream_t st) {
+    const SkParams s0 = sk_params(p0), s1 = p1 ? sk_params(*p1) : s0;
+    const int tiles0 = s0.tiles_m * s0.tiles_n, tiles = tiles0 + (p1 ? s1.tiles_m * s1.tiles_n : 0);
+    if constexpr (KEEP) {
+        return epi == FINO_EPI_RESIDUAL ? launch_gemm_sk_t<T, FINO_EPI_RESIDUAL, true>(s0, s1, tiles0, tiles, st)
+                                        : launch_gemm_sk_t<T, FINO_EPI_GATED_RESIDUAL, true>(s0, s1, tiles0, tiles, st);
+    }
+    switch (epi) {
+        case FINO_EPI_NONE: return launch_gemm_sk_t<T, FINO_EPI_NONE, false>(s0, s1, tiles0, tiles, st);
+        case FINO_EPI_RESIDUAL: return launch_gemm_sk_t<T, FINO_EPI_RESIDUAL, false>(s0, s1, tiles0, tiles, st);
+        default: return launch_gemm_sk_t<T, FINO_EPI_GATED_RESIDUAL, false>(s0, s1, tiles0, tiles, st);
+    }
+}
+
 template <typename T, bool GENERIC, bool KEEP = false>
 int launch_gemm_e(const GemmParams& p, int epi, int tile_m, hipStream_t st) {
+    if (!GENERIC && sk_wanted(p, epi, tile_m)) return launch_gemm_sk<T, KEEP>(p, nullptr, epi, st);
     const bool fits32 = ((p.m - 1) * p.lda + p.k) * 2 < (1ll << 31) && ((p.n - 1) * p.ldw + p.k) * 2 < (1ll << 31);
     if (epi == FINO_EPI_F32 || epi == FINO_EPI_F32_RESIDUAL) {
         if (GENERIC || !fits32) {
@@ -738,17 +1008,28 @@
     float acc[16];
 #pragma unroll
     for (int i = 0; i < 16; ++i) acc[i] = 0.f;
-    for (int64_t kk = lane; kk < k; kk += 64) {
-        float wv;
-        if (WT == -1) wv = ((const float*)w)[col * k + kk];
-        else if (WT == FINO_BF16) wv = BF16::to_f32(((const uint16_t*)w)[col * k + kk]);
-        else wv = F16::to_f32(((const uint16_t*)w)[col * k + kk]);
-#pragma unroll
-        for (int i = 0; i < 16; ++i) {
-            if (i < m) {
-                float xv = x[(int64_t)i * k + kk];
-                if (silu_input) xv = xv / (1.0f + __expf(-xv));
-                acc[i] += xv * wv;
+    constexpr int kDepth = 8;
+    for (int64_t k0 = lane; k0 < k; k0 += 64 * kDepth) {
+        float wv[kDepth];
+#pragma unroll
+        for (int u = 0; u < kDepth; ++u) {
+            const int64_t kk = k0 + 64 * u;
+            const int64_t kc = kk < k ? kk : k0;
+            if (WT == -1) wv[u] = ((const float*)w)[col * k + kc];
+            else if (WT == FINO_BF16) wv[u] = BF16::to_f32(((const uint16_t*)w)[col * k + kc]);
+            else wv[u] = F16::to_f32(((const uint16_t*)w)[col * k + kc]);
+        }
+#pragma unroll
+        for (int u = 0; u < kDepth; ++u) {
+            const int64_t kk = k0 + 64 * u;
+            if (kk >= k) break;
+#pragma unroll
+            for (int i = 0; i < 16; ++i) {
+                if (i < m) {
+                    float xv = x[(int64_t)i * k + kk];
+                    if (silu_input) xv = xv / (1.0f + __expf(-xv));
+                    acc[i] += xv * wv[u];
+                }
             }
         }
     }
@@ -784,10 +1065,10 @@
                              0, 0, 0, stream);
 }
 
-static int gemm_impl(const void* a, const void* w, const void* bias, void* c, int64_t m, int64_t n, int64_t k, int64_t lda,
-                     int64_t ldw, int64_t ldc, int epilogue, const void* r, int64_t ldr, const float* gate,
-                     int64_t mod_stride, const int32_t* sel, int dtype, void* c2, int64_t ldc2, int64_t n_split, void* keep,
-                     int64_t ldk, int tile_m, void* stream) {
+static int gemm_prepare(GemmParams& p, const void* a, const void* w, const void* bias, void* c, int64_t m, int64_t n, int64_t k,
+                        int64_t lda, int64_t ldw, int64_t ldc, int epilogue, const void* r, int64_t ldr, const float* gate,
+                        int64_t mod_stride, const int32_t* sel, int dtype, void* c2, int64_t ldc2, int64_t n_split, void* keep,
+                        int64_t ldk, int tile_m) {
     FINO_CHECK(dtype == FINO_BF16 || dtype == FINO_F16, FINO_ERR_ARG, "fino_gemm: dtype %d", dtype);
     FINO_CHECK(tile_m == 0 || (tile_m >= 2 && tile_m <= 8), FINO_ERR_ARG, "fino_gemm: tile_m=%d (0 = planned, 2 .. 8)", tile_m);
     if (c2 || n_split) {
@@ -817,7 +1098,7 @@
     if (epilogue == FINO_EPI_GATED_RESIDUAL || epilogue == FINO_EPI_GATED_RESIDUAL_STAGED)
         FINO_CHECK(gate && fino_aligned16(gate) && mod_stride % 4 == 0, FINO_ERR_ARG, "fino_gemm: gate operand");
     if (m == 0) return FINO_OK;
-    GemmParams p = {};
+    p = {};
     p.c2 = (uint16_t*)c2; p.ldc2 = ldc2; p.n_split = n_split;
     if (keep) { p.c2 = (uint16_t*)keep; p.ldc2 = ldk; p.n_split = 0; }
     p.a = (const uint16_t*)a; p.w = (const uint16_t*)w; p.bias = (const uint16_t*)bias; p.c = (uint16_t*)c;
@@ -826,13 +1107,16 @@
     p.tiles_m = (int)((m + BM - 1) / BM);
     p.tiles_n = (int)((n + BN - 1) / BN);
     p.group_m = fino_tune_get(FINO_TUNE_GEMM_GROUP_M);
-    hipStream_t st = (hipStream_t)stream;
-    const bool generic = (k % BK) != 0;
     if (p.group_m <= 0) p.group_m = gemm_default_group_m(p.tiles_n, k);
     {
         const int rk = fino_tune_get(FINO_TUNE_GEMM_RASTER);
         if (rk == 1 || (rk == 3 && (k >= 8192 || n >= 8192)) || (rk != 2 && rk != 3 && k >= 8192)) p.group_m |= 0x100;
     }
+    return FINO_OK;
+}
+
+static int gemm_dispatch(const GemmParams& p, int epilogue, int dtype, bool keep, int tile_m, hipStream_t st) {
+    const bool generic = (p.k % BK) != 0;
     if (keep) {
         if (dtype == FINO_BF16)
             return generic ? launch_gemm_e<BF16, true, true>(p, epilogue, tile_m, st)
@@ -843,6 +1127,40 @@
     if (dtype == FINO_BF16)
         return generic ? launch_gemm_e<BF16, true>(p, epilogue, tile_m, st) : launch_gemm_e<BF16, false>(p, epilogue, tile_m, st);
     return generic ? launch_gemm_e<F16, true>(p, epilogue, tile_m, st) : launch_gemm_e<F16, false>(p, epilogue, tile_m, st);
+}
+
+static int gemm_impl(const void* a, const void* w, const void* bias, void* c, int64_t m, int64_t n, int64_t k, int64_t lda,
+                     int64_t ldw, int64_t ldc, int epilogue, const void* r, int64_t ldr, const float* gate,
+                     int64_t mod_stride, const int32_t* sel, int dtype, void* c2, int64_t ldc2, int64_t n_split, void* keep,
+                     int64_t ldk, int tile_m, void* stream) {
+    GemmParams p = {};
+    if (int rc = gemm_prepare(p, a, w, bias, c, m, n, k, lda, ldw, ldc, epilogue, r, ldr, gate, mod_stride, sel, dtype, c2, ldc2,
+                              n_split, keep, ldk, tile_m))
+        return rc;
+    if (m == 0) return FINO_OK;
+    return gemm_dispatch(p, epilogue, dtype, keep != nullptr, tile_m, (hipStream_t)stream);
+}
+
+extern "C" int fino_gemm_pair(const void* a0, const void* w0, void* c0, const void* r0, const int32_t* sel0, int64_t m0,
+                              int64_t k0, int64_t lda0, int64_t ldw0, int64_t ldc0, int64_t ldr0, const void* a1, const void* w1,
+                              void* c1, const void* r1, const int32_t* sel1, int64_t m1, int64_t k1, int64_t lda1, int64_t ldw1,
+                              int64_t ldc1, int64_t ldr1, const void* bias, int64_t n, int epilogue, const float* gate,
+                              int64_t mod_stride, int dtype, void* stream) {
+    FINO_CHECK(epilogue != FINO_EPI_F32 && epilogue != FINO_EPI_F32_RESIDUAL, FINO_ERR_ARG,
+               "fino_gemm_pair: epilogue %d (the fp32-output epilogues take one problem: fino_gemm)", epilogue);
+    GemmParams p0 = {}, p1 = {};
+    if (int rc = gemm_prepare(p0, a0, w0, bias, c0, m0, n, k0, lda0, ldw0, ldc0, epilogue, r0, ldr0, gate, mod_stride, sel0, dtype,
+                              nullptr, 0, 0, nullptr, 0, 0))
+        return rc;
+    if (int rc = gemm_prepare(p1, a1, w1, bias, c1, m1, n, k1, lda1, ldw1, ldc1, epilogue, r1, ldr1, gate, mod_stride, sel1, dtype,
+                              nullptr, 0, 0, nullptr, 0, 0))
+        return rc;
+    hipStream_t st = (hipStream_t)stream;
+    if (m0 > 0 && m1 > 0 && sk_wanted(p0, epilogue, 0) && sk_wanted(p1, epilogue, 0))
+        return dtype == FINO_BF16 ? launch_gemm_sk<BF16>(p0, &p1, epilogue, st) : launch_gemm_sk<F16>(p0, &p1, epilogue, st);
+    if (m0 > 0)
+        if (int rc = gemm_dispatch(p0, epilogue, dtype, false, 0, st)) return rc;
+    return m1 > 0 ? gemm_dispatch(p1, epilogue, dtype, false, 0, st) : FINO_OK;
 }
 
 extern "C" int fino_gemm_split_n(const void* a, const void* w, const void* bias, void* c, int64_t m, int64_t n, int64_t k,
diff --git a/frameino_amd/ops.py b/frameino_amd/ops.py
--- a/frameino_amd/ops.py
+++ b/frameino_amd/ops.py
@@ -490,6 +490,38 @@
     return out
 
 
+def attention_probs_per_sample(q, k, heads, lk_b, tail_mult, kps, outs, scale=None, q_rrms=None, q_weight=None):
+    import ctypes
+    assert q.dim() == 3 and k.dim() == 3
+    b, lq, hd = q.shape
+    lk = k.shape[1]
+    dh = hd // heads
+    for t in (q, k):
+        assert t.stride(2) == 1 and t.is_cuda
+    assert len(kps) == b and len(outs) == b and len(lk_b) == b and len(tail_mult) == b
+    for o_, kp in zip(outs, kps):
+        assert o_.shape == (lq, heads * kp) and o_.stride(1) == 1 and o_.dtype == q.dtype and o_.is_cuda
+    scale = dh ** -0.5 if scale is None else scale
+    lk_arr = (ctypes.c_int * b)(*[int(x) for x in lk_b])
+    mult_arr = (ctypes.c_float * b)(*[float(x) for x in tail_mult])
+    p_arr = (ctypes.c_void_p * b)(*[o_.data_ptr() for o_ in outs])
+    kp_arr = (ctypes.c_int * b)(*[int(x) for x in kps])
+    rs_arr = (ctypes.c_int64 * b)(*[o_.stride(0) for o_ in outs])
+    ev = _timed("attn_cross")
+    _lib.check(_lib.lib().fino_attn_probs_per_sample(_p(q), _p(k), ctypes.cast(p_arr, ctypes.c_void_p),
+                                                    ctypes.cast(kp_arr, ctypes.c_void_p), ctypes.cast(rs_arr, ctypes.c_void_p),
+                                                    b, heads, lq, lk, dh, q.stride(0), q.stride(1), dh, k.stride(0), k.stride(1),
+                                                    dh, float(scale), _dt(q), ctypes.cast(lk_arr, ctypes.c_void_p),
+                                                    ctypes.cast(mult_arr, ctypes.c_void_p), _p(q_rrms),
+                                                    q_rrms.stride(0) if q_rrms is not None else 0, _p(q_weight), _stream()),
+               "fino_attn_probs_per_sample")
+    if ev is not None:
+        ev.record()
+        kt_ = KernelTimer.active
+        kt_.flops["attn_cross"] = kt_.flops.get("attn_cross", 0.0) + 2.0 * lq * hd * sum(int(x) for x in lk_b)
+    return outs
+
+
 _attn_fp8_ws = {}
 
 
@@ -660,6 +692,35 @@
     return out
 
 
+def gemm_pair(a, w, bias=None, epilogue=EPI_NONE, residual=(None, None), gate=None, sel=(None, None), out=(None, None)):
+    a2, w2, o2, r2, ms, flops, byts = [], [], [], [], 0, 0.0, 0.0
+    outs = list(out)
+    n = w[0].shape[0]
+    for i in range(2):
+        ai, m, k, lda = _rows2d(a[i])
+        wi = w[i]
+        assert wi.dim() == 2 and wi.stride(1) == 1 and wi.shape == (n, k) and wi.dtype == ai.dtype == a[0].dtype
+        if outs[i] is None:
+            outs[i] = torch.empty((m, n), dtype=ai.dtype, device=ai.device)
+        oi, om, on, ldc = _rows2d(outs[i])
+        assert (om, on) == (m, n)
+        ri, ldr, ms = _epi_operands(residual[i], gate)
+        a2.append((ai, m, k, lda)); w2.append(wi); o2.append((oi, ldc)); r2.append((ri, ldr))
+        flops += 2.0 * m * n * k
+        byts += 2.0 * (m * k + n * k + m * n * (2 if residual[i] is not None else 1))
+    if bias is not None:
+        assert bias.dtype == a[0].dtype and bias.is_contiguous()
+    done = _timed_gemm(epilogue, flops, byts)
+    args = []
+    for i in range(2):
+        (ai, m, k, lda), (oi, ldc), (ri, ldr) = a2[i], o2[i], r2[i]
+        args += [_p(ai), _p(w2[i]), _p(oi), _p(ri), _p(sel[i]), m, k, lda, w2[i].stride(0), ldc, ldr]
+    _lib.check(_lib.lib().fino_gemm_pair(*args, _p(bias), n, epilogue, _p(gate), ms, _dt(a[0]), _stream()), "fino_gemm_pair")
+    if done is not None:
+        done()
+    return tuple(outs)
+
+
 def gemm_blocked_a(a_blocks, rows, w, bias, residual, gate, sel, out, tile_m=0):
     if a_blocks.dim() == 3:
         a_blocks = a_blocks[None]
diff --git a/frameino_amd/transformer_wan.py b/frameino_amd/transformer_wan.py
--- a/frameino_amd/transformer_wan.py
+++ b/frameino_amd/transformer_wan.py
@@ -133,6 +133,7 @@
         self._init_self_attention_options()
         self.dedup_text_padding = os.environ.get("FINO_TEXT_FOLD", "1") != "0"
         self.reassociate_text_out = os.environ.get("FINO_TEXT_REASSOC", "1") != "0"
+        self.text_tail_pair = True
         self.skip_dead_rows = os.environ.get("FINO_SKIP_DEAD_ROWS", "1") != "0"
 
     @property
@@ -737,6 +738,14 @@
             rr = text.rrms
             for r0, r1 in segs:
                 o.row_rrms(q2[r0:r1], a2.norm_q.eps, out=rr[r0:r1])
+            if b == 2 and c.keep is None and not c.tk and self.text_tail_pair and hasattr(o, "gemm_pair"):
+                ns = s1 - s0
+                pbs = [text.pbuf[i][:ns] for i in range(2)]
+                o.attention_probs_per_sample(q2.view(b, n, d)[:, s0:s1], kv[:, :, :d], heads, text.tail[0], text.tail[1],
+                                             text.kp, pbs, q_rrms=rr[:b * n].view(b, n)[:, s0:s1], q_weight=a2.norm_q.weight)
+                xs = tuple(x[i * n + s0:i * n + s1] for i in range(2))
+                o.gemm_pair(pbs, text.w2[li], a2.to_out[0].bias, o.EPI_RESIDUAL, residual=xs, out=xs)
+                return
             for i in range(b):
                 r0, r1 = i * n + s0, i * n + s1
                 pr = o.attention_probs(q2[r0:r1].view(1, s1 - s0, d), kv[i:i + 1, :, :d], heads, text.tail[0][i:i + 1],
diff --git a/include/frameino_hip.h b/include/frameino_hip.h
--- a/include/frameino_hip.h
+++ b/include/frameino_hip.h
@@ -20,7 +20,8 @@
 const char* fino_last_error(void);
 
 enum { FINO_TUNE_GEMM_GROUP_M = 0, FINO_TUNE_GEMM_RASTER = 1, FINO_TUNE_CONV_LOOP = 2, FINO_TUNE_GEMM_TILE_M = 3,
-       FINO_TUNE_ATTN_KERNEL = 4, FINO_TUNE_ATTN_FP8_KERNEL = 5, FINO_TUNE_ATTN_WALK_GRID = 6, FINO_TUNE_COUNT = 8 };
+       FINO_TUNE_ATTN_KERNEL = 4, FINO_TUNE_ATTN_FP8_KERNEL = 5, FINO_TUNE_ATTN_WALK_GRID = 6, FINO_TUNE_GEMM_SHORT_K = 7,
+       FINO_TUNE_COUNT = 8 };
 int fino_tune_set(int key, int value);
 int fino_tune_get(int key);
 
@@ -136,6 +137,11 @@
                     int64_t q_bs, int64_t q_rs, int64_t q_hs, int64_t k_bs, int64_t k_rs, int64_t k_hs, int kp, int64_t p_bs,
                     int64_t p_rs, float scale, int dtype, const int* lk_b, const float* tail_mult, const float* q_rrms,
                     int64_t q_rrms_bs, const void* q_weight, void* stream);
+int fino_attn_probs_per_sample(const void* q, const void* k, void* const* p_b, const int* kp_b, const int64_t* p_rs_b, int batch,
+                               int heads, int64_t lq, int64_t lk, int head_dim, int64_t q_bs, int64_t q_rs, int64_t q_hs,
+                               int64_t k_bs, int64_t k_rs, int64_t k_hs, float scale, int dtype, const int* lk_b,
+                               const float* tail_mult, const float* q_rrms, int64_t q_rrms_bs, const void* q_weight,
+                               void* stream);
 int fino_row_rrms(const void* x, int64_t rows, int dim, int64_t ldx, float eps, float* rrms, int dtype, void* stream);
 
 int64_t fino_attn_partial_bytes(int batch, int heads, int64_t lq, int head_dim);
@@ -165,6 +171,11 @@
 int fino_gemm_keep(const void* a, const void* w, const void* bias, void* c, int64_t m, int64_t n, int64_t k, int64_t lda,
                    int64_t ldw, int64_t ldc, int epilogue, const void* r, int64_t ldr, const float* gate,
                    int64_t mod_stride, const int32_t* sel, int dtype, void* keep, int64_t ldk, int tile_m, void* stream);
+int fino_gemm_pair(const void* a0, const void* w0, void* c0, const void* r0, const int32_t* sel0, int64_t m0, int64_t k0,
+                   int64_t lda0, int64_t ldw0, int64_t ldc0, int64_t ldr0, const void* a1, const void* w1, void* c1,
+                   const void* r1, const int32_t* sel1, int64_t m1, int64_t k1, int64_t lda1, int64_t ldw1, int64_t ldc1,
+                   int64_t ldr1, const void* bias, int64_t n, int epilogue, const float* gate, int64_t mod_stride, int dtype,
+                   void* stream);
 int fino_gemm_blocked_a(const void* a, const void* w, const void* bias, void* c, int64_t m, int64_t n, int64_t k,
                         int64_t a_block_k, int64_t a_block_stride, int a_groups, int64_t a_group_stride, int64_t lda,
                         int64_t ldw, int64_t ldc, const void* r, int64_t ldr, const float* gate, int64_t mod_stride,
```

Measured after the change: 3.741 denoise-steps/s, median of 6. Within noise of the previous version (+0.2%).
